# graphdeco-inria/nerfshop

Measured on AMD Instinct MI355X. Metric: render_msamples_per_s_1080p, higher is better.
Workload: dtype f16 storage / f32 accumulate (MFMA), f32 marching+compositing; 1 GPU; lego-like snapshot 1920x1080, one cage edit (BASELINE configs[2]/[4]); samples_per_frame=25213758, frames_in_flight=1, cell_records=levels 0..11, 9.2 GB (nrs_model_set_cell_cache default)

## Files before the change

### include/nrs.h

```cpp
#ifndef NRS_H
#define NRS_H

#include <stddef.h>
#include <stdint.h>

#ifdef __cplusplus
extern "C" {
#endif

#define NRS_ABI_VERSION 3

typedef enum nrs_status {
	NRS_OK = 0,
	NRS_ERR_INVALID_ARG = -1,
	NRS_ERR_UNSUPPORTED = -2,
	NRS_ERR_HIP = -3,
	NRS_ERR_NO_DEVICE = -4,
	NRS_ERR_STATE = -5
} nrs_status;

typedef enum nrs_activation {
	NRS_ACT_NONE = 0, NRS_ACT_RELU = 1, NRS_ACT_LOGISTIC = 2, NRS_ACT_EXPONENTIAL = 3
} nrs_activation;

typedef enum nrs_render_mode {
	NRS_RENDER_AO = 0, NRS_RENDER_SHADE = 1, NRS_RENDER_NORMALS = 2, NRS_RENDER_POSITIONS = 3,
	NRS_RENDER_DEPTH = 4, NRS_RENDER_DISTANCE = 5, NRS_RENDER_STEPSIZE = 6, NRS_RENDER_DISTORTION = 7,
	NRS_RENDER_COST = 8, NRS_RENDER_SLICE = 9, NRS_RENDER_ENCODING_VIS = 11
} nrs_render_mode;

typedef enum nrs_layout { NRS_PLANES = 0, NRS_INTERLEAVED = 1 } nrs_layout;

typedef enum nrs_grid_acc { NRS_GRID_ACC_FP32 = 0, NRS_GRID_ACC_NETWORK = 1 } nrs_grid_acc;
typedef enum nrs_mlp_acc { NRS_MLP_ACC_FP32 = 0, NRS_MLP_ACC_FP16 = 1 } nrs_mlp_acc;

typedef struct nrs_model_desc {
	uint32_t n_levels;
	uint32_t n_features_per_level;
	uint32_t log2_hashmap_size;
	uint32_t base_resolution;
	float    per_level_scale;
	uint32_t n_neurons;
	uint32_t density_hidden_layers;
	uint32_t density_output_dims;
	uint32_t rgb_hidden_layers;
	uint32_t sh_degree;
	uint32_t rgb_activation;
	uint32_t density_activation;
	float    aabb_min[3];
	float    aabb_max[3];
} nrs_model_desc;

#define NRS_GRID_SIZE       128u
#define NRS_GRID_CASCADES   5u
#define NRS_GRID_VOLUME     (128u * 128u * 128u)
#define NRS_BITFIELD_BYTES  (NRS_GRID_VOLUME * NRS_GRID_CASCADES / 8u)
#define NRS_NETWORK_INPUT_FLOATS 7u
#define NRS_NETWORK_OUTPUT_WIDTH 16u

typedef struct nrs_tet_mesh {
	uint32_t        n_vertices;
	uint32_t        n_tets;
	const float*    h_vertices;
	const float*    h_original_vertices;
	const uint32_t* h_tets;
	const uint32_t* h_lut_offsets;
	const uint32_t* h_lut_idx;
	const uint8_t*  h_original_bitfield;
	const float*    h_local_rotations;
	uint32_t        copy;
	uint32_t        apply_poisson;
	float           residual_amplitude;
	const float*    h_boundary_shs;
	const float*    h_boundary_outside_density;
	const float*    h_boundary_residual_density;
	uint32_t        correct_direction;
} nrs_tet_mesh;

typedef struct nrs_affine_duplication {
	float    selection_center[3];
	float    selection_scale[3];
	float    selection_rot[9];
	float    translation[3];
	float    scale[3];
	float    rotation[9];
	uint32_t hide_original;
	uint32_t correct_dir;
} nrs_affine_duplication;

typedef struct nrs_render_params {
	uint32_t struct_size;
	int32_t  resolution[2];
	float    focal_length[2];
	float    camera_matrix0[12];
	float    camera_matrix1[12];
	float    rolling_shutter[4];
	float    screen_center[2];
	float    render_aabb_min[3];
	float    render_aabb_max[3];
	uint32_t spp_index;
	uint32_t snap_to_pixel_centers;
	float    min_transmittance;
	float    cone_angle_constant;
	uint32_t render_mode;
	uint32_t linear_colors;
	uint32_t apply_operators;
	uint32_t poisson_target;
	uint32_t min_mip;
	uint32_t max_march_steps;
	uint32_t tile_size;
	uint32_t tile_first;
	uint32_t tile_stride;
	float    dof;
	float    slice_plane_z;
	float    depth_scale;
	uint32_t show_accel;
	uint32_t distortion_mode;
	float    distortion_params[7];
	const float* d_distortion_map;
	int32_t  distortion_resolution[2];
	int32_t  envmap_resolution[2];
	const float* d_envmap;
	uint32_t glow_mode;
	float    glow_y_cutoff;
	uint32_t visualized_layer;
	uint32_t visualized_dimension;
} nrs_render_params;
#define NRS_RENDER_PARAMS_INIT { (uint32_t)sizeof(nrs_render_params) }

typedef struct nrs_render_stats {
	uint64_t n_samples;
	uint32_t n_rays_alive;
	uint32_t n_rays_hit;
} nrs_render_stats;

typedef struct nrs_grid_update {
	uint32_t n_uniform_samples;
	uint32_t n_nonuniform_samples;
	uint32_t reset_grid;
	uint32_t max_cascade;
	float    decay;
	uint32_t ema_step;
	uint64_t rng_state;
	uint64_t rng_inc;
} nrs_grid_update;

typedef struct nrs_ctx   nrs_ctx;
typedef struct nrs_model nrs_model;
typedef struct nrs_edit  nrs_edit;

const char* nrs_last_error(void);
int         nrs_abi_version(void);

int  nrs_ctx_create(int device, nrs_ctx** out);
void nrs_ctx_destroy(nrs_ctx* ctx);
int  nrs_ctx_device_info(const nrs_ctx* ctx, char* name_out, size_t name_len, int* n_cus, size_t* hbm_bytes);
int  nrs_ctx_set_lane_teams(nrs_ctx* ctx, int lanes_per_ray);
int  nrs_ctx_set_ray_handover(nrs_ctx* ctx, int enabled);
int  nrs_ctx_ray_handovers(const nrs_ctx* ctx, uint64_t* n_rays, uint64_t* n_handovers);

int    nrs_model_create(nrs_ctx* ctx, const nrs_model_desc* desc, nrs_model** out);
void   nrs_model_destroy(nrs_model* model);
size_t nrs_model_n_params(const nrs_model_desc* desc);
int    nrs_model_level_table(const nrs_model_desc* desc, float* scale, uint32_t* resolution,
                             uint32_t* entry_offset, uint32_t* entry_count, uint32_t* hashed);
int    nrs_model_set_params(nrs_model* model, const void* h_params_fp16, size_t n_params);
int    nrs_model_set_params_device(nrs_model* model, const void* d_params_fp16, size_t n_params, void* stream);
int    nrs_model_set_numerics(nrs_model* model, uint32_t grid_acc, uint32_t mlp_acc);
int    nrs_model_set_cell_cache(nrs_model* model, size_t max_bytes);
size_t nrs_model_cell_cache_bytes(const nrs_model* model, uint32_t* n_levels_out);
int    nrs_model_set_sparse_cell_cache(nrs_model* model, const uint8_t* h_mask_bitfield, size_t max_bytes);
size_t nrs_model_sparse_cell_cache_bytes(const nrs_model* model, uint32_t* first_level_out, uint32_t* n_levels_out);
int    nrs_model_set_density_bitfield(nrs_model* model, const uint8_t* h_bitfield, size_t n_bytes);
int    nrs_model_set_density_grid(nrs_model* model, const float* h_grid, size_t n_floats);
int    nrs_model_get_density_bitfield(nrs_model* model, uint8_t* h_bitfield_out, size_t n_bytes);
int    nrs_model_get_march_accelerator(nrs_model* model, int which, float* h_box12, uint32_t* h_mask1024);
int    nrs_model_get_density_grid(nrs_model* model, float* h_grid_out, size_t n_floats);
int    nrs_model_update_density_grid(nrs_model* model, nrs_edit* const* edits, int n_edits, nrs_grid_update* u, void* stream);
void   nrs_rng_seed(uint64_t seed, uint64_t* state_out, uint64_t* inc_out);

typedef struct nrs_comm nrs_comm;
int  nrs_comm_unique_id(uint8_t* out128);
int  nrs_comm_create(int device, int rank, int n_ranks, const uint8_t* unique_id128, nrs_comm** out);
void nrs_comm_destroy(nrs_comm* comm);
int  nrs_comm_info(const nrs_comm* comm, int* rank_out, int* n_ranks_out, int* rccl_version_out, char* lib_path_out, size_t lib_path_len);
int  nrs_comm_probe_self_p2p(nrs_comm* comm, const float* d_src, float* d_dst, size_t n_floats, int pairs, void* stream);
int  nrs_gather_tiles(nrs_ctx* ctx, nrs_comm* comm, int root, const nrs_render_params* p, uint32_t tiles_per_rank_padded, const float* d_local,
                      float* d_recv, float* d_image, float* d_depth, void* stream);

int nrs_network_inference(nrs_model* model, void* stream, uint32_t n, const float* d_in,
                          void* d_out_fp16, uint32_t ld_out, int layout);
int nrs_network_density(nrs_model* model, void* stream, uint32_t n, const float* d_in, uint32_t ld_in,
                        void* d_out_fp16, uint32_t ld_out, int layout);
int nrs_network_input_gradient(nrs_model* model, void* stream, uint32_t n, const float* d_in, uint32_t ld_in, float* d_grad_out_nx3);
int nrs_network_visualize_activation(nrs_model* model, void* stream, uint32_t layer, uint32_t dimension, uint32_t n, const float* d_in, float* d_out_n);
int nrs_network_backward(nrs_model* model, void* stream, uint32_t n, const float* d_in, uint32_t ld_in,
                         const void* d_dL_doutput_fp16, uint32_t ld_dout, int layout, float* d_dL_dparams, size_t n_params, int accumulate,
                         float* d_dL_dinput);
int nrs_density_on_grid(nrs_model* model, void* stream, const uint32_t res3d[3], const float aabb_min[3], const float aabb_max[3],
                        int mask_with_density_grid, float* d_out);
int nrs_rgba_on_grid(nrs_model* model, void* stream, const uint32_t res3d[3], const float render_aabb_min[3],
                     const float render_aabb_max[3], const float ray_dir[3], float* d_out_rgba);
int nrs_project_selection_pixels(nrs_model* model, void* stream, const nrs_render_params* params, const int32_t* d_pixels_xy,
                                 uint32_t n_pixels, float transmittance_threshold, float* d_positions, uint32_t* d_cells, uint8_t* d_found);
uint32_t nrs_upper_cell_idx(uint32_t cell_idx, uint32_t target_level);
int nrs_selection_cells(const float* h_positions, const uint32_t* h_cells, const uint8_t* h_found, uint32_t n, int automatic_max_level,
                        uint32_t* growing_level_inout, uint32_t* out_cells, float* out_positions, uint32_t* n_out);
int  nrs_poisson_boundary(nrs_model* model, const float* h_vertices, uint32_t n_verts, uint32_t sh_width, uint32_t hemisphere_width,
                          const float* h_jitter, int is_inside, float* h_density_out, float* h_sh_out);
void nrs_poisson_sample_coords(const float* vertices, uint32_t n_verts, uint32_t sh_width, uint32_t hemisphere_width, const float* jitter,
                               const float aabb_min[3], const float aabb_max[3], float* coords7_out);
int nrs_hashgrid_encode(nrs_model* model, void* stream, uint32_t n, const float* d_in, uint32_t ld_in,
                        void* d_out_fp16);

int  nrs_edit_create(nrs_ctx* ctx, const nrs_model_desc* desc, const nrs_tet_mesh* mesh, nrs_edit** out);
int  nrs_edit_create_affine(nrs_ctx* ctx, const nrs_model_desc* desc, const nrs_affine_duplication* op, nrs_edit** out);
void nrs_edit_destroy(nrs_edit* edit);
int  nrs_edit_map_rays(nrs_edit* edit, void* stream, uint32_t n, float* d_coords, uint8_t* d_empty_mask);
int  nrs_edit_map_positions(nrs_edit* edit, void* stream, uint32_t n, float* d_pos, uint32_t ld,
                            uint8_t* d_empty_mask);

int  nrs_edit_set_mvc(nrs_edit* edit, const float* h_weights, uint32_t n_cage_vertices);
int  nrs_edit_update_cage(nrs_edit* edit, void* stream, const float* h_cage_vertices, uint32_t n_cage_vertices);
int  nrs_edit_update_vertices(nrs_edit* edit, void* stream, const float* h_vertices, uint32_t n_vertices);
int  nrs_edit_lut_size(const nrs_edit* edit, uint32_t* n_idx_out, uint32_t* max_per_cell_out);
int  nrs_edit_poisson_interpolate(nrs_edit* edit, void* stream, const float* h_gamma, uint32_t n_cage_vertices, const float* h_inside_density,
                                  const float* h_outside_density, const float* h_inside_shs, const float* h_outside_shs, float residual_amplitude);
int  nrs_edit_download_poisson(nrs_edit* edit, float* h_boundary_shs, float* h_outside_density, float* h_residual_density);
int  nrs_edit_download(nrs_edit* edit, float* h_vertices, uint32_t* h_lut_offsets, uint32_t* h_lut_idx, float* h_rotations,
                       uint8_t* h_original_bitfield, float* h_bbox6);

int nrs_render_nerf(nrs_model* model, const nrs_render_params* params, nrs_edit* const* edits, int n_edits,
                    float* d_frame, float* d_depth, uint32_t* d_steps, void* stream, nrs_render_stats* h_stats);
typedef enum nrs_color_space { NRS_COLOR_LINEAR = 0, NRS_COLOR_SRGB = 1, NRS_COLOR_VISPOSNEG = 2 } nrs_color_space;
int nrs_accumulate(nrs_ctx* ctx, void* stream, uint32_t width, uint32_t height, const float* d_frame, float* d_accumulate, uint32_t sample_count, uint32_t color_space);
uint32_t nrs_render_owned_tiles(const nrs_render_params* params);
uint32_t nrs_render_tile_pitch(const nrs_render_params* params);
int nrs_detile(nrs_ctx* ctx, void* stream, const nrs_render_params* params, uint32_t n_ranks,
               uint32_t tiles_per_rank_padded, const float* d_tiles, uint32_t channels, size_t rank_stride_floats, float* d_image);
int nrs_trace_samples(nrs_model* model, const nrs_render_params* params, void* stream, uint32_t n_pixels,
                      const uint32_t* d_pixel_idx, uint32_t max_samples, float* d_t, float* d_dt, uint32_t* d_count);

typedef struct nrs_snapshot nrs_snapshot;
int          nrs_snapshot_open(const char* path, nrs_snapshot** out);
void         nrs_snapshot_close(nrs_snapshot* snapshot);
int          nrs_snapshot_model_desc(const nrs_snapshot* snapshot, nrs_model_desc* desc_out, uint32_t* aabb_scale_out);
const void*  nrs_snapshot_params_fp16(const nrs_snapshot* snapshot, size_t* n_params_out);
const float* nrs_snapshot_density_grid(const nrs_snapshot* snapshot, size_t* n_floats_out);
int          nrs_snapshot_camera(const nrs_snapshot* snapshot, float* camera_matrix12_out);
typedef struct nrs_edits nrs_edits;
int          nrs_edits_open(const char* path, nrs_edits** out);
void         nrs_edits_close(nrs_edits* edits);
uint32_t     nrs_edits_count(const nrs_edits* edits);
const char*  nrs_edits_type(const nrs_edits* edits, uint32_t i);
int          nrs_edits_affine(const nrs_edits* edits, uint32_t i, nrs_affine_duplication* op_out);
int          nrs_edits_cage(const nrs_edits* edits, uint32_t i, nrs_tet_mesh* mesh_out, const float** h_mvc_weights_out,
                            const float** h_cage_vertices_out, const float** h_cage_original_vertices_out,
                            const uint32_t** h_cage_triangles_out, uint32_t* n_cage_vertices_out, uint32_t* n_cage_triangles_out);

typedef struct nrs_tet_lut nrs_tet_lut;
int  nrs_tet_lut_build(const float* h_vertices, uint32_t n_vertices, const uint32_t* h_tets, uint32_t n_tets,
                       int n_threads, nrs_tet_lut** out);
uint32_t        nrs_tet_lut_n_idx(const nrs_tet_lut* lut);
uint32_t        nrs_tet_lut_max_per_cell(const nrs_tet_lut* lut);
const uint32_t* nrs_tet_lut_offsets(const nrs_tet_lut* lut);
const uint32_t* nrs_tet_lut_idx(const nrs_tet_lut* lut);
const uint8_t*  nrs_tet_lut_bitfield(const nrs_tet_lut* lut);
void            nrs_tet_lut_destroy(nrs_tet_lut* lut);
int nrs_mvc_compute(const float* h_cage_vertices, uint32_t n_cage_vertices, const uint32_t* h_cage_triangles,
                    uint32_t n_cage_triangles, const float* h_points, uint32_t n_points,
                    float* h_weights_out, uint8_t* h_labels_out);
int nrs_mvc_apply(const float* h_weights, const float* h_cage_vertices, uint32_t n_cage_vertices,
                  uint32_t n_points, float* h_points_out);
int nrs_tet_local_rotations(const float* h_vertices, const float* h_original_vertices, const uint32_t* h_tets,
                            uint32_t n_tets, float* h_rotations_out);

#define NRS_SPP_BATCH_MAX 64u
#define NRS_SPP_BATCH_MAX_RESOLUTION 8192
int nrs_render_nerf_spp(nrs_model* model, const nrs_render_params* params, nrs_edit* const* edits, int n_edits, uint32_t spp_count,
                        float* d_frames, float* d_depths, uint32_t* d_steps, size_t slab_stride_pixels, void* stream, nrs_render_stats* h_stats);
int nrs_accumulate_spp(nrs_ctx* ctx, void* stream, uint32_t width, uint32_t height, const float* d_frames, size_t slab_stride_pixels, uint32_t spp_count,
                       float* d_accumulate, uint32_t sample_count, uint32_t color_space);
int nrs_ctx_render_launches(const nrs_ctx* ctx, uint64_t* n_dispatches_out, uint32_t* last_schedule_out);

typedef struct nrs_sample_view {
	float camera_matrix0[12], camera_matrix1[12];
	float focal_length[2];
	float dof;
	float slice_plane_z;
} nrs_sample_view;
int nrs_render_nerf_spp_views(nrs_model* model, const nrs_render_params* params, nrs_edit* const* edits, int n_edits, uint32_t spp_count, const nrs_sample_view* h_views,
                              float* d_frames, float* d_depths, uint32_t* d_steps, size_t slab_stride_pixels, void* stream, nrs_render_stats* h_stats);

typedef struct nrs_camera_keyframe { float R[4], T[3], slice, scale, fov, dof; } nrs_camera_keyframe;
typedef struct nrs_camera_path nrs_camera_path;
int nrs_log_space_lerp(const float begin[12], const float end[12], float t, float out[12]);
int nrs_camera_keyframe_matrix(const nrs_camera_keyframe* key, float out[12]);
int nrs_camera_keyframe_from_matrix(const float matrix[12], float slice, float scale, float fov, float dof, nrs_camera_keyframe* out);
int nrs_camera_path_eval(const nrs_camera_keyframe* keys, uint32_t n_keys, float t, nrs_camera_keyframe* out);
int nrs_camera_path_open(const char* path, nrs_camera_path** out);
uint32_t nrs_camera_path_count(const nrs_camera_path* path);
int nrs_camera_path_keyframes(const nrs_camera_path* path, nrs_camera_keyframe* out, uint32_t capacity);
void nrs_camera_path_close(nrs_camera_path* path);
int nrs_motion_views(const float start[12], const float end[12], float shutter_fraction, uint32_t spp_count, uint32_t first_sample, uint32_t spp_total,
                     const int32_t resolution[2], int fov_axis, const nrs_camera_keyframe* keys, uint32_t n_keys, float start_time, float end_time,
                     const nrs_sample_view* base_view, nrs_sample_view* out_views);

int    nrs_model_create_ex(nrs_ctx* ctx, const nrs_model_desc* desc, uint32_t n_extra_dims, nrs_model** out);
size_t nrs_model_n_params_ex(const nrs_model_desc* desc, uint32_t n_extra_dims);
int    nrs_model_n_extra_dims(const nrs_model* model);
int    nrs_model_set_light_dir(nrs_model* model, const float dir[3]);
int    nrs_network_inference_strided(nrs_model* model, void* stream, uint32_t n, const float* d_in, uint32_t ld_in, void* d_out_fp16, uint32_t ld_out, int layout);
#define NRS_SNAPSHOT_ALLOW_LIGHT_DIRS 1u
int      nrs_snapshot_open_ex(const char* path, uint32_t flags, nrs_snapshot** out);
uint32_t nrs_snapshot_n_extra_dims(const nrs_snapshot* snapshot);

typedef enum nrs_tonemap_curve { NRS_TONEMAP_IDENTITY = 0, NRS_TONEMAP_ACES = 1, NRS_TONEMAP_HABLE = 2, NRS_TONEMAP_REINHARD = 3 } nrs_tonemap_curve;
#define NRS_TONEMAP_RGBA32F 0u
#define NRS_TONEMAP_RGBA8 1u
typedef struct nrs_tonemap_params {
	uint32_t struct_size;
	float    exposure;
	float    background_color[4];
	uint32_t color_space;
	uint32_t output_color_space;
	uint32_t tonemap_curve;
	uint32_t clamp_output;
	uint32_t output_format;
} nrs_tonemap_params;
// ... 120 lines not shown
```

### nerfshop_amd/_abi.py

```python
import ctypes as C
import os

_HERE = os.path.dirname(os.path.abspath(__file__))
LIB_PATH = os.environ.get("NRS_LIB_PATH") or os.path.join(_HERE, "csrc", "libnrs.so")

NRS_OK = 0
GRID_SIZE = 128
GRID_CASCADES = 5
GRID_VOLUME = GRID_SIZE ** 3
BITFIELD_BYTES = GRID_VOLUME * GRID_CASCADES // 8
N_LUT_CELLS = GRID_VOLUME * GRID_CASCADES

ACT_NONE, ACT_RELU, ACT_LOGISTIC, ACT_EXPONENTIAL = 0, 1, 2, 3
RENDER_AO, RENDER_SHADE, RENDER_NORMALS, RENDER_POSITIONS, RENDER_DEPTH, RENDER_DISTANCE, RENDER_STEPSIZE, RENDER_DISTORTION, RENDER_COST, RENDER_SLICE = range(10)
RENDER_ENCODING_VIS = 11
LAYOUT_PLANES, LAYOUT_INTERLEAVED = 0, 1


class ModelDesc(C.Structure):
    _fields_ = [
        ("n_levels", C.c_uint32),
        ("n_features_per_level", C.c_uint32),
        ("log2_hashmap_size", C.c_uint32),
        ("base_resolution", C.c_uint32),
# ... 45 lines not shown


class RenderParams(C.Structure):
    _fields_ = [
        ("struct_size", C.c_uint32),
        ("resolution", C.c_int32 * 2),
        ("focal_length", C.c_float * 2),
        ("camera_matrix0", C.c_float * 12),
        ("camera_matrix1", C.c_float * 12),
        ("rolling_shutter", C.c_float * 4),
        ("screen_center", C.c_float * 2),
        ("render_aabb_min", C.c_float * 3),
        ("render_aabb_max", C.c_float * 3),
        ("spp_index", C.c_uint32),
        ("snap_to_pixel_centers", C.c_uint32),
        ("min_transmittance", C.c_float),
        ("cone_angle_constant", C.c_float),
        ("render_mode", C.c_uint32),
        ("linear_colors", C.c_uint32),
        ("apply_operators", C.c_uint32),
        ("poisson_target", C.c_uint32),
        ("min_mip", C.c_uint32),
        ("max_march_steps", C.c_uint32),
        ("tile_size", C.c_uint32),
        ("tile_first", C.c_uint32),
        ("tile_stride", C.c_uint32),
        ("dof", C.c_float),
        ("slice_plane_z", C.c_float),
        ("depth_scale", C.c_float),
        ("show_accel", C.c_uint32),
        ("distortion_mode", C.c_uint32),
        ("distortion_params", C.c_float * 7),
        ("d_distortion_map", C.c_void_p),
        ("distortion_resolution", C.c_int32 * 2),
        ("envmap_resolution", C.c_int32 * 2),
        ("d_envmap", C.c_void_p),
        ("glow_mode", C.c_uint32),
        ("glow_y_cutoff", C.c_float),
        ("visualized_layer", C.c_uint32),
        ("visualized_dimension", C.c_uint32),
    ]

    def __init__(self, *args, **kw):
        super().__init__(*args, **kw)
        self.struct_size = C.sizeof(RenderParams)


class RenderStats(C.Structure):
    _fields_ = [("n_samples", C.c_uint64), ("n_rays_alive", C.c_uint32), ("n_rays_hit", C.c_uint32)]


class GridUpdate(C.Structure):
    _fields_ = [
        ("n_uniform_samples", C.c_uint32),
        ("n_nonuniform_samples", C.c_uint32),
        ("reset_grid", C.c_uint32),
        ("max_cascade", C.c_uint32),
        ("decay", C.c_float),
        ("ema_step", C.c_uint32),
        ("rng_state", C.c_uint64),
        ("rng_inc", C.c_uint64),
    ]


class TonemapParams(C.Structure):
    _fields_ = [
        ("struct_size", C.c_uint32),
        ("exposure", C.c_float),
        ("background_color", C.c_float * 4),
        ("color_space", C.c_uint32),
        ("output_color_space", C.c_uint32),
        ("tonemap_curve", C.c_uint32),
        ("clamp_output", C.c_uint32),
        ("output_format", C.c_uint32),
    ]

    def __init__(self, *args, **kw):
        super().__init__(*args, **kw)
        self.struct_size = C.sizeof(TonemapParams)


class SampleView(C.Structure):
    _fields_ = [("camera_matrix0", C.c_float * 12), ("camera_matrix1", C.c_float * 12), ("focal_length", C.c_float * 2), ("dof", C.c_float), ("slice_plane_z", C.c_float)]


class CameraKeyframe(C.Structure):
    _fields_ = [("R", C.c_float * 4), ("T", C.c_float * 3), ("slice", C.c_float), ("scale", C.c_float), ("fov", C.c_float), ("dof", C.c_float)]


LOSS_L2, LOSS_L1, LOSS_MAPE, LOSS_SMAPE, LOSS_HUBER, LOSS_LOG_L1, LOSS_RELATIVE_L2 = range(7)


class RayLossParams(C.Structure):
    _fields_ = [("struct_size", C.c_uint32), ("loss_type", C.c_uint32), ("loss_scale", C.c_float), ("color_space", C.c_uint32), ("train_in_linear_colors", C.c_uint32),
                ("background", C.c_float * 3), ("near_distance", C.c_float), ("density_l1_reg", C.c_uint32), ("max_samples_compacted", C.c_uint32)]

    def __init__(self, **kw):
        super().__init__()
        self.struct_size = C.sizeof(RayLossParams)
        self.loss_type, self.loss_scale, self.color_space, self.train_in_linear_colors = LOSS_L2, 128.0, 0, 0
        for k, v in kw.items():
            if k == "background":
                self.background = (C.c_float * 3)(*[float(x) for x in v])
            elif k in dict(self._fields_):
                setattr(self, k, v)
            else:
                raise TypeError(f"RayLossParams has no field {k}")


class AdamParams(C.Structure):
    _fields_ = [("struct_size", C.c_uint32), ("beta1", C.c_float), ("beta2", C.c_float), ("epsilon", C.c_float), ("l2_reg", C.c_float),
                ("non_matrix_lr_factor", C.c_float), ("ema_decay", C.c_float)]

    def __init__(self, **kw):
        super().__init__()
        self.struct_size = C.sizeof(AdamParams)
        self.beta1, self.beta2, self.epsilon, self.l2_reg, self.non_matrix_lr_factor, self.ema_decay = 0.9, 0.99, 1e-15, 1e-6, 1.0, 0.95
        for k, v in kw.items():
            if k not in dict(self._fields_):
                raise TypeError(f"AdamParams has no field {k}")
            setattr(self, k, v)


class TrainingCamera(C.Structure):
    _fields_ = [("struct_size", C.c_uint32), ("xform_start", C.c_float * 12), ("xform_end", C.c_float * 12), ("focal_length", C.c_float * 2),
                ("principal_point", C.c_float * 2), ("rolling_shutter", C.c_float * 4), ("distortion_mode", C.c_uint32), ("distortion_params", C.c_float * 7)]

    def __init__(self, *args, **kw):
        super().__init__(*args, **kw)
        self.struct_size = C.sizeof(TrainingCamera)


class DatasetRaysParams(C.Structure):
    _fields_ = [("struct_size", C.c_uint32), ("n_rays_total", C.c_uint32), ("rng_state", C.c_uint64), ("rng_inc", C.c_uint64), ("snap_to_pixel_centers", C.c_uint32),
                ("random_bg_color", C.c_uint32)]

    def __init__(self, *args, **kw):
        super().__init__(*args, **kw)
        self.struct_size = C.sizeof(DatasetRaysParams)


IMAGE_RGBA8_SRGB, IMAGE_RGBA32F_LINEAR, IMAGE_RGBA16F_LINEAR = 0, 1, 2
IMAGE_WHITE_TRANSPARENT, IMAGE_BLACK_TRANSPARENT = 1, 2
RNG_STEP_DELTA = 1 << 32
OPT_MASTER, OPT_M, OPT_V, OPT_STEPS, OPT_EMA, OPT_PARAMS_FP16 = range(6)
OPT_EXPORT_WEIGHTS, OPT_EXPORT_EMA = 0, 1
BASE_LEARNING_RATE, BASE_DECAY_START, BASE_DECAY_INTERVAL, BASE_DECAY_BASE = 1e-2, 20000, 10000, 0.33

EXPORTS = [
    "nrs_last_error", "nrs_abi_version", "nrs_edit_poisson_interpolate", "nrs_edit_download_poisson", "nrs_comm_unique_id", "nrs_comm_create", "nrs_comm_info", "nrs_comm_destroy", "nrs_gather_tiles", "nrs_comm_probe_self_p2p",
    "nrs_ctx_create", "nrs_ctx_destroy", "nrs_ctx_device_info", "nrs_ctx_set_lane_teams", "nrs_ctx_set_ray_handover", "nrs_ctx_ray_handovers",
    "nrs_model_create", "nrs_model_destroy", "nrs_model_n_params", "nrs_model_level_table",
    "nrs_model_set_params", "nrs_model_set_params_device", "nrs_model_set_numerics", "nrs_model_set_cell_cache", "nrs_model_cell_cache_bytes", "nrs_model_set_sparse_cell_cache", "nrs_model_sparse_cell_cache_bytes", "nrs_model_set_density_bitfield", "nrs_model_set_density_grid",
    "nrs_model_get_density_bitfield", "nrs_model_get_march_accelerator", "nrs_model_get_density_grid", "nrs_model_update_density_grid", "nrs_rng_seed",
    "nrs_network_inference", "nrs_network_density", "nrs_hashgrid_encode", "nrs_density_on_grid", "nrs_rgba_on_grid", "nrs_network_input_gradient", "nrs_network_visualize_activation",
    "nrs_poisson_boundary", "nrs_poisson_sample_coords", "nrs_project_selection_pixels", "nrs_upper_cell_idx", "nrs_selection_cells",
    "nrs_edit_create", "nrs_edit_create_affine", "nrs_edit_destroy", "nrs_edit_map_rays", "nrs_edit_map_positions",
    "nrs_edit_set_mvc", "nrs_edit_update_cage", "nrs_edit_update_vertices", "nrs_edit_lut_size", "nrs_edit_download",
    "nrs_render_nerf", "nrs_render_owned_tiles", "nrs_render_tile_pitch", "nrs_detile", "nrs_trace_samples", "nrs_accumulate",
    "nrs_snapshot_open", "nrs_snapshot_close", "nrs_snapshot_model_desc", "nrs_snapshot_params_fp16", "nrs_snapshot_density_grid",
    "nrs_snapshot_camera", "nrs_edits_open", "nrs_edits_close", "nrs_edits_count", "nrs_edits_type", "nrs_edits_cage", "nrs_edits_affine",
    "nrs_tet_lut_build", "nrs_tet_lut_n_idx", "nrs_tet_lut_max_per_cell", "nrs_tet_lut_offsets",
    "nrs_tet_lut_idx", "nrs_tet_lut_bitfield", "nrs_tet_lut_destroy",
    "nrs_mvc_compute", "nrs_mvc_apply", "nrs_tet_local_rotations",
    "nrs_render_nerf_spp", "nrs_accumulate_spp", "nrs_ctx_render_launches",
    "nrs_model_create_ex", "nrs_model_n_params_ex", "nrs_model_n_extra_dims", "nrs_model_set_light_dir", "nrs_network_inference_strided",
    "nrs_snapshot_open_ex", "nrs_snapshot_n_extra_dims",
    "nrs_tonemap", "nrs_accumulate_spp_tonemap", "nrs_tonemap_output_bytes",
    "nrs_render_nerf_spp_views", "nrs_log_space_lerp", "nrs_camera_keyframe_matrix", "nrs_camera_keyframe_from_matrix", "nrs_camera_path_eval",
    "nrs_camera_path_open", "nrs_camera_path_count", "nrs_camera_path_keyframes", "nrs_camera_path_close", "nrs_motion_views",
    "nrs_marching_cubes_res", "nrs_marching_cubes_table", "nrs_mesh_write", "nrs_mesh_from_density", "nrs_mesh_extract", "nrs_mesh_color_inputs",
    "nrs_mesh_counts", "nrs_mesh_device", "nrs_mesh_download", "nrs_mesh_destroy",
    "nrs_selection_create", "nrs_selection_destroy", "nrs_selection_reset", "nrs_selection_grow", "nrs_selection_upscale", "nrs_selection_state",
    "nrs_selection_get_cells", "nrs_selection_get_bitfield", "nrs_selection_set_structuring_elements", "nrs_bitfield_morph", "nrs_bitfield_morph_host",
    "nrs_selection_dilate", "nrs_selection_erode", "nrs_selection_fine_mesh",
    "nrs_network_backward",
    "nrs_training_samples", "nrs_ray_loss",
    "nrs_adam_bias_table", "nrs_exponential_decay_lr", "nrs_optimizer_create", "nrs_optimizer_create_for_model", "nrs_optimizer_destroy", "nrs_optimizer_set_weights",
    "nrs_optimizer_step", "nrs_optimizer_get_state", "nrs_optimizer_set_state", "nrs_optimizer_export_fp16", "nrs_optimizer_step_count", "nrs_optimizer_set_step_count",
    "nrs_optimizer_n_params",
    "nrs_dataset_create", "nrs_dataset_destroy", "nrs_dataset_set_image", "nrs_dataset_set_camera", "nrs_dataset_get_image", "nrs_dataset_rays", "nrs_dataset_mark_untrained", "nrs_rng_advance",
]
SNAPSHOT_ALLOW_LIGHT_DIRS = 1
SPP_BATCH_MAX = 64
COLOR_LINEAR, COLOR_SRGB, COLOR_VISPOSNEG = 0, 1, 2
TONEMAP_IDENTITY, TONEMAP_ACES, TONEMAP_HABLE, TONEMAP_REINHARD = 0, 1, 2, 3
TONEMAP_RGBA32F, TONEMAP_RGBA8 = 0, 1
SE_CUBE, SE_SPHERE = 0, 1
MORPH_DILATE, MORPH_ERODE = 0, 1
MESH_THRESH_DEFAULT = 2.5

_lib = None


class NrsError(RuntimeError):
    pass


def load():
    global _lib
    if _lib is not None:
        return _lib
    if not os.path.exists(LIB_PATH):
        raise NrsError(
            f"{LIB_PATH} is missing: the HIP extension has not been built "
            "(run `python -c 'import __graft_entry__ as g; g.build()'`). There is no CPU fallback.")
    import torch
    lib = C.CDLL(LIB_PATH)
    P, U32, I = C.c_void_p, C.c_uint32, C.c_int
    lib.nrs_last_error.restype = C.c_char_p
    lib.nrs_abi_version.restype = I
    lib.nrs_ctx_create.argtypes = [I, C.POINTER(P)]
    lib.nrs_ctx_destroy.argtypes = [P]
    lib.nrs_ctx_destroy.restype = None
    lib.nrs_ctx_device_info.argtypes = [P, C.c_char_p, C.c_size_t, C.POINTER(I), C.POINTER(C.c_size_t)]
    lib.nrs_model_create.argtypes = [P, C.POINTER(ModelDesc), C.POINTER(P)]
    lib.nrs_ctx_set_lane_teams.argtypes = [P, C.c_int]
    lib.nrs_ctx_set_ray_handover.argtypes = [P, C.c_int]
    lib.nrs_ctx_ray_handovers.argtypes = [P, C.POINTER(C.c_uint64), C.POINTER(C.c_uint64)]
    lib.nrs_model_destroy.argtypes = [P]
    lib.nrs_model_destroy.restype = None
    lib.nrs_model_n_params.argtypes = [C.POINTER(ModelDesc)]
    lib.nrs_model_n_params.restype = C.c_size_t
    lib.nrs_model_level_table.argtypes = [C.POINTER(ModelDesc), P, P, P, P, P]
    lib.nrs_model_set_params.argtypes = [P, P, C.c_size_t]
    lib.nrs_project_selection_pixels.argtypes = [P, P, C.POINTER(RenderParams), P, C.c_uint32, C.c_float, P, P, P]
    lib.nrs_poisson_boundary.argtypes = [P, P, C.c_uint32, C.c_uint32, C.c_uint32, P, C.c_int, P, P]
    lib.nrs_poisson_sample_coords.argtypes = [P, C.c_uint32, C.c_uint32, C.c_uint32, P, P, P, P]
    lib.nrs_poisson_sample_coords.restype = None
    lib.nrs_upper_cell_idx.argtypes = [C.c_uint32, C.c_uint32]
    lib.nrs_upper_cell_idx.restype = C.c_uint32
    lib.nrs_selection_cells.argtypes = [P, P, P, C.c_uint32, C.c_int, P, P, P, P]
    lib.nrs_model_set_cell_cache.argtypes = [P, C.c_size_t]
    lib.nrs_model_cell_cache_bytes.argtypes = [P, P]
    lib.nrs_model_cell_cache_bytes.restype = C.c_size_t
    lib.nrs_model_set_numerics.argtypes = [P, C.c_uint32, C.c_uint32]
    lib.nrs_model_set_params_device.argtypes = [P, P, C.c_size_t, P]
    lib.nrs_edit_poisson_interpolate.argtypes = [P, P, P, C.c_uint32, P, P, P, P, C.c_float]
    lib.nrs_edit_download_poisson.argtypes = [P, P, P, P]
    lib.nrs_comm_unique_id.argtypes = [P]
    lib.nrs_comm_create.argtypes = [C.c_int, C.c_int, C.c_int, P, P]
    lib.nrs_comm_info.argtypes = [P, P, P, P, P, C.c_size_t]
    lib.nrs_comm_destroy.argtypes = [P]
    lib.nrs_comm_destroy.restype = None
    lib.nrs_gather_tiles.argtypes = [P, P, C.c_int, P, C.c_uint32, P, P, P, P, P]
    lib.nrs_comm_probe_self_p2p.argtypes = [P, P, P, C.c_size_t, C.c_int, P]
    lib.nrs_model_set_sparse_cell_cache.argtypes = [P, P, C.c_size_t]
    lib.nrs_model_sparse_cell_cache_bytes.argtypes = [P, P, P]
    lib.nrs_model_sparse_cell_cache_bytes.restype = C.c_size_t
    lib.nrs_model_set_density_bitfield.argtypes = [P, P, C.c_size_t]
    lib.nrs_model_set_density_grid.argtypes = [P, P, C.c_size_t]
    lib.nrs_model_get_density_bitfield.argtypes = [P, P, C.c_size_t]
    lib.nrs_model_get_density_grid.argtypes = [P, P, C.c_size_t]
    lib.nrs_model_get_march_accelerator.argtypes = [P, I, P, P]
    lib.nrs_model_update_density_grid.argtypes = [P, C.POINTER(P), I, C.POINTER(GridUpdate), P]
    lib.nrs_rng_seed.argtypes = [C.c_uint64, C.POINTER(C.c_uint64), C.POINTER(C.c_uint64)]
    lib.nrs_rng_seed.restype = None
    lib.nrs_network_inference.argtypes = [P, P, U32, P, P, U32, I]
    lib.nrs_network_density.argtypes = [P, P, U32, P, U32, P, U32, I]
    lib.nrs_hashgrid_encode.argtypes = [P, P, U32, P, U32, P]
    lib.nrs_network_input_gradient.argtypes = [P, P, U32, P, U32, P]
    lib.nrs_network_visualize_activation.argtypes = [P, P, U32, U32, U32, P, P]
    if hasattr(lib, "nrs_network_backward"):
        lib.nrs_network_backward.argtypes = [P, P, U32, P, U32, P, U32, I, P, C.c_size_t, I, P]
    if hasattr(lib, "nrs_ray_loss"):
        lib.nrs_training_samples.argtypes = [P, P, U32, P, P, C.c_float, U32, P, U32, P, P, P]
        lib.nrs_ray_loss.argtypes = [P, P, C.POINTER(RayLossParams), U32, P, P, U32, P, U32, P, U32, I, P, P, P, P, P, P, U32, I, P, P]
    if hasattr(lib, "nrs_optimizer_step"):
        lib.nrs_adam_bias_table.argtypes = [C.c_float, C.c_float, P, U32, C.POINTER(U32)]
        lib.nrs_exponential_decay_lr.argtypes = [C.c_float, U32, U32, C.c_float, U32]
        lib.nrs_exponential_decay_lr.restype = C.c_float
        lib.nrs_optimizer_create.argtypes = [P, C.c_size_t, C.c_size_t, C.POINTER(AdamParams), C.POINTER(P)]
        lib.nrs_optimizer_create_for_model.argtypes = [P, C.POINTER(AdamParams), C.POINTER(P)]
        lib.nrs_optimizer_destroy.argtypes = [P]
        lib.nrs_optimizer_destroy.restype = None
        lib.nrs_optimizer_set_weights.argtypes = [P, P, I, P]
        lib.nrs_optimizer_step.argtypes = [P, P, P, C.c_float, C.c_float, I]
        lib.nrs_optimizer_get_state.argtypes = [P, I, P, C.c_size_t]
        lib.nrs_optimizer_set_state.argtypes = [P, I, P, C.c_size_t]
        lib.nrs_optimizer_export_fp16.argtypes = [P, I, P, P]
        lib.nrs_optimizer_step_count.argtypes = [P]
        lib.nrs_optimizer_step_count.restype = U32
        lib.nrs_optimizer_set_step_count.argtypes = [P, U32]
        lib.nrs_optimizer_n_params.argtypes = [P, C.POINTER(C.c_size_t)]
        lib.nrs_optimizer_n_params.restype = C.c_size_t
    if hasattr(lib, "nrs_dataset_rays"):
        lib.nrs_dataset_create.argtypes = [P, U32, U32, U32, C.POINTER(P)]
        lib.nrs_dataset_destroy.argtypes = [P]
        lib.nrs_dataset_destroy.restype = None
        lib.nrs_dataset_set_image.argtypes = [P, U32, I, P, I, U32, U32, P]
        lib.nrs_dataset_set_camera.argtypes = [P, U32, C.POINTER(TrainingCamera)]
        lib.nrs_dataset_get_image.argtypes = [P, U32, P]
        lib.nrs_dataset_rays.argtypes = [P, P, C.POINTER(DatasetRaysParams), U32, P, P, P, P, P]
        lib.nrs_dataset_mark_untrained.argtypes = [P, P, I, P]
        lib.nrs_rng_advance.argtypes = [C.POINTER(C.c_uint64), C.c_uint64, C.c_uint64]
        lib.nrs_rng_advance.restype = None
    lib.nrs_density_on_grid.argtypes = [P, P, C.POINTER(U32 * 3), C.POINTER(C.c_float * 3), C.POINTER(C.c_float * 3), I, P]
    lib.nrs_rgba_on_grid.argtypes = [P, P, C.POINTER(U32 * 3), C.POINTER(C.c_float * 3), C.POINTER(C.c_float * 3), C.POINTER(C.c_float * 3), P]
    lib.nrs_edit_create.argtypes = [P, C.POINTER(ModelDesc), C.POINTER(TetMesh), C.POINTER(P)]
    lib.nrs_edit_create_affine.argtypes = [P, C.POINTER(ModelDesc), C.POINTER(AffineDuplicationOp), C.POINTER(P)]
    lib.nrs_edits_affine.argtypes = [P, U32, C.POINTER(AffineDuplicationOp)]
    lib.nrs_edit_destroy.argtypes = [P]
    lib.nrs_edit_destroy.restype = None
    lib.nrs_edit_map_rays.argtypes = [P, P, U32, P, P]
    lib.nrs_edit_map_positions.argtypes = [P, P, U32, P, U32, P]
    lib.nrs_edit_set_mvc.argtypes = [P, P, U32]
    lib.nrs_edit_update_cage.argtypes = [P, P, P, U32]
    lib.nrs_edit_update_vertices.argtypes = [P, P, P, U32]
    lib.nrs_edit_lut_size.argtypes = [P, C.POINTER(U32), C.POINTER(U32)]
    lib.nrs_edit_download.argtypes = [P, P, P, P, P, P, P]
    lib.nrs_render_nerf.argtypes = [P, C.POINTER(RenderParams), C.POINTER(P), I, P, P, P, P, C.POINTER(RenderStats)]
    lib.nrs_render_owned_tiles.argtypes = [C.POINTER(RenderParams)]
    lib.nrs_render_owned_tiles.restype = U32
    lib.nrs_render_tile_pitch.argtypes = [C.POINTER(RenderParams)]
    lib.nrs_render_tile_pitch.restype = U32
    lib.nrs_detile.argtypes = [P, P, C.POINTER(RenderParams), U32, U32, P, U32, C.c_size_t, P]
    lib.nrs_trace_samples.argtypes = [P, C.POINTER(RenderParams), P, U32, P, U32, P, P, P]
    lib.nrs_accumulate.argtypes = [P, P, U32, U32, P, P, U32, U32]
    if hasattr(lib, "nrs_render_nerf_spp"):
        lib.nrs_render_nerf_spp.argtypes = [P, C.POINTER(RenderParams), C.POINTER(P), I, U32, P, P, P, C.c_size_t, P, C.POINTER(RenderStats)]
        lib.nrs_accumulate_spp.argtypes = [P, P, U32, U32, P, C.c_size_t, U32, P, U32, U32]
        lib.nrs_ctx_render_launches.argtypes = [P, C.POINTER(C.c_uint64), C.POINTER(U32)]
    if hasattr(lib, "nrs_model_create_ex"):
        lib.nrs_model_create_ex.argtypes = [P, C.POINTER(ModelDesc), U32, C.POINTER(P)]
        lib.nrs_model_n_params_ex.argtypes = [C.POINTER(ModelDesc), U32]
        lib.nrs_model_n_params_ex.restype = C.c_size_t
        lib.nrs_model_n_extra_dims.argtypes = [P]
        lib.nrs_model_set_light_dir.argtypes = [P, C.POINTER(C.c_float * 3)]
        lib.nrs_network_inference_strided.argtypes = [P, P, U32, P, U32, P, U32, I]
        lib.nrs_snapshot_open_ex.argtypes = [C.c_char_p, U32, C.POINTER(P)]
        lib.nrs_snapshot_n_extra_dims.argtypes = [P]
        lib.nrs_snapshot_n_extra_dims.restype = U32
    if hasattr(lib, "nrs_tonemap"):
        lib.nrs_tonemap.argtypes = [P, P, U32, U32, P, C.POINTER(TonemapParams), P]
        lib.nrs_accumulate_spp_tonemap.argtypes = [P, P, U32, U32, P, C.c_size_t, U32, P, U32, C.POINTER(TonemapParams), P]
        lib.nrs_tonemap_output_bytes.argtypes = [U32, U32, U32]
        lib.nrs_tonemap_output_bytes.restype = C.c_size_t
    if hasattr(lib, "nrs_render_nerf_spp_views"):
        F12 = C.POINTER(C.c_float * 12)
        lib.nrs_render_nerf_spp_views.argtypes = [P, C.POINTER(RenderParams), C.POINTER(P), I, U32, P, P, P, P, C.c_size_t, P, C.POINTER(RenderStats)]
        lib.nrs_log_space_lerp.argtypes = [F12, F12, C.c_float, F12]
        lib.nrs_camera_keyframe_matrix.argtypes = [C.POINTER(CameraKeyframe), F12]
        lib.nrs_camera_keyframe_from_matrix.argtypes = [F12, C.c_float, C.c_float, C.c_float, C.c_float, C.POINTER(CameraKeyframe)]
        lib.nrs_camera_path_eval.argtypes = [P, U32, C.c_float, C.POINTER(CameraKeyframe)]
        lib.nrs_camera_path_open.argtypes = [C.c_char_p, C.POINTER(P)]
        lib.nrs_camera_path_count.argtypes = [P]
        lib.nrs_camera_path_count.restype = U32
        lib.nrs_camera_path_keyframes.argtypes = [P, P, U32]
        lib.nrs_camera_path_close.argtypes = [P]
        lib.nrs_camera_path_close.restype = None
        lib.nrs_motion_views.argtypes = [F12, F12, C.c_float, U32, U32, U32, C.POINTER(C.c_int32 * 2), I, P, U32, C.c_float, C.c_float, C.POINTER(SampleView), P]
    if hasattr(lib, "nrs_mesh_from_density"):
        F3, U3 = C.POINTER(C.c_float * 3), C.POINTER(U32 * 3)
        lib.nrs_marching_cubes_res.argtypes = [U32, F3, F3, U3]
        lib.nrs_marching_cubes_table.argtypes = [P, C.POINTER(U32)]
        lib.nrs_mesh_write.argtypes = [C.c_char_p, U32, P, P, P, U32, P, C.c_float, F3]
        lib.nrs_mesh_from_density.argtypes = [P, P, U3, F3, F3, C.c_float, P, C.POINTER(P)]
        lib.nrs_mesh_extract.argtypes = [P, P, U3, F3, F3, C.c_float, I, I, C.POINTER(P)]
        lib.nrs_mesh_color_inputs.argtypes = [P, P, P, P]
        lib.nrs_mesh_counts.argtypes = [P, C.POINTER(U32), C.POINTER(U32), C.POINTER(U32)]
        lib.nrs_mesh_device.argtypes = [P, C.POINTER(P), C.POINTER(P), C.POINTER(P), C.POINTER(P), C.POINTER(P)]
        lib.nrs_mesh_download.argtypes = [P, P, P, P, P, P]
        lib.nrs_mesh_destroy.argtypes = [P]
        lib.nrs_mesh_destroy.restype = None
    if hasattr(lib, "nrs_selection_create"):
        PU32 = C.POINTER(U32)
        lib.nrs_selection_create.argtypes = [P, C.c_size_t, U32, C.POINTER(P)]
        lib.nrs_selection_destroy.argtypes = [P]
        lib.nrs_selection_destroy.restype = None
        lib.nrs_selection_reset.argtypes = [P, P, U32, U32]
        lib.nrs_selection_grow.argtypes = [P, C.c_float, U32, U32, PU32]
        lib.nrs_selection_upscale.argtypes = [P]
        lib.nrs_selection_state.argtypes = [P, PU32, PU32, PU32, C.POINTER(I)]
        lib.nrs_selection_get_cells.argtypes = [P, P, P]
        lib.nrs_selection_get_bitfield.argtypes = [P, P]
        lib.nrs_selection_set_structuring_elements.argtypes = [P, I, I, I, I]
        lib.nrs_bitfield_morph.argtypes = [P, P, P, U32, I, I, I, P]
        lib.nrs_bitfield_morph_host.argtypes = [P, U32, I, I, I, P]
        lib.nrs_selection_dilate.argtypes = [P, P, P]
        lib.nrs_selection_erode.argtypes = [P, P, P]
        lib.nrs_selection_fine_mesh.argtypes = [P, P, P, I, C.POINTER(P)]
    lib.nrs_snapshot_open.argtypes = [C.c_char_p, C.POINTER(P)]
    lib.nrs_snapshot_close.argtypes = [P]
    lib.nrs_snapshot_close.restype = None
    lib.nrs_snapshot_model_desc.argtypes = [P, C.POINTER(ModelDesc), C.POINTER(U32)]
    lib.nrs_snapshot_params_fp16.argtypes = [P, C.POINTER(C.c_size_t)]
    lib.nrs_snapshot_params_fp16.restype = P
    lib.nrs_snapshot_density_grid.argtypes = [P, C.POINTER(C.c_size_t)]
    lib.nrs_snapshot_density_grid.restype = P
    lib.nrs_snapshot_camera.argtypes = [P, P]
    lib.nrs_edits_open.argtypes = [C.c_char_p, C.POINTER(P)]
    lib.nrs_edits_close.argtypes = [P]
    lib.nrs_edits_close.restype = None
    lib.nrs_edits_count.argtypes = [P]
    lib.nrs_edits_count.restype = U32
    lib.nrs_edits_type.argtypes = [P, U32]
    lib.nrs_edits_type.restype = C.c_char_p
    lib.nrs_edits_cage.argtypes = [P, U32, C.POINTER(TetMesh), C.POINTER(P), C.POINTER(P), C.POINTER(P), C.POINTER(P), C.POINTER(U32), C.POINTER(U32)]
    lib.nrs_tet_lut_build.argtypes = [P, U32, P, U32, I, C.POINTER(P)]
    for name in ("nrs_tet_lut_n_idx", "nrs_tet_lut_max_per_cell"):
        getattr(lib, name).argtypes = [P]
        getattr(lib, name).restype = U32
    for name in ("nrs_tet_lut_offsets", "nrs_tet_lut_idx", "nrs_tet_lut_bitfield"):
        getattr(lib, name).argtypes = [P]
        getattr(lib, name).restype = P
    lib.nrs_tet_lut_destroy.argtypes = [P]
    lib.nrs_tet_lut_destroy.restype = None
# ... 11 lines not shown
```

### nerfshop_amd/csrc/nrs_api_model.cpp

```cpp
#include "nrs_host.h"
#include "nrs_optimizer.h"

#include <cmath>
#include <cstdio>
#include <cstdlib>
#include <new>

using namespace nrs;

static int refresh_accel(nrs_model* m, void* stream) {
	hipStream_t s = (hipStream_t)stream;
	float* d_out = reinterpret_cast<float*>(m->d_accel_masks.get() + 2 * kCoarseWords);
	NRS_LAUNCH(launch_occ_accel(m->dm.bitfield, m->d_accel_masks.get(), d_out, m->d_accel_masks.get() + 2 * kCoarseWords + 24, stream));
	float h[24];
	HIP_TRY(hipMemcpyAsync(h, d_out, sizeof(h), hipMemcpyDeviceToHost, s));
	HIP_TRY(hipStreamSynchronize(s));
	OccAccel* acc[2] = {&m->accel_any, &m->accel_exact};
	for (int f = 0; f < 2; ++f)
		for (int k = 0; k < 3; ++k) {
			acc[f]->box.mn[k] = h[f * 12 + k];
			acc[f]->box.mx[k] = h[f * 12 + 3 + k];
			acc[f]->cell[k] = h[f * 12 + 6 + k];
			acc[f]->inv_cell[k] = h[f * 12 + 9 + k];
		}
	m->accel_any.mask = m->d_accel_masks.get();
	m->accel_exact.mask = m->d_accel_masks.get() + kCoarseWords;
	return NRS_OK;
}
DeviceModel nrs::model_for_launch(const nrs_model* m, const nrs_render_params& p) {
	DeviceModel dm = m->dm;
	dm.occ = (p.cone_angle_constant == 0.f && p.min_mip == 0) ? m->accel_exact : m->accel_any;
	return dm;
}
int nrs::model_refresh_bitfield(nrs_model* m, void* stream) {
	hipStream_t s = (hipStream_t)stream;
	HIP_TRY(hipMemsetAsync(m->d_bitfield.get(), 0, NRS_BITFIELD_BYTES, s));
	NRS_LAUNCH(launch_grid_to_bitfield(m->d_density_grid.get(), m->d_bitfield.get(), m->ctx->d_mean.get(), stream));
	NRS_TRY(refresh_accel(m, stream));
	m->have_bitfield = true;
	return NRS_OK;
}

extern "C" {

static void update_light(nrs_model* m) {
	const float* l = m->light_dir;
	const float n = std::sqrt(l[0] * l[0] + l[1] * l[1] + l[2] * l[2]);
	for (int k = 0; k < 3; ++k) m->dm.light01[k] = (l[k] / n + 1.0f) * 0.5f;
}
int nrs_model_n_extra_dims(const nrs_model* m) { return m ? (int)m->n_extra_dims : 0; }
int nrs_model_set_light_dir(nrs_model* m, const float dir[3]) {
	if (!m || !dir) return fail(NRS_ERR_INVALID_ARG, "nrs_model_set_light_dir: NULL argument");
	const float n2 = dir[0] * dir[0] + dir[1] * dir[1] + dir[2] * dir[2];
	if (!std::isfinite(n2) || !(n2 > 0.f)) return fail(NRS_ERR_INVALID_ARG, "nrs_model_set_light_dir: the direction must be finite and non-zero (it is normalised at use)");
	for (int k = 0; k < 3; ++k) m->light_dir[k] = dir[k];
	update_light(m);
	return NRS_OK;
}
static int model_create(nrs_ctx* ctx, const nrs_model_desc* desc, uint32_t n_extra_dims, nrs_model** out, const char* who) {
	if (!ctx || !desc || !out) return fail(NRS_ERR_INVALID_ARG, std::string(who) + ": NULL argument");
	if (n_extra_dims != 0u && n_extra_dims != 3u) return fail(NRS_ERR_UNSUPPORTED, "nrs_model_create_ex: n_extra_dims must be 0 or 3 (light directions, dataset.has_light_dirs)");
	if (desc_supported(*desc))
		if (const char* why = extra_dims_refusal(*desc, n_extra_dims)) return fail(NRS_ERR_UNSUPPORTED, std::string("nrs_model_create_ex: ") + why);
	if (!desc_supported(*desc)) return fail(NRS_ERR_UNSUPPORTED, "model description outside configs/nerf/base.json's family (hash grid 16 x 2, 64-wide density network of 0..1 hidden layers, rgb network of 0..3 hidden layers or none)");
	for (int k = 0; k < 3; ++k)
		if (!(desc->aabb_max[k] > desc->aabb_min[k])) return fail(NRS_ERR_INVALID_ARG, std::string(who) + ": empty aabb");
	HIP_TRY(hipSetDevice(ctx->device));
	nrs_model* m = new (std::nothrow) nrs_model();
	if (!m) return fail(NRS_ERR_STATE, "out of host memory");
	m->ctx = ctx;
	m->desc = *desc;
	m->total_entries = make_levels(*desc, m->dm.levels);
	for (int k = 0; k < 3; ++k) { m->dm.aabb.mn[k] = desc->aabb_min[k]; m->dm.aabb.mx[k] = desc->aabb_max[k]; }
	m->dm.diag_pow2 = 1;
	for (int k = 0; k < 3; ++k) {
		const float diag = desc->aabb_max[k] - desc->aabb_min[k];
		int e = 0;
		if (std::frexp(diag, &e) != 0.5f) m->dm.diag_pow2 = 0;
		m->dm.inv_diag[k] = 1.0f / diag;
	}
	m->dm.rgb_deep = desc->sh_degree != 0 && desc->rgb_hidden_layers == 3 ? 1u : 0u;
	m->dm.no_dir = desc->sh_degree == 0 ? 1u : 0u;
	m->n_extra_dims = m->dm.n_extra_dims = n_extra_dims;
	update_light(m);
	m->dm.rgb_activation = desc->rgb_activation;
	m->dm.density_activation = desc->density_activation;
	hipError_t he = m->d_grid.alloc(m->total_entries);
	if (he == hipSuccess) he = m->d_wfrag.alloc(kWfragDeviceBytes / 2);
	if (he == hipSuccess) he = m->d_bitfield.alloc(NRS_BITFIELD_BYTES);
	if (he == hipSuccess) he = m->d_accel_masks.alloc(2 * kCoarseWords + 64);
	if (he == hipSuccess) he = hipMemset(m->d_accel_masks.get(), 0, 2 * kCoarseWords * 4);
	if (he == hipSuccess) he = m->d_density_grid.alloc((size_t)kGridVol * kCascades);
	if (he == hipSuccess) he = hipMemset(m->d_density_grid.get(), 0, (size_t)kGridVol * kCascades * 4);
	if (he != hipSuccess) {
		nrs_model_destroy(m);
		return fail_hip(he, n_extra_dims ? "nrs_model_create_ex: device allocation" : "nrs_model_create: device allocation");
	}
	m->dm.grid = m->d_grid.get();
	m->dm.wfrag = m->d_wfrag.get();
	m->dm.bitfield = m->d_bitfield.get();
	if (const char* e = getenv("NRS_CELL_CACHE_GB")) {
		size_t budget = (size_t)(atof(e) * 1073741824.0), free_b = 0, total_b = 0;
		if (hipMemGetInfo(&free_b, &total_b) == hipSuccess) budget = std::min(budget, free_b / 4);
		if (nrs_model_set_cell_cache(m, budget) != NRS_OK) (void)nrs_model_set_cell_cache(m, 0);
	}
	*out = m;
	return NRS_OK;
}
int nrs_model_create(nrs_ctx* ctx, const nrs_model_desc* desc, nrs_model** out) { return model_create(ctx, desc, 0u, out, "nrs_model_create"); }
int nrs_model_create_ex(nrs_ctx* ctx, const nrs_model_desc* desc, uint32_t n_extra_dims, nrs_model** out) { return model_create(ctx, desc, n_extra_dims, out, "nrs_model_create_ex"); }
void nrs_model_destroy(nrs_model* m) {
	delete m;
}
static uint32_t plan_cell_cache(const LevelParams* lv, size_t budget, LevelParams* out, size_t* bytes) {
	uint32_t n = 0;
	uint64_t records = 0, fit = 0;
	for (uint32_t l = 0; l < kLevels; ++l) {
		const uint64_t cells = (uint64_t)lv[l].resolution * lv[l].resolution * lv[l].resolution;
		if ((records + cells) * 32ull > budget || records + cells >= (1ull << 32) || lv[l].resolution >= 4096u) break;
		records += cells;
		if (l & 1u) { n = l + 1; fit = records; }
	}
	uint64_t first = 0;
	for (uint32_t l = 0; l < kLevels; ++l) {
		out[l] = lv[l];
		out[l].cached = l < n ? 1u : 0u;
		out[l].rec_first = l < n ? (uint32_t)first : 0u;
		out[l].rec_res = l < n ? lv[l].resolution : 0u;
		out[l].rec_res2 = out[l].rec_res * out[l].rec_res;
		if (l < n) first += (uint64_t)lv[l].resolution * lv[l].resolution * lv[l].resolution;
	}
	*bytes = (size_t)fit * 32;
	return n;
}
static int rebuild_cell_cache(nrs_model* m, void* stream = nullptr, bool sync = true) {
	if (!m->have_params) return NRS_OK;
	if (m->cached_levels) NRS_LAUNCH(launch_cell_records(m->dm, m->cached_levels, m->d_records.get(), stream));
	for (uint32_t l = m->sparse_first; l < m->sparse_first + m->sparse_levels; ++l)
		NRS_LAUNCH(launch_brick_fill(m->dm, m->dm.levels[l], m->d_slots.get() + m->slot_first[l], m->slot_count[l], m->d_records2.get(), stream));
	if (sync) HIP_TRY(hipStreamSynchronize((hipStream_t)stream));
	return NRS_OK;
}
static void drop_sparse_cell_cache(nrs_model* m) {
	m->d_bricks.reset(); m->d_slots.reset(); m->d_records2.reset();
	m->sparse_bytes = 0; m->sparse_first = m->sparse_levels = 0;
	for (uint32_t l = 0; l < kLevels; ++l)
		if (m->dm.levels[l].cached == 2u) { m->dm.levels[l].cached = 0; m->dm.levels[l].rec_first = m->dm.levels[l].rec_res = m->dm.levels[l].rec_res2 = m->dm.levels[l].tab_first = 0; }
	m->dm.records2 = nullptr; m->dm.bricks = nullptr;
}
static int mark_sparse_bricks(nrs_model* m, const uint8_t* h_mask_bitfield, size_t max_bytes) {
	const uint32_t first = m->cached_levels;
	DeviceBuffer<uint8_t> d_mask;
	DeviceBuffer<uint32_t> d_counter, d_tmp_table;
	hipError_t he = d_mask.alloc(NRS_BITFIELD_BYTES);
	if (he == hipSuccess) he = hipMemcpy(d_mask.get(), h_mask_bitfield, NRS_BITFIELD_BYTES, hipMemcpyHostToDevice);
	if (he == hipSuccess) he = d_counter.alloc(kLevels);
	if (he == hipSuccess) he = hipMemset(d_counter.get(), 0, 4 * kLevels);
	if (he != hipSuccess) { (void)hipGetLastError(); return fail(NRS_ERR_HIP, "nrs_model_set_sparse_cell_cache: out of device memory"); }
	LevelParams lv[kLevels];
	uint32_t counts[kLevels] = {}, nbs[kLevels] = {};
	uint64_t used = 0, table_total = 0, bricks_total = 0;
	uint32_t n_ok = 0;
	for (uint32_t l = first; l + 1 < kLevels; l += 2) {
		uint64_t pair_bytes = 0, pair_tables = 0, pair_bricks = 0;
		bool ok = true;
		for (uint32_t k = l; k < l + 2 && ok; ++k) {
			const uint32_t nb = (m->dm.levels[k].resolution + kBrick - 1) / kBrick;
			const uint64_t entries = (uint64_t)nb * nb * nb;
			if (entries * 4ull > max_bytes - std::min<uint64_t>(max_bytes, used + pair_bytes) || table_total + pair_tables + entries >= (1ull << 32)) { ok = false; break; }
			if (d_tmp_table.alloc(entries) != hipSuccess || hipMemset(d_tmp_table.get(), 0, entries * 4ull) != hipSuccess) { (void)hipGetLastError(); ok = false; break; }
			lv[k] = m->dm.levels[k];
			lv[k].rec_res = nb; lv[k].rec_res2 = nb * nb; lv[k].tab_first = 0; lv[k].rec_first = 0;
			NRS_LAUNCH(launch_brick_mark(m->dm, lv[k], d_mask.get(), d_tmp_table.get(), d_counter.get() + k, nullptr, 0, nullptr));
			if (hipMemcpy(&counts[k], d_counter.get() + k, 4, hipMemcpyDeviceToHost) != hipSuccess) return fail(NRS_ERR_HIP, "nrs_model_set_sparse_cell_cache: read-back");
			d_tmp_table.reset();
			nbs[k] = nb;
			pair_tables += entries; pair_bricks += counts[k];
			pair_bytes += entries * 4ull + (uint64_t)counts[k] * ((uint64_t)kBrickCells * 32ull + 4ull);
			if (dev_knob("NRS_SPARSE_LOG"))
				fprintf(stderr, "[nrs sparse] level %u: res %u, %u^3 bricks (table %.1f MB), %u bricks marked = %.2f GB of records\n", k, m->dm.levels[k].resolution, nb, entries * 4e-6,
				        counts[k], counts[k] * 16384e-9);
		}
		if (!ok || used + pair_bytes > max_bytes || (bricks_total + pair_bricks) * kBrickCells >= (1ull << 32)) break;
		used += pair_bytes; table_total += pair_tables; bricks_total += pair_bricks;
		n_ok += 2;
	}
	if (!n_ok || !bricks_total) return NRS_OK;
	he = m->d_bricks.alloc(table_total);
	if (he == hipSuccess) he = hipMemset(m->d_bricks.get(), 0, table_total * 4ull);
	if (he == hipSuccess) he = m->d_slots.alloc(bricks_total);
	if (he == hipSuccess) he = m->d_records2.alloc(bricks_total * kBrickCells * 2ull);
	if (he == hipSuccess) he = hipMemset(d_counter.get(), 0, 4 * kLevels);
	if (he != hipSuccess) { (void)hipGetLastError(); return fail(NRS_ERR_HIP, "nrs_model_set_sparse_cell_cache: out of device memory (records)"); }
	m->dm.records2 = m->d_records2.get(); m->dm.bricks = m->d_bricks.get();
	uint64_t tab = 0, slot0 = 0;
	for (uint32_t l = first; l < first + n_ok; ++l) {
		lv[l].tab_first = (uint32_t)tab;
		lv[l].rec_first = (uint32_t)(slot0 * kBrickCells);
		NRS_LAUNCH(launch_brick_mark(m->dm, lv[l], d_mask.get(), m->d_bricks.get() + tab, d_counter.get() + l, m->d_slots.get() + slot0, counts[l], nullptr));
		m->slot_first[l] = (uint32_t)slot0; m->slot_count[l] = counts[l];
		lv[l].cached = 2u;
		m->dm.levels[l] = lv[l];
		tab += (uint64_t)nbs[l] * nbs[l] * nbs[l];
		slot0 += counts[l];
	}
	m->sparse_first = first; m->sparse_levels = n_ok;
	m->sparse_bytes = (size_t)used;
	return NRS_OK;
}
int nrs_model_set_sparse_cell_cache(nrs_model* m, const uint8_t* h_mask_bitfield, size_t max_bytes) {
	if (!m) return fail(NRS_ERR_INVALID_ARG, "nrs_model_set_sparse_cell_cache: NULL model");
	HIP_TRY(hipSetDevice(m->ctx->device));
	HIP_TRY(hipDeviceSynchronize());
	drop_sparse_cell_cache(m);
	if (!h_mask_bitfield || !max_bytes) return NRS_OK;
	if (const int st = mark_sparse_bricks(m, h_mask_bitfield, max_bytes)) {
		drop_sparse_cell_cache(m);
		return st;
	}
	return m->sparse_levels ? rebuild_cell_cache(m) : NRS_OK;
}
size_t nrs_model_sparse_cell_cache_bytes(const nrs_model* m, uint32_t* first_level, uint32_t* n_levels) {
	if (!m) return 0;
	if (first_level) *first_level = m->sparse_first;
	if (n_levels) *n_levels = m->sparse_levels;
	return m->sparse_bytes;
}
int nrs_model_set_cell_cache(nrs_model* m, size_t max_bytes) {
	if (!m) return fail(NRS_ERR_INVALID_ARG, "nrs_model_set_cell_cache: NULL model");
	HIP_TRY(hipSetDevice(m->ctx->device));
	HIP_TRY(hipDeviceSynchronize());
	drop_sparse_cell_cache(m);
	LevelParams lv[kLevels];
	size_t bytes = 0;
	const uint32_t n = plan_cell_cache(m->dm.levels, max_bytes, lv, &bytes);
	if (bytes != m->records_bytes) {
		m->d_records.reset();
		m->records_bytes = 0;
		m->cached_levels = 0;
		for (uint32_t l = 0; l < kLevels; ++l) { m->dm.levels[l].cached = 0; }
		m->dm.records = nullptr;
		if (bytes && m->d_records.alloc(bytes / sizeof(uint4)) != hipSuccess) {
			(void)hipGetLastError();
			return fail(NRS_ERR_HIP, "nrs_model_set_cell_cache: out of device memory for the cell records");
// ... 18 lines not shown
	if (n_mlp) *n_mlp = k;
	if (n_params) *n_params = (size_t)k + (size_t)m->total_entries * 2;
}
uint16_t* nrs::model_grid_fp16(nrs_model* m) { return (uint16_t*)m->d_grid.get(); }
int nrs::model_mlp_from_device(nrs_model* m, const uint16_t* d, void* stream) {
	if (!m->d_wfrag_src.get()) {
		static_assert(kDensityW + 64 * 48 + 2 * 64 * 64 + 16 * 64 < kFragNegate, "weight indices + 1 fit 15 bits");
		std::vector<uint16_t> ident(n_mlp_weights(m->desc, m->n_extra_dims)), canon(kCanonW), src(kWfragDeviceBytes / 2);
		for (size_t i = 0; i < ident.size(); ++i) ident[i] = (uint16_t)(i + 1);
		lower_weights(m->desc, ident.data(), canon.data(), kLowerIndices, m->n_extra_dims);
		make_weight_fragments(canon.data(), src.data(), kFragOne);
		DeviceBuffer<uint16_t> fresh;
		HIP_TRY(fresh.alloc(kWfragDeviceBytes / 2));
		const hipError_t up = hipMemcpy(fresh.get(), src.data(), kWfragDeviceBytes, hipMemcpyHostToDevice);
		if (up != hipSuccess) return fail_hip(up, "nrs_model_set_params_device: upload of the weight permutation");
		m->d_wfrag_src = std::move(fresh);
	}
	NRS_LAUNCH(launch_weight_fragments(d, m->d_wfrag_src.get(), (uint16_t*)m->d_wfrag.get(), kWfragDeviceBytes / 2, stream));
	return NRS_OK;
}
int nrs::model_grid_written(nrs_model* m, void* stream) {
	m->have_params = true;
	return rebuild_cell_cache(m, stream, false);
}
extern "C" {

int nrs_model_set_params(nrs_model* m, const void* h_params_fp16, size_t n_params) {
	if (!m || !h_params_fp16) return fail(NRS_ERR_INVALID_ARG, "nrs_model_set_params: NULL argument");
	const uint32_t n_mlp = n_mlp_weights(m->desc, m->n_extra_dims);
	const size_t expect = (size_t)n_mlp + (size_t)m->total_entries * 2;
	if (n_params != expect) {
		char buf[160];
		snprintf(buf, sizeof(buf), "nrs_model_set_params: got %zu params, the description implies %zu", n_params, expect);
		return fail(NRS_ERR_INVALID_ARG, buf);
	}
	HIP_TRY(hipSetDevice(m->ctx->device));
	const uint16_t* w = (const uint16_t*)h_params_fp16;
	std::vector<uint16_t> canon(kCanonW), frag(kWfragDeviceBytes / 2);
	lower_weights(m->desc, w, canon.data(), kLowerValues, m->n_extra_dims);
	make_weight_fragments(canon.data(), frag.data());
	HIP_TRY(hipMemcpy(m->d_wfrag.get(), frag.data(), kWfragDeviceBytes, hipMemcpyHostToDevice));
	HIP_TRY(hipMemcpy(m->d_grid.get(), w + n_mlp, (size_t)m->total_entries * 4, hipMemcpyHostToDevice));
	m->have_params = true;
	return rebuild_cell_cache(m);
}
int nrs_model_set_params_device(nrs_model* m, const void* d_params_fp16, size_t n_params, void* stream) {
	if (!m || !d_params_fp16) return fail(NRS_ERR_INVALID_ARG, "nrs_model_set_params_device: NULL argument");
	const uint32_t n_mlp = n_mlp_weights(m->desc, m->n_extra_dims);
	const size_t expect = (size_t)n_mlp + (size_t)m->total_entries * 2;
	if (n_params != expect) {
		char buf[160];
		snprintf(buf, sizeof(buf), "nrs_model_set_params_device: got %zu params, the description implies %zu", n_params, expect);
		return fail(NRS_ERR_INVALID_ARG, buf);
	}
	HIP_TRY(hipSetDevice(m->ctx->device));
	const uint16_t* d = (const uint16_t*)d_params_fp16;
	NRS_TRY(model_mlp_from_device(m, d, stream));
	HIP_TRY(hipMemcpyAsync(m->d_grid.get(), d + n_mlp, (size_t)m->total_entries * 4, hipMemcpyDeviceToDevice, (hipStream_t)stream));
	return model_grid_written(m, stream);
}
int nrs_model_set_numerics(nrs_model* m, uint32_t grid_acc, uint32_t mlp_acc) {
	if (!m) return fail(NRS_ERR_INVALID_ARG, "nrs_model_set_numerics: NULL model");
	if (grid_acc > NRS_GRID_ACC_NETWORK || mlp_acc > NRS_MLP_ACC_FP16) return fail(NRS_ERR_INVALID_ARG, "nrs_model_set_numerics: unknown mode");
	m->dm.numerics = (grid_acc == NRS_GRID_ACC_NETWORK ? 1u : 0u) | (mlp_acc == NRS_MLP_ACC_FP16 ? 2u : 0u);
	return NRS_OK;
}
int nrs_model_set_density_bitfield(nrs_model* m, const uint8_t* h_bitfield, size_t n_bytes) {
	if (!m || !h_bitfield) return fail(NRS_ERR_INVALID_ARG, "nrs_model_set_density_bitfield: NULL argument");
	if (n_bytes != NRS_BITFIELD_BYTES) return fail(NRS_ERR_INVALID_ARG, "nrs_model_set_density_bitfield: expected 5*128^3/8 bytes");
	HIP_TRY(hipSetDevice(m->ctx->device));
	HIP_TRY(hipMemcpy(m->d_bitfield.get(), h_bitfield, n_bytes, hipMemcpyHostToDevice));
	NRS_TRY(refresh_accel(m, nullptr));
	m->have_bitfield = true;
	return NRS_OK;
}
int nrs_model_set_density_grid(nrs_model* m, const float* h_grid, size_t n_floats) {
	if (!m || !h_grid) return fail(NRS_ERR_INVALID_ARG, "nrs_model_set_density_grid: NULL argument");
	if (n_floats != (size_t)kGridVol * kCascades) return fail(NRS_ERR_INVALID_ARG, "nrs_model_set_density_grid: expected 5*128^3 floats");
	HIP_TRY(hipSetDevice(m->ctx->device));
	HIP_TRY(hipMemcpy(m->d_density_grid.get(), h_grid, n_floats * 4, hipMemcpyHostToDevice));
	return model_refresh_bitfield(m, nullptr);
}
int nrs_model_get_density_grid(nrs_model* m, float* h_out, size_t n_floats) {
	if (!m || !h_out || n_floats != (size_t)kGridVol * kCascades) return fail(NRS_ERR_INVALID_ARG, "nrs_model_get_density_grid: bad argument");
	HIP_TRY(hipSetDevice(m->ctx->device));
	HIP_TRY(hipMemcpy(h_out, m->d_density_grid.get(), n_floats * 4, hipMemcpyDeviceToHost));
	return NRS_OK;
}

static const uint64_t kPcgMult = 0x5851f42d4c957f2dULL;
static uint64_t pcg_advance(uint64_t state, uint64_t inc, uint64_t delta) {
	uint64_t cur_mult = kPcgMult, cur_plus = inc, acc_mult = 1u, acc_plus = 0u;
	while (delta > 0) {
		if (delta & 1) { acc_mult *= cur_mult; acc_plus = acc_plus * cur_mult + cur_plus; }
		cur_plus = (cur_mult + 1) * cur_plus;
		cur_mult *= cur_mult;
		delta >>= 1;
	}
	return acc_mult * state + acc_plus;
}
void nrs_rng_advance(uint64_t* state, uint64_t inc, uint64_t delta) {
	if (state) *state = pcg_advance(*state, inc, delta);
}
void nrs_rng_seed(uint64_t seed, uint64_t* state_out, uint64_t* inc_out) {
	const uint64_t inc = (1u << 1u) | 1u;
	uint64_t state = 0u;
	state = state * kPcgMult + inc;
	state += seed;
	state = state * kPcgMult + inc;
	if (state_out) *state_out = state;
	if (inc_out) *inc_out = inc;
}

int nrs_model_update_density_grid(nrs_model* m, nrs_edit* const* edits, int n_edits, nrs_grid_update* u, void* stream) {
	if (!m || !u) return fail(NRS_ERR_INVALID_ARG, "nrs_model_update_density_grid: NULL argument");
	if (!m->have_params) return fail(NRS_ERR_STATE, "nrs_model_update_density_grid: parameters not set (nrs_model_set_params)");
	if (u->max_cascade >= kCascades) return fail(NRS_ERR_INVALID_ARG, "nrs_model_update_density_grid: max_cascade must be < 5");
	if (n_edits < 0 || n_edits > nrs_ctx::kMaxEdits) return fail(NRS_ERR_INVALID_ARG, "nrs_model_update_density_grid: too many edit operators");
	if (n_edits > 0 && !edits) return fail(NRS_ERR_INVALID_ARG, "nrs_model_update_density_grid: edits is NULL");
	if ((uint64_t)u->n_uniform_samples + u->n_nonuniform_samples > 0x40000000ull)
		return fail(NRS_ERR_INVALID_ARG, "nrs_model_update_density_grid: more than 2^30 samples");
	nrs_ctx* ctx = m->ctx;
	HIP_TRY(hipSetDevice(ctx->device));
	hipStream_t s = (hipStream_t)stream;
	const size_t grid_bytes = (size_t)kGridVol * kCascades * 4;
	if (!m->d_density_tmp.get()) HIP_TRY(m->d_density_tmp.alloc((size_t)kGridVol * kCascades));
	DeviceEdit* d_refresh_edits = ctx->d_edits.get() + (size_t)nrs_ctx::kInFlight * nrs_ctx::kMaxEdits;
	if (n_edits > 0) {
		DeviceEdit host_edits[nrs_ctx::kMaxEdits];
		for (int i = 0; i < n_edits; ++i) {
			if (!edits[i]) return fail(NRS_ERR_INVALID_ARG, "nrs_model_update_density_grid: NULL edit operator");
			host_edits[i] = edits[i]->de;
		}
		HIP_TRY(hipMemcpyAsync(d_refresh_edits, host_edits, sizeof(DeviceEdit) * n_edits, hipMemcpyHostToDevice, s));
		HIP_TRY(hipStreamSynchronize(s));
	}
	if (u->reset_grid) HIP_TRY(hipMemsetAsync(m->d_density_grid.get(), 0, grid_bytes, s));
	HIP_TRY(hipMemsetAsync(m->d_density_tmp.get(), 0, grid_bytes, s));
	const uint64_t rng_nonuniform = pcg_advance(u->rng_state, u->rng_inc, 1ull << 32);
	NRS_LAUNCH(launch_grid_update(m->dm, d_refresh_edits, n_edits, *u, rng_nonuniform, m->d_density_grid.get(), m->d_density_tmp.get(), ctx->n_cus, stream));
	u->rng_state = pcg_advance(u->rng_state, u->rng_inc, 2ull << 32);
	u->ema_step += 1;
	return model_refresh_bitfield(m, stream);
}
int nrs_model_get_march_accelerator(nrs_model* m, int which, float* h_box12, uint32_t* h_mask) {
	if (!m || !h_box12 || !h_mask || which < 0 || which > 1) return fail(NRS_ERR_INVALID_ARG, "nrs_model_get_march_accelerator: bad argument");
	if (!m->have_bitfield) return fail(NRS_ERR_STATE, "nrs_model_get_march_accelerator: occupancy not set (nrs_model_set_density_bitfield/_grid)");
	HIP_TRY(hipSetDevice(m->ctx->device));
	const OccAccel& a = which ? m->accel_exact : m->accel_any;
	for (int k = 0; k < 3; ++k) { h_box12[k] = a.box.mn[k]; h_box12[3 + k] = a.box.mx[k]; h_box12[6 + k] = a.cell[k]; h_box12[9 + k] = a.inv_cell[k]; }
	HIP_TRY(hipMemcpy(h_mask, a.mask, kCoarseWords * 4, hipMemcpyDeviceToHost));
	return NRS_OK;
}
int nrs_model_get_density_bitfield(nrs_model* m, uint8_t* h_out, size_t n_bytes) {
	if (!m || !h_out || n_bytes != NRS_BITFIELD_BYTES) return fail(NRS_ERR_INVALID_ARG, "nrs_model_get_density_bitfield: bad argument");
	HIP_TRY(hipSetDevice(m->ctx->device));
	HIP_TRY(hipMemcpy(h_out, m->d_bitfield.get(), n_bytes, hipMemcpyDeviceToHost));
	return NRS_OK;
}

}
```

### nerfshop_amd/csrc/nrs_device.cuh

```cuda
#pragma once
#include <hip/hip_runtime.h>
#include "nrs_internal.h"

namespace nrs {

struct f3 { float x, y, z; };
__device__ __forceinline__ f3 mk3(float x, float y, float z) { return f3{x, y, z}; }
__device__ __forceinline__ f3 operator+(f3 a, f3 b) { return {a.x + b.x, a.y + b.y, a.z + b.z}; }
__device__ __forceinline__ f3 operator-(f3 a, f3 b) { return {a.x - b.x, a.y - b.y, a.z - b.z}; }
__device__ __forceinline__ f3 operator*(f3 a, float s) { return {a.x * s, a.y * s, a.z * s}; }
__device__ __forceinline__ f3 operator*(float s, f3 a) { return {s * a.x, s * a.y, s * a.z}; }
__device__ __forceinline__ float sum3(float a, float b, float c) { return a + (b + c); }
__device__ __forceinline__ float dot3(f3 a, f3 b) { return sum3(a.x * b.x, a.y * b.y, a.z * b.z); }
__device__ __forceinline__ f3 mat3_mul(const float* M, f3 v) {
	return {sum3(M[0] * v.x, M[3] * v.y, M[6] * v.z), sum3(M[1] * v.x, M[4] * v.y, M[7] * v.z), sum3(M[2] * v.x, M[5] * v.y, M[8] * v.z)};
}
__device__ __forceinline__ f3 cross3(f3 a, f3 b) { return {a.y * b.z - a.z * b.y, a.z * b.x - a.x * b.z, a.x * b.y - a.y * b.x}; }

__device__ __forceinline__ bool box_contains(const Box3& b, f3 p) {
	return p.x >= b.mn[0] && p.x <= b.mx[0] && p.y >= b.mn[1] && p.y <= b.mx[1] && p.z >= b.mn[2] && p.z <= b.mx[2];
}

#define NRS_SQRT3 1.73205080757f
#define NRS_MIN_STEP (NRS_SQRT3 / 1024)
// ... 193 lines not shown
		apply_camera_distortion(prm, x0 + step0, x1, f00, f01);
		apply_camera_distortion(prm, x0, x1 - step1, b10, b11);
		apply_camera_distortion(prm, x0, x1 + step1, f10, f11);
		const float J00 = 1 + (f00 - b00) / (2 * step0), J01 = (f10 - b10) / (2 * step1), J10 = (f01 - b01) / (2 * step0), J11 = 1 + (f11 - b11) / (2 * step1);
		const float invdet = 1.0f / (J00 * J11 - J10 * J01);
		const float i00 = J11 * invdet, i10 = -J10 * invdet, i01 = -J01 * invdet, i11 = J00 * invdet;
		const float r0 = x0 + dx0 - x00, r1 = x1 + dx1 - x01;
		const float s0 = i00 * r0 + i01 * r1, s1 = i10 * r0 + i11 * r1;
		x0 -= s0; x1 -= s1;
		if (s0 * s0 + s1 * s1 < kMaxStepNorm) break;
	}
	u = x0; v = x1;
}
template <typename P>
__device__ __forceinline__ bool f_theta_undistortion(P prm, float uvx, float uvy, float cx, float cy, f3& dir) {
	const float xpix = (uvx - cx) * prm[5], ypix = (uvy - cy) * prm[6];
	const float norm = sqrtf(xpix * xpix + ypix * ypix);
	const float alpha = prm[0] + norm * (prm[1] + norm * (prm[2] + norm * (prm[3] + norm * prm[4])));
	float sin_alpha, cos_alpha;
	sincosf(alpha, &sin_alpha, &cos_alpha);
	if (cos_alpha <= 1.17549435e-38f || norm == 0.f) return false;
	sin_alpha *= 1.f / norm;
	dir = {sin_alpha * xpix, sin_alpha * ypix, cos_alpha};
	return true;
}
__device__ __forceinline__ void read_image2(const float* __restrict__ data, const int32_t* res, float px, float py, float& o0, float& o1) {
	const float fx = px * (float)(res[0] - 1), fy = py * (float)(res[1] - 1);
	const int tx = (int)fx, ty = (int)fy;
	const float wx = fx - (float)tx, wy = fy - (float)ty;
	const int x0 = max(min(tx, res[0] - 1), 0), x1 = max(min(tx + 1, res[0] - 1), 0), y0 = max(min(ty, res[1] - 1), 0), y1 = max(min(ty + 1, res[1] - 1), 0);
	const float2* d = reinterpret_cast<const float2*>(data);
	const float2 a = d[x0 + y0 * res[0]], b = d[x1 + y0 * res[0]], c = d[x0 + y1 * res[0]], e = d[x1 + y1 * res[0]];
	const float w00 = (1 - wx) * (1 - wy), w10 = (wx) * (1 - wy), w01 = (1 - wx) * (wy), w11 = (wx) * (wy);
	o0 = ((w00 * a.x + w10 * b.x) + w01 * c.x) + w11 * e.x;
	o1 = ((w00 * a.y + w10 * b.y) + w01 * c.y) + w11 * e.y;
}
__device__ __forceinline__ float4 read_envmap(const float* __restrict__ data, const int32_t* res, f3 dir) {
	const float PI = 3.14159265358979323846f;
	const f3 d = {dir.z, -dir.x, dir.y};
	const float theta = acosf(fminf(fmaxf(d.z, -1.0f), 1.0f));
	const float phi = atan2f(d.y, d.x);
	const float cyl_x = theta / PI, cyl_y = (phi / (2.0f * PI) + 0.5f);
	const float fx = cyl_y * (float)(res[0] - 1), fy = cyl_x * (float)(res[1] - 1);
	const int tx = (int)fx, ty = (int)fy;
	const float wx = fx - (float)tx, wy = fy - (float)ty;
	auto wrapx = [&](int x) { return x < 0 ? x + res[0] : (x >= res[0] ? x - res[0] : x); };
	const int x0 = wrapx(tx), x1 = wrapx(tx + 1), y0 = max(min(ty, res[1] - 1), 0), y1 = max(min(ty + 1, res[1] - 1), 0);
	const float4* q = reinterpret_cast<const float4*>(data);
	const float4 a = q[x0 + y0 * res[0]], b = q[x1 + y0 * res[0]], c = q[x0 + y1 * res[0]], e = q[x1 + y1 * res[0]];
	const float w00 = (1 - wx) * (1 - wy), w10 = (wx) * (1 - wy), w01 = (1 - wx) * (wy), w11 = (wx) * (wy);
	return make_float4(((w00 * a.x + w10 * b.x) + w01 * c.x) + w11 * e.x, ((w00 * a.y + w10 * b.y) + w01 * c.y) + w11 * e.y,
	                   ((w00 * a.z + w10 * b.z) + w01 * c.z) + w11 * e.z, ((w00 * a.w + w10 * b.w) + w01 * c.w) + w11 * e.w);
}

#define NRS_GLOBAL __attribute__((address_space(1)))
#define NRS_CONSTANT __attribute__((address_space(4)))
template <bool LENS = false, bool SPP = false, bool UNIFORM = false>
__device__ __forceinline__ void pixel_ray_raw(const nrs_render_params& p, uint32_t x, uint32_t y, float off_x, float off_y, float focus_z, f3& o, f3& d, bool use_dof = true, uint32_t spp = 0u,
                                              const nrs_sample_view* vw = nullptr) {
	const float W = (float)p.resolution[0], H = (float)p.resolution[1];
	const uint32_t idx = x + (uint32_t)p.resolution[0] * y;
	float u = ((float)x + 0.5f) * (1.f / W);
	float v = ((float)y + 0.5f) * (1.f / H);
	float ray_time = p.rolling_shutter[0] + p.rolling_shutter[1] * u + p.rolling_shutter[2] * v;
	float rs_rand = (p.rolling_shutter[3] != 0.f) ? ld_random_val(SPP ? spp : p.spp_index, idx * 72239731u) : 0.f;
	ray_time = ray_time + p.rolling_shutter[3] * rs_rand;
	float cam[12], v_focal_x = 0.f, v_focal_y = 0.f, v_dof = 0.f;
	const bool viewed = SPP && vw;
	if (!viewed) {
		#pragma unroll
		for (int i = 0; i < 12; ++i) cam[i] = p.camera_matrix0[i] * ray_time + p.camera_matrix1[i] * (1.f - ray_time);
	} else {
		if (UNIFORM) {
			const NRS_CONSTANT float* c = (const NRS_CONSTANT float*)vw;
			v_focal_x = c[24]; v_focal_y = c[25]; v_dof = c[26];
			if (use_dof) focus_z = c[27];
		} else {
			const NRS_GLOBAL float* c = (const NRS_GLOBAL float*)vw;
			v_focal_x = c[24]; v_focal_y = c[25]; v_dof = c[26];
			if (use_dof) focus_z = c[27];
		}
	}
	float uvx = ((float)x + off_x) / W;
	float uvy = ((float)y + off_y) / H;
	f3 dir = {(uvx - p.screen_center[0]) * W / (viewed ? v_focal_x : p.focal_length[0]), (uvy - p.screen_center[1]) * H / (viewed ? v_focal_y : p.focal_length[1]), 1.0f};
	if (LENS && p.distortion_mode == 2u) {
		if (!f_theta_undistortion(p.distortion_params, uvx, uvy, p.screen_center[0], p.screen_center[1], dir)) {
			o = mk3(1000.f, 0.f, 0.f); d = mk3(0.f, 0.f, 1.f);
			return;
		}
	} else if (LENS && p.distortion_mode == 1u) {
		iterative_camera_undistortion(p.distortion_params, dir.x, dir.y);
	}
	if (LENS && p.d_distortion_map) {
		float d0, d1;
		read_image2(p.d_distortion_map, p.distortion_resolution, uvx, uvy, d0, d1);
		dir.x += d0; dir.y += d1;
	}
	if (viewed) {
		static_assert(offsetof(nrs_sample_view, camera_matrix1) == 48 && offsetof(nrs_sample_view, focal_length) == 96 && offsetof(nrs_sample_view, slice_plane_z) == 108, "record layout");
		if (UNIFORM) {
			const NRS_CONSTANT float* c = (const NRS_CONSTANT float*)vw;
			#pragma unroll
			for (int i = 0; i < 12; ++i) cam[i] = c[i] * ray_time + c[12 + i] * (1.f - ray_time);
		} else {
			const NRS_GLOBAL float* c = (const NRS_GLOBAL float*)vw;
			#pragma unroll
			for (int i = 0; i < 12; ++i) cam[i] = c[i] * ray_time + c[12 + i] * (1.f - ray_time);
		}
	}
	d = mat3_mul(cam, dir);
	o = {cam[9], cam[10], cam[11]};
	if (LENS && use_dof && (viewed ? v_dof : p.dof) != 0.0f) {
		const f3 lookat = o + d * focus_z;
		float r0, r1, bx, by;
		ld_random_val_2d(SPP ? spp : p.spp_index, x * 19349663u + y * 96925573u, r0, r1);
		square2disk_shirley(r0 * 2.0f - 1.0f, r1 * 2.0f - 1.0f, bx, by);
		bx = (viewed ? v_dof : p.dof) * bx; by = (viewed ? v_dof : p.dof) * by;
		o = {o.x + (cam[0] * bx + cam[3] * by), o.y + (cam[1] * bx + cam[4] * by), o.z + (cam[2] * bx + cam[5] * by)};
		const f3 diff = lookat - o;
		d = {diff.x / focus_z, diff.y / focus_z, diff.z / focus_z};
	}
}
template <bool LENS = false, bool SPP = false, bool UNIFORM = false>
__device__ __forceinline__ void ray_origin_dir(const nrs_render_params& p, uint32_t x, uint32_t y, float off_x, float off_y, f3& o, f3& d, uint32_t spp = 0u, const nrs_sample_view* vw = nullptr) {
	pixel_ray_raw<LENS, SPP, UNIFORM>(p, x, y, off_x, off_y, p.slice_plane_z, o, d, true, spp, vw);
	float n = sqrtf(dot3(d, d));
	d = {d.x / n, d.y / n, d.z / n};
}

template <bool LENS = false, bool SPP = false>
__device__ __forceinline__ Ray init_ray(const nrs_render_params& p, uint32_t x, uint32_t y, float off_x, float off_y, uint32_t spp = 0u, const nrs_sample_view* vw = nullptr) {
	Ray r;
	ray_origin_dir<LENS, SPP, SPP>(p, x, y, off_x, off_y, r.o, r.d, spp, vw);
	float tmin;
	ray_intersect(p.render_aabb_min, p.render_aabb_max, r.o, r.d, tmin);
	r.t = fmaxf(tmin, NRS_NEAR_DISTANCE) + 1e-6f;
	Box3 bb;
	#pragma unroll
	for (int i = 0; i < 3; ++i) { bb.mn[i] = p.render_aabb_min[i]; bb.mx[i] = p.render_aabb_max[i]; }
	r.alive = box_contains(bb, r.o + r.d * r.t);
	return r;
}

__device__ __forceinline__ bool ray_meets_box_ahead(const Box3& b, f3 o, f3 idir, float t) {
	const float ax = (b.mn[0] - o.x) * idir.x, bx = (b.mx[0] - o.x) * idir.x;
	const float ay = (b.mn[1] - o.y) * idir.y, by = (b.mx[1] - o.y) * idir.y;
	const float az = (b.mn[2] - o.z) * idir.z, bz = (b.mx[2] - o.z) * idir.z;
	const float tnear = fmaxf(fmaxf(fminf(ax, bx), fminf(ay, by)), fmaxf(fminf(az, bz), t));
	const float tfar = fminf(fminf(fmaxf(ax, bx), fmaxf(ay, by)), fmaxf(az, bz));
	return tnear <= tfar;
}

__device__ __forceinline__ float coarse_safe_until(const DeviceModel& m, const uint32_t* __restrict__ mask, f3 o, f3 d, f3 idir, float t) {
	const Box3& b = m.occ.box;
	const float ax = (b.mn[0] - o.x) * idir.x, bx = (b.mx[0] - o.x) * idir.x;
	const float ay = (b.mn[1] - o.y) * idir.y, by = (b.mx[1] - o.y) * idir.y;
	const float az = (b.mn[2] - o.z) * idir.z, bz = (b.mx[2] - o.z) * idir.z;
	const float tnear = fmaxf(fmaxf(fminf(ax, bx), fminf(ay, by)), fmaxf(fminf(az, bz), t));
	const float tfar = fminf(fminf(fmaxf(ax, bx), fmaxf(ay, by)), fmaxf(az, bz));
	if (!(tnear <= tfar)) return -1.f;
	const f3 p = o + d * tnear;
	const float hi = (float)(kCoarse - 1);
	int cx = (int)__builtin_amdgcn_fmed3f((p.x - b.mn[0]) * m.occ.inv_cell[0], 0.f, hi);
	int cy = (int)__builtin_amdgcn_fmed3f((p.y - b.mn[1]) * m.occ.inv_cell[1], 0.f, hi);
	int cz = (int)__builtin_amdgcn_fmed3f((p.z - b.mn[2]) * m.occ.inv_cell[2], 0.f, hi);
	const int sx = d.x >= 0.f ? 1 : -1, sy = d.y >= 0.f ? 1 : -1, sz = d.z >= 0.f ? 1 : -1;
	const float inf = __builtin_huge_valf();
	float tmx = d.x != 0.f ? ((b.mn[0] + (float)(cx + (sx > 0 ? 1 : 0)) * m.occ.cell[0]) - o.x) * idir.x : inf;
	float tmy = d.y != 0.f ? ((b.mn[1] + (float)(cy + (sy > 0 ? 1 : 0)) * m.occ.cell[1]) - o.y) * idir.y : inf;
	float tmz = d.z != 0.f ? ((b.mn[2] + (float)(cz + (sz > 0 ? 1 : 0)) * m.occ.cell[2]) - o.z) * idir.z : inf;
	const float tdx = fabsf(m.occ.cell[0] * idir.x), tdy = fabsf(m.occ.cell[1] * idir.y), tdz = fabsf(m.occ.cell[2] * idir.z);
	float t_enter = tnear;
	#pragma unroll 1
	for (int it = 0; it < (int)(3 * kCoarse); ++it) {
		const uint32_t idx = ((uint32_t)cz * kCoarse + (uint32_t)cy) * kCoarse + (uint32_t)cx;
		if ((mask[idx >> 5] >> (idx & 31)) & 1u) return fmaxf(t_enter - 1e-4f, 0.f);
		const bool step_x = tmx <= tmy && tmx <= tmz, step_y = !step_x && tmy <= tmz, step_z = !step_x && !step_y;
		t_enter = step_x ? tmx : (step_y ? tmy : tmz);
		cx += step_x ? sx : 0; cy += step_y ? sy : 0; cz += step_z ? sz : 0;
		tmx += step_x ? tdx : 0.f; tmy += step_y ? tdy : 0.f; tmz += step_z ? tdz : 0.f;
		if ((uint32_t)(cx | cy | cz) > kCoarse - 1) return -1.f;
	}
	return 0.f;
}

constexpr uint32_t kJumpMinSteps = 14u;
__device__ __forceinline__ bool lattice_jump(f3 o, f3 d, f3 idir, float t_safe, uint32_t mip, float& t) {
	const float margin = 0.02f * (float)(1u << mip);
	const float k_want = floorf((t_safe - t - margin) * (1.0f / NRS_MIN_STEP));
	bool ok = k_want >= (float)kJumpMinSteps && k_want < 60000.0f;
	float k_left = ok ? k_want : 0.0f;
	float tc = t;
	#pragma unroll 1
	for (int seg = 0; seg < 2; ++seg) {
		const uint32_t b = __float_as_uint(tc);
		const int e_t = (int)(b >> 23);
		const float x = ldexpf(NRS_MIN_STEP, 150 - e_t), qf = rintf(x);
		const bool seg_ok = e_t >= 24 && e_t <= 137 && fabsf(x - qf) != 0.5f && qf >= 1.0f && qf < 8388608.0f;
		const float left = (float)(0x7fffffu - (b & 0x7fffffu));
		const float k_bin = fmaxf(floorf(left * __builtin_amdgcn_rcpf(qf)) - 1.0f, 0.0f);
		const float k = seg_ok ? fminf(k_left, k_bin) : 0.0f;
		tc = __uint_as_float(b + (uint32_t)k * (uint32_t)qf);
		k_left -= k;
		#pragma unroll
		for (int i = 0; i < 3; ++i) {
			const bool step = k_left > 0.0f;
			tc = step ? tc + NRS_MIN_STEP : tc;
			k_left = step ? k_left - 1.0f : k_left;
		}
	}
	ok = ok && (k_want - k_left) >= (float)kJumpMinSteps + 8.0f;
	ok = ok && mip_from_pos(o + d * t) == 0 && mip_from_pos(o + d * tc) == 0;
	__builtin_amdgcn_sched_barrier(0);
	const uint32_t bk = __float_as_uint(tc);
	const float q_here = rintf(ldexpf(NRS_MIN_STEP, 150 - (int)(bk >> 23)));
	const uint32_t back = 4u * (uint32_t)q_here;
	const uint32_t res = kGrid >> mip;
	const float inv_res = ldexpf(1.0f, (int)mip - 7);
	const float B = (fmaxf(fmaxf(fabsf(idir.x), fabsf(idir.y)), fabsf(idir.z)) + 1.0f) * 2e-6f * fmaxf(t_safe, 1.0f);
	bool taken = false;
	float t_new = t;
	#pragma unroll 1
	for (uint32_t attempt = 0; attempt < 3u; ++attempt) {
		const bool in_binade = attempt == 0u || (bk & 0x7fffffu) >= attempt * back + (uint32_t)q_here;
		const float tk = __uint_as_float(bk - (in_binade ? attempt * back : 0u));
		const f3 pk = o + d * tk;
		const float g = tk + distance_to_next_voxel(pk, d, idir, res, inv_res);
		float u = tk + NRS_MIN_STEP;
		#pragma unroll
		for (int i = 0; i < 7; ++i) {
			const float mstep = __builtin_amdgcn_fmed3f((g - u) * 0x1p100f, 0.0f, 1.0f);
			u = fmaf(mstep, NRS_MIN_STEP, u);
		}
		bool pass = ok && in_binade && u >= g;
		pass = pass && (g + NRS_MIN_STEP + B < t_safe);
		pass = pass && (u - g > B) && (g - (u - NRS_MIN_STEP) > B);
		t_new = (pass && !taken) ? u : t_new;
		taken = taken || pass;
		if (!__any(ok && !taken)) break;
	}
	t = t_new;
	return taken;
}

constexpr float kJumpSpan = 0.06f;
constexpr int kLookEvery = 6;
constexpr uint32_t kMarchLdsWords = kCoarseWords + kGrid;
__device__ __forceinline__ void stage_march_lds(uint32_t* __restrict__ lds, const uint32_t* __restrict__ mask) {
	for (uint32_t i = threadIdx.x; i < kCoarseWords; i += blockDim.x) lds[i] = mask[i];
	for (uint32_t i = threadIdx.x; i < kGrid; i += blockDim.x) lds[kCoarseWords + i] = expand_bits(i);
}
struct OccWord { uint32_t tag; uint32_t lo, hi; };
__device__ __forceinline__ uint32_t occupancy_bit_index(f3 pos, uint32_t mip, const uint32_t* __restrict__ march_lds) {
	const float mip_scale = ldexpf(1.0f, -(int)mip);
	f3 q = pos - mk3(0.5f, 0.5f, 0.5f);
	q = q * mip_scale;
	q = q + mk3(0.5f, 0.5f, 0.5f);
	const int ix = (int)(q.x * (float)kGrid), iy = (int)(q.y * (float)kGrid), iz = (int)(q.z * (float)kGrid);
	const uint32_t* spread = march_lds + kCoarseWords;
	return (spread[clampi_(ix, 0, kGrid - 1)] | (spread[clampi_(iy, 0, kGrid - 1)] << 1) | (spread[clampi_(iz, 0, kGrid - 1)] << 2)) + mip * kGridVol;
}
__device__ __forceinline__ bool occupied_at_cached(f3 pos, const uint8_t* __restrict__ bitfield, uint32_t mip, const uint32_t* __restrict__ march_lds, OccWord& w) {
	const uint32_t idx = occupancy_bit_index(pos, mip, march_lds);
	const uint32_t tag = idx >> 6;
	if (tag != w.tag) {
		const uint2 v = reinterpret_cast<const uint2*>(bitfield)[tag];
		w.tag = tag; w.lo = v.x; w.hi = v.y;
	}
	const uint32_t bit = idx & 63u;
	return (((bit & 32u) ? w.hi : w.lo) >> (bit & 31u)) & 1u;
}
__device__ __forceinline__ bool occupied_at(f3 pos, const uint8_t* __restrict__ bitfield, uint32_t mip, const uint32_t* __restrict__ march_lds) {
	const float mip_scale = ldexpf(1.0f, -(int)mip);
	f3 q = pos - mk3(0.5f, 0.5f, 0.5f);
	q = q * mip_scale;
	q = q + mk3(0.5f, 0.5f, 0.5f);
	const int ix = (int)(q.x * (float)kGrid), iy = (int)(q.y * (float)kGrid), iz = (int)(q.z * (float)kGrid);
	const uint32_t* spread = march_lds + kCoarseWords;
	const uint32_t idx = spread[clampi_(ix, 0, kGrid - 1)] | (spread[clampi_(iy, 0, kGrid - 1)] << 1) | (spread[clampi_(iz, 0, kGrid - 1)] << 2);
	return get_bitfield_at(idx, mip, bitfield);
}
template <bool JUMP = false>
__device__ __forceinline__ bool march_to_occupied(const nrs_render_params& p, const DeviceModel& m, const uint32_t* __restrict__ march_lds, f3 o, f3 d,
                                                  float& t, f3& pos, float& dt, uint32_t* n_iter = nullptr) {
	const uint32_t* __restrict__ coarse_mask = march_lds;
	const uint8_t* __restrict__ bitfield = m.bitfield;
	const Box3& occ_box = m.occ.box;
	Box3 bb;
	#pragma unroll
	for (int i = 0; i < 3; ++i) { bb.mn[i] = p.render_aabb_min[i]; bb.mx[i] = p.render_aabb_max[i]; }
	const float cone = p.cone_angle_constant;
	int until_look = 0;
	uint32_t mip;
	bool in_occ;
	OccWord occ_word{0xffffffffu, 0u, 0u};
	#define NRS_OCCUPIED(pos_, mip_) occupied_at_cached(pos_, bitfield, mip_, march_lds, occ_word)
	if (n_iter) ++*n_iter;
	pos = o + d * t;
	if (!box_contains(bb, pos)) return false;
	dt = calc_dt(t, cone);
	mip = max(p.min_mip, (uint32_t)mip_from_dt(dt, pos));
	in_occ = box_contains(occ_box, pos);
	if (in_occ && NRS_OCCUPIED(pos, mip)) return true;
	const f3 idir = mk3(1.0f / d.x, 1.0f / d.y, 1.0f / d.z);
	bool first = true;
	while (1) {
		if (!first) {
			if (n_iter) ++*n_iter;
			pos = o + d * t;
			if (!box_contains(bb, pos)) return false;
			dt = calc_dt(t, cone);
			mip = max(p.min_mip, (uint32_t)mip_from_dt(dt, pos));
			in_occ = box_contains(occ_box, pos);
			if (in_occ && NRS_OCCUPIED(pos, mip)) return true;
		}
		first = false;
		if (!in_occ && !ray_meets_box_ahead(occ_box, o, idir, t)) return false;
		if (until_look-- == 0) {
			until_look = kLookEvery;
			float t_safe = coarse_safe_until(m, coarse_mask, o, d, idir, t);
			if (t_safe < 0.f) return false;
			{
				const float ax = (bb.mn[0] - o.x) * idir.x, bx = (bb.mx[0] - o.x) * idir.x;
				const float ay = (bb.mn[1] - o.y) * idir.y, by = (bb.mx[1] - o.y) * idir.y;
				const float az = (bb.mn[2] - o.z) * idir.z, bz = (bb.mx[2] - o.z) * idir.z;
				t_safe = fminf(t_safe, fminf(fminf(fmaxf(ax, bx), fmaxf(ay, by)), fmaxf(az, bz)) - 1e-4f);
			}
			while (1) {
				if (JUMP && cone == 0.f && t_safe - t > kJumpSpan && lattice_jump(o, d, idir, t_safe, mip, t)) {
					if (n_iter) ++*n_iter;
					pos = o + d * t;
					dt = calc_dt(t, cone);
					mip = max(p.min_mip, (uint32_t)mip_from_dt(dt, pos));
				}
				const uint32_t lres = kGrid >> mip;
				const float linv = ldexpf(1.0f, (int)mip - 7);
				const float border = t + distance_to_next_voxel(pos, d, idir, lres, linv);
				if (!(border + calc_dt(border, cone) < t_safe)) break;
				t = advance_to_next_voxel(t, cone, pos, d, idir, lres, linv);
				if (n_iter) ++*n_iter;
				pos = o + d * t;
				dt = calc_dt(t, cone);
				mip = max(p.min_mip, (uint32_t)mip_from_dt(dt, pos));
			}
		}
		uint32_t res = kGrid >> mip;
		t = advance_to_next_voxel(t, cone, pos, d, idir, res, ldexpf(1.0f, (int)mip - 7));
	}
	#undef NRS_OCCUPIED
}

__device__ __forceinline__ bool stands_in_occupied_cell(const nrs_render_params& p, const DeviceModel& m, const uint32_t* __restrict__ march_lds, f3 o, f3 d, float t) {
	Box3 bb;
	#pragma unroll
	for (int i = 0; i < 3; ++i) { bb.mn[i] = p.render_aabb_min[i]; bb.mx[i] = p.render_aabb_max[i]; }
	const f3 pos = o + d * t;
	if (!box_contains(bb, pos)) return false;
	const float dt = calc_dt(t, p.cone_angle_constant);
	const uint32_t mip = max(p.min_mip, (uint32_t)mip_from_dt(dt, pos));
	if (!box_contains(m.occ.box, pos)) return false;
	return occupied_at(pos, m.bitfield, mip, march_lds);
}

template <bool SPP = false>
__device__ __forceinline__ bool first_hit(const nrs_render_params& p, const DeviceModel& m, const uint32_t* __restrict__ march_lds, uint32_t pixel_idx, Ray& r,
                                          uint32_t* n_iter = nullptr, uint32_t spp = 0u) {
	float dt = calc_dt(r.t, p.cone_angle_constant);
	r.t += ld_random_val(SPP ? spp : p.spp_index, pixel_idx * 786433u) * dt;
	f3 pos;
	return march_to_occupied<true>(p, m, march_lds, r.o, r.d, r.t, pos, dt, n_iter);
}

__device__ __forceinline__ float scalar_tp(f3 a, f3 b, f3 c) { return dot3(a, cross3(b, c)); }
__device__ __forceinline__ bool same_side_tet(f3 v1, f3 v2, f3 v3, f3 v4, f3 p) {
	f3 normal = cross3(v2 - v1, v3 - v1);
	float dotV4 = dot3(normal, v4 - v1);
	float dotP = dot3(normal, p - v1);
	return signbit(dotV4) == signbit(dotP);
}
__device__ __forceinline__ bool point_in_tet(f3 v1, f3 v2, f3 v3, f3 v4, f3 p) {
	return same_side_tet(v1, v2, v3, v4, p) && same_side_tet(v2, v3, v4, v1, p) && same_side_tet(v3, v4, v1, v2, p) &&
	       same_side_tet(v4, v1, v2, v3, p);
}
__device__ __forceinline__ void bary_tet(f3 a, f3 b, f3 c, f3 d, f3 p, float out[4]) {
	f3 vap = p - a, vbp = p - b, vab = b - a, vac = c - a, vad = d - a, vbc = c - b, vbd = d - b;
	float va6 = scalar_tp(vbp, vbd, vbc);
	float vb6 = scalar_tp(vap, vac, vad);
	float vc6 = scalar_tp(vap, vad, vab);
	float vd6 = scalar_tp(vap, vab, vac);
	float v6 = (float)(1. / (double)scalar_tp(vab, vac, vad));
	out[0] = va6 * v6; out[1] = vb6 * v6; out[2] = vc6 * v6; out[3] = vd6 * v6;
}
template <typename T>
__device__ __forceinline__ const NRS_GLOBAL T* gp(const T* p) { return (const NRS_GLOBAL T*)p; }
__device__ __forceinline__ f3 ld3(const float* __restrict__ a, uint32_t i) {
	typedef float f3a __attribute__((ext_vector_type(3), aligned(4)));
	const f3a v = *(const NRS_GLOBAL f3a*)(gp(a) + 3 * (size_t)i);
	return {v.x, v.y, v.z};
}

__device__ __forceinline__ bool point_in_tet_rec(const float* __restrict__ recs, uint32_t t, f3 p) {
	typedef float f4n __attribute__((ext_vector_type(4)));
	const NRS_GLOBAL f4n* q = gp(reinterpret_cast<const f4n*>(recs)) + 8 * (size_t)t;
	const f4n v0 = q[0], v1 = q[1], v2 = q[2], n0 = q[3], n1 = q[4], n2 = q[5], sg = q[6];
	const float d0 = dot3(mk3(n0.x, n0.y, n0.z), p - mk3(v0.x, v0.y, v0.z));
	const float d1 = dot3(mk3(n0.w, n1.x, n1.y), p - mk3(v0.w, v1.x, v1.y));
	const float d2 = dot3(mk3(n1.z, n1.w, n2.x), p - mk3(v1.z, v1.w, v2.x));
	const float d3 = dot3(mk3(n2.y, n2.z, n2.w), p - mk3(v2.y, v2.z, v2.w));
	const uint32_t got = (__float_as_uint(d0) >> 31) | ((__float_as_uint(d1) >> 31) << 1) | ((__float_as_uint(d2) >> 31) << 2) | ((__float_as_uint(d3) >> 31) << 3);
	return got == __float_as_uint(sg.x);
}
__device__ __forceinline__ uint32_t scan_entries_for_tet(const DeviceEdit& e, const NRS_GLOBAL uint32_t* lut_idx, uint32_t j0, uint32_t j1, uint32_t t, f3 p, uint32_t* n_tested) {
	uint32_t found = 0xffffffffu;
	#pragma unroll 1
	for (uint32_t j = j0; j < j1; ++j) {
		const uint32_t t_next = lut_idx[min(j + 1, j1 - 1)];
		if (n_tested) ++*n_tested;
		if (point_in_tet_rec(e.planes, t, p)) { found = t; break; }
		t = t_next;
	}
	return found;
}
__device__ __forceinline__ uint32_t scan_list_for_tet(const DeviceEdit& e, const uint32_t* __restrict__ off, const uint32_t* __restrict__ idx, uint32_t cell, f3 p, uint32_t* n_tested = nullptr) {
	const NRS_GLOBAL uint32_t* lut_off = gp(off);
	const NRS_GLOBAL uint32_t* lut_idx = gp(idx);
	const uint32_t j0 = lut_off[cell], j1 = lut_off[cell + 1];
	if (j0 >= j1) return 0xffffffffu;
	return scan_entries_for_tet(e, lut_idx, j0, j1, lut_idx[j0], p, n_tested);
}
__device__ __forceinline__ uint32_t scan_cell_for_tet(const DeviceEdit& e, uint32_t cell, f3 p, uint32_t* n_tested = nullptr) { return scan_list_for_tet(e, e.lut_off, e.lut_idx, cell, p, n_tested); }
__device__ __forceinline__ uint32_t scan_fine_cell_for_tet(const DeviceEdit& e, uint32_t cell, f3 p, uint32_t* n_tested = nullptr) {
	typedef uint32_t u2n __attribute__((ext_vector_type(2)));
	const u2n head = *reinterpret_cast<const NRS_GLOBAL u2n*>(gp(e.fine_head) + cell);
	const uint32_t n = head.y >> kFineHeadTetBits;
	return scan_entries_for_tet(e, gp(e.fine_idx), head.x, head.x + n, head.y & ((1u << kFineHeadTetBits) - 1u), p, n_tested);
}
template <bool SHORT = true>
__device__ __forceinline__ uint32_t find_tet(const DeviceEdit& e, f3 u, const uint32_t* __restrict__ march_lds, uint32_t* n_tested = nullptr) {
	const int level = mip_from_pos(u);
	if (e.fine_off) {
		typedef int32_t i4n __attribute__((ext_vector_type(4)));
		i4n lo, ext;
		const int level_u = __builtin_amdgcn_readfirstlane(level);
		if (SHORT && __all(level == level_u)) {
			const NRS_CONSTANT i4n* win = (const NRS_CONSTANT i4n*)reinterpret_cast<const i4n*>(&e.fine_win[0][0]) + 2 * level_u;
			lo = win[0]; ext = win[1];
		} else {
			const NRS_GLOBAL i4n* win = gp(reinterpret_cast<const i4n*>(&e.fine_win[0][0])) + 2 * level;
			lo = win[0]; ext = win[1];
		}
		const float mip_scale = ldexpf(1.0f, -level);
		f3 q = u - mk3(0.5f, 0.5f, 0.5f);
		q = q * mip_scale;
		q = q + mk3(0.5f, 0.5f, 0.5f);
		if (ext.w != kFinePlain) {
			const int fres_i = (int)(kGrid << ext.w);
			const float fres = (float)fres_i;
			const int hi = fres_i - 1;
			const int fx = clampi_((int)(q.x * fres), 0, hi) - lo.x, fy = clampi_((int)(q.y * fres), 0, hi) - lo.y, fz = clampi_((int)(q.z * fres), 0, hi) - lo.z;
			if ((uint32_t)fx >= (uint32_t)ext.x || (uint32_t)fy >= (uint32_t)ext.y || (uint32_t)fz >= (uint32_t)ext.z) return 0xffffffffu;
			const uint32_t cell = (uint32_t)lo.w + ((uint32_t)fz * (uint32_t)ext.y + (uint32_t)fy) * (uint32_t)ext.x + (uint32_t)fx;
			if (SHORT && e.fine_head) return scan_fine_cell_for_tet(e, cell, u, n_tested);
			return scan_list_for_tet(e, e.fine_off, e.fine_idx, cell, u, n_tested);
		}
	}
	const uint32_t cell = march_lds ? occupancy_bit_index(u, (uint32_t)level, march_lds) : (uint32_t)level * kGridVol + cascaded_grid_idx_at(u, (uint32_t)level);
	return scan_cell_for_tet(e, cell, u, n_tested);
}

constexpr uint32_t kTetNotSearched = 0xfffffffeu;
template <bool RECORD = true, bool SHORT = true>
__device__ __forceinline__ bool tet_warp(const DeviceEdit& e, bool with_dir, f3& wpos, f3& wdir, const uint32_t* __restrict__ march_lds = nullptr, uint32_t* scan_out = nullptr,
                                         uint32_t* n_tested = nullptr) {
	bool in_deformed = false;
	if (scan_out) *scan_out = kTetNotSearched;
	if (box_contains(e.warped_bbox, wpos)) {
		const f3 u = unwarp_position(wpos, e.aabb);
		if (n_tested) *n_tested |= 0x10000u;
		const uint32_t found = find_tet<SHORT>(e, u, march_lds, n_tested);
		if (n_tested && found != 0xffffffffu) *n_tested |= 0x20000u;
		if (scan_out) *scan_out = found;
		__builtin_amdgcn_sched_barrier(0);
		if (found != 0xffffffffu) {
			if constexpr (!RECORD) {
				typedef uint32_t u4n __attribute__((ext_vector_type(4)));
				const u4n tv = gp(reinterpret_cast<const u4n*>(e.tets))[found];
				float bc[4];
				{
					const f3 a = ld3(e.verts, tv.x), b = ld3(e.verts, tv.y), c = ld3(e.verts, tv.z), d = ld3(e.verts, tv.w);
					bary_tet(a, b, c, d, u, bc);
				}
				__builtin_amdgcn_sched_barrier(0);
				f3 canon = bc[0] * ld3(e.orig, tv.x) + bc[1] * ld3(e.orig, tv.y);
				canon = canon + bc[2] * ld3(e.orig, tv.z);
				canon = canon + bc[3] * ld3(e.orig, tv.w);
				wpos = e.diag_pow2 ? mk3((canon.x - e.aabb.mn[0]) * e.inv_diag[0], (canon.y - e.aabb.mn[1]) * e.inv_diag[1], (canon.z - e.aabb.mn[2]) * e.inv_diag[2])
				                   : warp_position(canon, e.aabb);
				__builtin_amdgcn_sched_barrier(0);
				if (with_dir && e.rot) {
					const f3 ud = unwarp_direction(wdir);
					const f3 c0 = ld3(e.rot, 3u * found), c1 = ld3(e.rot, 3u * found + 1u), c2 = ld3(e.rot, 3u * found + 2u);
					const float R[9] = {c0.x, c0.y, c0.z, c1.x, c1.y, c1.z, c2.x, c2.y, c2.z};
					const f3 rd = mat3_mul(R, ud);
					wdir = warp_direction(rd);
				}
			} else {
				typedef float f4n __attribute__((ext_vector_type(4)));
				const NRS_GLOBAL f4n* pq = gp(reinterpret_cast<const f4n*>(e.planes)) + 8 * (size_t)found;
				const NRS_GLOBAL f4n* mq = gp(reinterpret_cast<const f4n*>(e.mapback)) + 6 * (size_t)found;
				const bool rotate = with_dir && e.rot;
				const f4n v0 = pq[0], v1 = pq[1], v2 = pq[2];
				const f4n o0 = mq[0], o1 = mq[1], o2 = mq[2];
				float bc[4];
				bary_tet(mk3(v0.x, v0.y, v0.z), mk3(v0.w, v1.x, v1.y), mk3(v1.z, v1.w, v2.x), mk3(v2.y, v2.z, v2.w), u, bc);
				__builtin_amdgcn_sched_barrier(0);
				f4n r0 = {0.f, 0.f, 0.f, 0.f}, r1 = {0.f, 0.f, 0.f, 0.f};
				float r2 = 0.f;
				if (rotate) { r0 = mq[3]; r1 = mq[4]; r2 = reinterpret_cast<const NRS_GLOBAL float*>(mq)[20]; }
				f3 canon = bc[0] * mk3(o0.x, o0.y, o0.z) + bc[1] * mk3(o0.w, o1.x, o1.y);
				canon = canon + bc[2] * mk3(o1.z, o1.w, o2.x);
				canon = canon + bc[3] * mk3(o2.y, o2.z, o2.w);
				wpos = e.diag_pow2 ? mk3((canon.x - e.aabb.mn[0]) * e.inv_diag[0], (canon.y - e.aabb.mn[1]) * e.inv_diag[1], (canon.z - e.aabb.mn[2]) * e.inv_diag[2])
				                   : warp_position(canon, e.aabb);
// ... 283 lines not shown
```

### nerfshop_amd/csrc/nrs_internal.h

```cpp
#pragma once
#include <stdint.h>
#include <stddef.h>
#include "../../include/nrs.h"
#include "nrs_route.h"

#include <stdlib.h>
#include <hip/hip_vector_types.h>

namespace nrs {

inline const char* dev_knob(const char* name) {
	static const bool on = []() { const char* e = getenv("NRS_DEV_KNOBS"); return e && e[0] && e[0] != '0'; }();
	return on ? getenv(name) : nullptr;
}

constexpr uint32_t kGrid = 128;
constexpr uint32_t kCascades = 5;
constexpr uint32_t kGridVol = kGrid * kGrid * kGrid;
constexpr uint32_t kLevels = 16;
constexpr uint32_t kCoarse = 32;
constexpr uint32_t kCoarseWords = kCoarse * kCoarse * kCoarse / 32;
static_assert((kCoarse & (kCoarse - 1)) == 0, "the block walk's bounds test (cx | cy | cz) needs a power of two");
constexpr uint32_t kDensityW = 64 * 32 + 16 * 64;
constexpr uint32_t kRgbW = 64 * 32 + 64 * 64 + 16 * 64;
constexpr uint32_t kCanonW = kDensityW + kRgbW + 64 * 64 + 64 * 16;

struct LevelParams {
	float    scale;
	uint32_t resolution;
	uint32_t res2;
	uint32_t offset;
	uint32_t count;
	uint32_t hashed;
	uint32_t mask;
	uint32_t cached;
	uint32_t rec_first;
	uint32_t rec_res;
	uint32_t rec_res2;
	uint32_t tab_first;
};

constexpr uint32_t kNumFrags = 26;
constexpr uint32_t kNumFragsDevice = 56;
constexpr uint32_t kFragBytes = 64 * 8 * 2;
constexpr uint32_t kWfragBytes = kNumFrags * kFragBytes;
constexpr uint32_t kWfragDeviceBytes = kNumFragsDevice * kFragBytes;
constexpr uint16_t kFragOne = 0xffffu, kFragMinusOne = 0xfffeu, kFragNegate = 0x8000u;

struct Box3 { float mn[3]; float mx[3]; };

inline uint32_t tile_pitch(uint32_t width, uint32_t tile_size) { return ((width + tile_size - 1u) / tile_size) | 1u; }

struct OccAccel {
	Box3 box;
	float cell[3], inv_cell[3];
	const uint32_t* mask;
};

struct DeviceModel {
	const uint32_t* grid;
	const uint16_t* wfrag;
	const uint8_t*  bitfield;
	const void*     records;
	const void*     records2;
	const uint32_t* bricks;
	LevelParams     levels[kLevels];
	Box3            aabb;
	float           inv_diag[3];
	uint32_t        diag_pow2;
	OccAccel        occ;
	uint32_t        rgb_activation;
	uint32_t        density_activation;
	uint32_t        numerics;
	uint32_t        rgb_deep;
	uint32_t        no_dir;
	uint32_t        n_extra_dims;
	float           light01[3];
};

struct AffineBox { float mn[3]; float u[3]; float v[3]; float w[3]; float uu, vv, ww; float center[3]; };
enum EditKind : uint32_t { kEditCage = 0, kEditAffine = 1 };

struct DeviceEdit {
	uint32_t kind;
	uint32_t a_hide_original, a_correct_dir, a_pad;
	AffineBox a_dst, a_sel;
	float a_translation[3], a_scale[3], a_rot[9];
	Box3 aabb;
	float inv_diag[3];
	uint32_t diag_pow2;
	Box3 bbox;
	Box3 warped_bbox;
	Box3 orig_warped_bbox;
	const uint32_t* lut_off;
	const uint32_t* lut_idx;
	const uint32_t* tets;
	const float*    verts;
	const float*    orig;
	const float*    rot;
	const uint32_t* fine_off;
	const uint32_t* fine_idx;
	int32_t         fine_win[kCascades][8];
	const float*    planes;
	const uint2*    fine_head;
	const float*    mapback;
	const uint8_t*  orig_bitfield;
	const float*    shs;
	const float*    out_density;
	const float*    res_density;
	float           residual_amplitude;
	uint32_t        copy;
	uint32_t        apply_poisson;
	uint32_t        pad;
};

struct RenderCounters {
	unsigned long long n_samples;
	uint32_t next_packet;
	uint32_t n_rays_alive;
	uint32_t n_rays_hit;
	uint32_t blocks_done;
	unsigned long long phase_cycles[8];
	unsigned long long walk[13];
};

struct RenderArgs {
	nrs_render_params p;
	const DeviceEdit* edits;
	int32_t  n_edits;
	uint32_t any_poisson;
	uint32_t any_affine;
	uint32_t extra;
	uint32_t gate;
	uint32_t n_packets;
	uint32_t tiles_x;
	uint32_t packets_per_tile_x;
	uint32_t pixels_owned;
	unsigned long long* feedback;
	uint32_t tail_every;
	uint32_t reteam;
	uint32_t tail_target;
	uint32_t all_tail;
	uint32_t steal;
	uint32_t fill_lanes;
	uint32_t p_big;
	uint32_t team;
	uint32_t spp_count;
	uint32_t spp_packets;
	uint32_t spp_big;
	uint32_t slab_stride;
	uint32_t max_steps;
	uint32_t dbg;
	float*    frame;
	float*    depth;
	uint32_t* steps;
	RenderCounters* counters;
	RenderCounters* counters_next;
	unsigned long long* wave_log;
	const nrs_sample_view* views;
};

int launch_render(RouteId row, const DeviceModel& m, const RenderArgs& a, int n_cus, void* stream);
int launch_views_upload(const nrs_sample_view* h_views, uint32_t n, nrs_sample_view* d_views, void* stream);
unsigned long long launch_render_dispatches();
int launch_slice(const DeviceModel& m, const RenderArgs& a, int n_cus, void* stream);
int launch_trace_samples(const DeviceModel& m, const nrs_render_params& p, uint32_t n_pixels, const uint32_t* d_pixel_idx,
                         uint32_t max_samples, float* d_t, float* d_dt, uint32_t* d_count, void* stream);
int launch_network(const DeviceModel& m, int mode, uint32_t n, const float* d_in, uint32_t ld_in, void* d_out, uint32_t ld_out,
                   int layout, int n_cus, void* stream, bool per_sample_light = false);
int launch_network_backward(const DeviceModel& m, uint32_t n, const float* d_in, uint32_t ld_in, const void* d_dout, uint32_t ld_dout, int layout,
                            float* d_dparams, float* d_dinput, int n_cus, void* stream);
int launch_selection_rays(const DeviceModel& m, const nrs_render_params& p, const int32_t* d_pixels, uint32_t n, float threshold,
                          float* d_positions, uint32_t* d_cells, uint8_t* d_found, void* stream);
int launch_poisson_fit(const DeviceModel& m, uint32_t n_verts, uint32_t n_sh, const float* d_coords, const void* d_net, int is_inside, float scale,
                       float* d_density, float* d_sh, void* stream);
int launch_cell_records(const DeviceModel& m, uint32_t n_levels, void* d_records, void* stream);
int launch_weight_fragments(const uint16_t* d_params, const uint16_t* d_src, uint16_t* d_frag, uint32_t n, void* stream);
constexpr uint32_t kBrick = 8, kBrickCells = kBrick * kBrick * kBrick;
#ifndef NRS_BRICK_MORTON
#define NRS_BRICK_MORTON 0
#endif
#if defined(__HIPCC__)
__host__ __device__
#endif
inline uint32_t brick_slot(uint32_t x, uint32_t y, uint32_t z) {
#if NRS_BRICK_MORTON
	auto spread = [](uint32_t v) { return (v & 1u) | ((v & 2u) << 2) | ((v & 4u) << 4); };
	return spread(x) | (spread(y) << 1) | (spread(z) << 2);
#else
	return (z << 6) | (y << 3) | x;
#endif
}
int launch_brick_mark(const DeviceModel& m, const LevelParams& lp, const uint8_t* d_mask, uint32_t* d_table, uint32_t* d_counter, uint32_t* d_slots, uint32_t capacity, void* stream);
int launch_brick_fill(const DeviceModel& m, const LevelParams& lp, const uint32_t* d_slots, uint32_t n_bricks, void* d_records2, void* stream);
int launch_grid_eval(const DeviceModel& m, int mode, const uint32_t res[3], const float box_mn[3], const float box_mx[3], const float dir01[3],
                     const float* d_density_grid, float* d_out, int n_cus, void* stream);
int launch_map_rays(const DeviceEdit& e, uint32_t n, float* d_coords, uint32_t ld, int with_dir, uint8_t* d_empty, void* stream);
int launch_grid_to_bitfield(const float* d_grid, uint8_t* d_bitfield, float* d_scratch_mean, void* stream);
int launch_occ_accel(const uint8_t* d_bitfield, uint32_t* d_masks, float* d_out, uint32_t* d_keys, void* stream);
int launch_grid_update(const DeviceModel& m, const DeviceEdit* d_edits, int n_edits, const nrs_grid_update& u, uint64_t rng_state_nonuniform,
                       float* d_grid, uint32_t* d_grid_tmp, int n_cus, void* stream);
int launch_accumulate(uint32_t n_pixels, const float* d_frame, float* d_accum, uint32_t sample_count, int color_space, void* stream);
int launch_accumulate_spp(uint32_t n_pixels, const float* d_frames, size_t slab_stride_pixels, uint32_t spp_count, float* d_accum, uint32_t sample_count, int color_space, void* stream);
int launch_tonemap(uint32_t n_pixels, const float* d_accum, const nrs_tonemap_params& p, void* d_out, void* stream);
int launch_accumulate_spp_tonemap(uint32_t n_pixels, const float* d_frames, size_t slab_stride_pixels, uint32_t spp_count, float* d_accum, uint32_t sample_count,
                                  const nrs_tonemap_params& p, void* d_out, void* stream);
int launch_detile(const nrs_render_params& p, uint32_t n_ranks, size_t rank_stride_floats, const float* d_tiles, uint32_t channels,
                  float* d_image, void* stream);
const char* launch_last_error();

constexpr uint32_t kLutScanTiles = kGridVol * kCascades / 4096;
constexpr uint32_t kFineMaxCells = 16u << 20;
constexpr uint32_t kFineScanTiles = kFineMaxCells / 4096;
constexpr int32_t kFinePlain = 0xff;
constexpr int32_t kFineMaxList = 96;
constexpr uint32_t kFineHeadTetBits = 25;
static_assert(kFineMaxList < (1 << (32 - kFineHeadTetBits)), "a fine list (a filtered LUT list of at most kFineMaxList tets) must fit the head word's length field");
int launch_mvc_apply(uint32_t n_points, uint32_t n_cv, const float* d_weights, const float* d_cage, float* d_points, void* stream);
int launch_bbox(uint32_t n, const float* d_verts, float* d_out6, void* stream);
int launch_poisson_interpolate(uint32_t n_points, uint32_t n_cv, const float* d_gamma, const float* d_per_cage, float* d_shs, float* d_out_density, float* d_res_density, void* stream);
int launch_lut_count_scan(uint32_t n_tets, const float* d_verts, const uint32_t* d_tets, uint32_t* d_counts, uint32_t* d_tile_sums,
                          uint32_t* d_offsets, uint32_t* d_total, unsigned long long* d_hit_masks ,
                          float cells0 , void* stream);
int launch_lut_fill(uint32_t n_tets, const float* d_verts, const uint32_t* d_tets, uint32_t* d_counts, const uint32_t* d_offsets, uint32_t* d_idx,
                    uint8_t* d_bitfield, uint32_t* d_scratch_u32 , uint32_t* d_big_cells, uint32_t n_work , unsigned long long* d_hit_masks , float cells0, void* stream);
uint32_t lut_big_list_capacity(size_t idx_capacity);
int launch_tet_planes(uint32_t n_tets, const float* d_verts, const uint32_t* d_tets, float* d_planes, void* stream);
int launch_fine_window(const uint32_t* d_lut_off, int32_t* d_window_out, void* stream);
int launch_fine_count_scan(const DeviceEdit& de, uint32_t n_fine_cells, uint32_t* d_counts, uint32_t* d_tile_sums, uint32_t* d_fine_off, uint32_t* d_total, void* stream);
int launch_fine_fill(const DeviceEdit& de, uint32_t n_fine_cells, const uint32_t* d_fine_off, uint32_t* d_fine_idx, uint2* d_fine_head , void* stream);
int launch_local_rotations(uint32_t n_tets, const float* d_verts, const float* d_orig, const uint32_t* d_tets, float* d_out, float* d_mapback, void* stream);
int launch_tet_mapback(uint32_t n_tets, const float* d_orig, const uint32_t* d_tets, const float* d_rot, float* d_mapback, void* stream);

constexpr uint32_t kMcBlock = 256;
constexpr uint32_t kMcRowCap = 32;
struct McGrid {
	uint32_t res[3];
	uint32_t n;
	float scale[3], offset[3];
	float thresh;
};
int launch_mc_count(const McGrid& g, const float* d_density, const uint8_t* d_n_tris , uint32_t* d_code, uint32_t* d_block_sums, void* stream);
int launch_mc_scan(uint32_t n_blocks, uint32_t* d_block_sums, uint32_t* d_totals, void* stream);
int launch_mc_emit(const McGrid& g, const float* d_density, const int8_t* d_table, uint32_t row_len, const uint32_t* d_code, const uint32_t* d_block_offs,
                   float* d_verts, uint32_t* d_vert_src, uint32_t* d_indices, void* stream);
int launch_mc_1ring(const McGrid& g, const float* d_density, const int8_t* d_table, uint32_t row_len, const uint32_t* d_code, const uint32_t* d_block_offs, uint32_t n_verts,
                    const uint32_t* d_vert_src, const float* d_verts, const uint32_t* d_indices, float* d_smoothed, float* d_normals, void* stream);
int launch_mesh_color_inputs(uint32_t n, const float* d_verts, const Box3& aabb, float* d_coords7, void* stream);
int launch_mesh_colors(uint32_t n, const void* d_net_fp16, uint32_t rgb_activation, int linear_colors, float* d_colors, void* stream);

constexpr uint32_t kMorphLevelWords = kGridVol / 32;
constexpr int32_t kMorphMaxRadius = 10;
constexpr uint32_t kMorphMaxTaps = (2 * kMorphMaxRadius + 1) * (2 * kMorphMaxRadius + 1);
struct MorphPlan {
	uint32_t n_taps, invert;
	int8_t dy[kMorphMaxTaps], dz[kMorphMaxTaps], half[kMorphMaxTaps];
};
int launch_morph_pack(const uint32_t* d_morton_level, uint32_t* d_rows, void* stream);
int launch_morph_unpack(const uint32_t* d_rows, uint32_t* d_morton_level, void* stream);
int launch_morph_rows(const MorphPlan& plan, const uint32_t* d_rows_in, uint32_t* d_rows_out, void* stream);
int launch_selection_lattice(const uint32_t* d_rows, float* d_lattice, void* stream);

struct RouteProbe {
	int32_t  status;
	int32_t  row;
	uint32_t team, all_tail, fill_lanes, tail_every, tail_target, hybrid;
	uint32_t row_has_batch;
	char     name[96];
	char     message[256];
};

void set_last_error(const char* msg);

}

extern "C" int nrs_route_probe(const nrs::RouteRequest* requests, uint32_t request_size, uint32_t n, nrs::RouteProbe* out, uint32_t probe_size);
extern "C" int nrs_route_probe_views(const nrs::RouteRequest* requests, uint32_t request_size, uint32_t n, uint32_t* views_out);
```

### nerfshop_amd/csrc/nrs_occupancy.hip

```cpp
#include <hip/hip_runtime.h>
#include "nrs_internal.h"
#include "nrs_launch.h"
#include "nrs_device.cuh"
#include "nrs_mlp.cuh"

namespace nrs {

constexpr uint32_t kMeanBlocks = 256;
__global__ __launch_bounds__(256) void grid_mean_partial_kernel(const float* __restrict__ grid, double* __restrict__ partial) {
	__shared__ double part[256];
	double acc = 0.0;
	const uint32_t per = kGridVol / kMeanBlocks;
	const float* g = grid + (size_t)blockIdx.x * per;
	for (uint32_t i = threadIdx.x; i < per; i += 256) acc += (double)(fmaxf(g[i], 0.f) / (float)kGridVol);
	part[threadIdx.x] = acc;
	__syncthreads();
	for (int s = 128; s > 0; s >>= 1) {
		if ((int)threadIdx.x < s) part[threadIdx.x] += part[threadIdx.x + s];
		__syncthreads();
	}
	if (threadIdx.x == 0) partial[blockIdx.x] = part[0];
}
__global__ __launch_bounds__(256) void grid_mean_final_kernel(const double* __restrict__ partial, float* __restrict__ mean_out) {
	__shared__ double part[256];
	part[threadIdx.x] = partial[threadIdx.x];
	__syncthreads();
	for (int s = 128; s > 0; s >>= 1) {
		if ((int)threadIdx.x < s) part[threadIdx.x] += part[threadIdx.x + s];
		__syncthreads();
	}
	if (threadIdx.x == 0) mean_out[0] = (float)part[0];
}
__global__ void grid_to_bitfield_kernel(uint32_t n_elements, const float* __restrict__ grid, uint8_t* __restrict__ bitfield, const float* __restrict__ mean) {
	const uint32_t i = blockIdx.x * blockDim.x + threadIdx.x;
	if (i >= n_elements) return;
	const float thresh = fminf(0.01f, *mean);
	uint8_t bits = 0;
	#pragma unroll
	for (uint32_t j = 0; j < 8; ++j) bits |= grid[(size_t)i * 8 + j] > thresh ? (uint8_t)(1u << j) : 0;
	bitfield[i] = bits;
}
__global__ void bitfield_max_pool_kernel(uint32_t n_elements, const uint8_t* __restrict__ prev_level, uint8_t* __restrict__ next_level) {
	const uint32_t i = blockIdx.x * blockDim.x + threadIdx.x;
	if (i >= n_elements) return;
	uint8_t bits = 0;
	#pragma unroll
	for (uint32_t j = 0; j < 8; ++j) bits |= prev_level[i * 8 + j] > 0 ? (uint8_t)(1u << j) : 0;
	const uint32_t x = morton3D_invert(i >> 0) + kGrid / 8, y = morton3D_invert(i >> 1) + kGrid / 8, z = morton3D_invert(i >> 2) + kGrid / 8;
	next_level[morton3D(x, y, z)] |= bits;
}

int launch_grid_to_bitfield(const float* d_grid, uint8_t* d_bitfield, float* d_scratch_mean, void* stream) {
	hipStream_t s = (hipStream_t)stream;
	double* partial = reinterpret_cast<double*>(d_scratch_mean + 2);
	hipLaunchKernelGGL(grid_mean_partial_kernel, dim3(kMeanBlocks), dim3(256), 0, s, d_grid, partial);
	hipLaunchKernelGGL(grid_mean_final_kernel, dim3(1), dim3(256), 0, s, partial, d_scratch_mean);
	const uint32_t n = kGridVol / 8 * kCascades;
	hipLaunchKernelGGL(grid_to_bitfield_kernel, dim3((n + 255) / 256), dim3(256), 0, s, n, d_grid, d_bitfield, d_scratch_mean);
	for (uint32_t level = 1; level < kCascades; ++level) {
		const uint32_t ne = kGridVol / 64;
		hipLaunchKernelGGL(bitfield_max_pool_kernel, dim3((ne + 255) / 256), dim3(256), 0, s, ne, d_bitfield + (size_t)(level - 1) * kGridVol / 8,
		                   d_bitfield + (size_t)level * kGridVol / 8);
	}
	NRS_LAUNCH_CHECK("grid_to_bitfield launch");
	return NRS_OK;
}

struct OccAccelOut { float mn[3], mx[3], cell[3], inv_cell[3]; };
__device__ __forceinline__ uint32_t float_key(float f) { const uint32_t u = __float_as_uint(f); return u ^ ((u >> 31) ? 0xffffffffu : 0x80000000u); }
__device__ __forceinline__ float key_float(uint32_t k) { return __uint_as_float(k ^ ((k >> 31) ? 0x80000000u : 0xffffffffu)); }
__device__ __forceinline__ bool accel_block_relevant(uint32_t level, const uint32_t c[3], float s, float margin) {
	if (level == 0) return true;
	float far = 0.f;
	for (int k = 0; k < 3; ++k) {
		const float a = ((float)c[k] / (float)kGrid - 0.5f) * s - margin, b = ((float)(c[k] + 2u) / (float)kGrid - 0.5f) * s + margin;
		far = fmaxf(far, fmaxf(fabsf(a), fabsf(b)));
	}
	return far >= ldexpf(1.0f, (int)level - 2);
}
__global__ void __launch_bounds__(256) occ_accel_bounds_kernel(const uint64_t* __restrict__ bitfield, uint32_t* __restrict__ keys) {
	const uint32_t i = blockIdx.x * 256 + threadIdx.x;
	const uint64_t w = bitfield[i];
	const float inf = __builtin_huge_valf();
	float mn[2][3] = {{inf, inf, inf}, {inf, inf, inf}}, mx[2][3] = {{-inf, -inf, -inf}, {-inf, -inf, -inf}};
	if (w) {
		const uint32_t level = i / (kGridVol / 64), byte0 = (i % (kGridVol / 64)) * 8;
		const float s = ldexpf(1.0f, (int)level), margin = s / (float)kGrid / 16.f;
		for (uint32_t j = 0; j < 8; ++j) {
			if (!((w >> (8 * j)) & 0xffu)) continue;
			const uint32_t m = (byte0 + j) * 8;
			const uint32_t c[3] = {morton3D_invert(m), morton3D_invert(m >> 1), morton3D_invert(m >> 2)};
			const bool exact = accel_block_relevant(level, c, s, margin);
			for (int k = 0; k < 3; ++k) {
				const float lo = ((float)c[k] / (float)kGrid - 0.5f) * s + 0.5f - margin, hi = ((float)(c[k] + 2u) / (float)kGrid - 0.5f) * s + 0.5f + margin;
				mn[0][k] = fminf(mn[0][k], lo); mx[0][k] = fmaxf(mx[0][k], hi);
				if (exact) { mn[1][k] = fminf(mn[1][k], lo); mx[1][k] = fmaxf(mx[1][k], hi); }
			}
		}
	}
	if (!__ballot(w != 0)) return;
	for (int f = 0; f < 2; ++f)
		for (int k = 0; k < 3; ++k) {
			float a = mn[f][k], b = mx[f][k];
			for (int o = 32; o; o >>= 1) { a = fminf(a, __shfl_xor(a, o)); b = fmaxf(b, __shfl_xor(b, o)); }
			if ((threadIdx.x & 63) == 0) {
				if (a < inf) atomicMin(&keys[f * 6 + k], float_key(a));
				if (b > -inf) atomicMax(&keys[f * 6 + 3 + k], float_key(b));
			}
		}
}
__global__ void occ_accel_box_kernel(const uint32_t* __restrict__ keys, OccAccelOut* __restrict__ out) {
	const uint32_t f = threadIdx.x;
	if (f >= 2) return;
	const float inf = __builtin_huge_valf();
	OccAccelOut o;
	const bool any = keys[f * 6] != 0xffffffffu;
	for (int k = 0; k < 3; ++k) {
		o.mn[k] = any ? key_float(keys[f * 6 + k]) : inf;
		o.mx[k] = any ? key_float(keys[f * 6 + 3 + k]) : -inf;
		o.cell[k] = any ? (o.mx[k] - o.mn[k]) / (float)kCoarse : 1.f;
		o.inv_cell[k] = any ? 1.0f / o.cell[k] : 1.f;
	}
	out[f] = o;
}
constexpr uint32_t kAccelMaskBlocks = 160, kAccelWordsPerThread = kCascades * (kGridVol / 64) / (kAccelMaskBlocks * 256);
static_assert(kAccelMaskBlocks * 256 * kAccelWordsPerThread == kCascades * (kGridVol / 64), "the mask pass covers the bitfield exactly");
__global__ void __launch_bounds__(256) occ_accel_mask_kernel(const uint64_t* __restrict__ bitfield, const OccAccelOut* __restrict__ acc, uint32_t* __restrict__ masks) {
	__shared__ uint32_t lmask[2 * kCoarseWords];
	for (uint32_t j = threadIdx.x; j < 2 * kCoarseWords; j += 256) lmask[j] = 0u;
	__syncthreads();
	const OccAccelOut a0 = acc[0], a1 = acc[1];
	for (uint32_t r = 0; r < kAccelWordsPerThread; ++r) {
		const uint32_t i = (blockIdx.x * kAccelWordsPerThread + r) * 256 + threadIdx.x;
		const uint64_t w = bitfield[i];
		if (!w) continue;
		const uint32_t level = i / (kGridVol / 64), byte0 = (i % (kGridVol / 64)) * 8;
		const float s = ldexpf(1.0f, (int)level), margin = s / (float)kGrid / 16.f;
		for (uint32_t j = 0; j < 8; ++j) {
			if (!((w >> (8 * j)) & 0xffu)) continue;
			const uint32_t m = (byte0 + j) * 8;
			const uint32_t c[3] = {morton3D_invert(m), morton3D_invert(m >> 1), morton3D_invert(m >> 2)};
			const bool exact = accel_block_relevant(level, c, s, margin);
			for (int f = 0; f < (exact ? 2 : 1); ++f) {
				const OccAccelOut& a = f ? a1 : a0;
				int lo[3], hi[3];
				for (int k = 0; k < 3; ++k) {
					const float wmin = ((float)c[k] / (float)kGrid - 0.5f) * s + 0.5f - margin, wmax = ((float)(c[k] + 2u) / (float)kGrid - 0.5f) * s + 0.5f + margin;
					lo[k] = min((int)kCoarse - 1, max(0, (int)floorf((wmin - a.mn[k]) * a.inv_cell[k])));
					hi[k] = min((int)kCoarse - 1, max(0, (int)floorf((wmax - a.mn[k]) * a.inv_cell[k])));
				}
				uint32_t* mask = lmask + f * kCoarseWords;
				static_assert(kCoarse == 32, "one mask word = one row of blocks along x");
				const uint32_t row = (0xffffffffu >> (31 - hi[0])) & (0xffffffffu << lo[0]);
				for (int z = lo[2]; z <= hi[2]; ++z)
					for (int y = lo[1]; y <= hi[1]; ++y) {
						const uint32_t word = (uint32_t)z * kCoarse + (uint32_t)y;
						if ((mask[word] & row) != row) atomicOr(&mask[word], row);
					}
			}
		}
	}
	__syncthreads();
	for (uint32_t j = threadIdx.x; j < 2 * kCoarseWords; j += 256)
		if (lmask[j]) atomicOr(&masks[j], lmask[j]);
}
int launch_occ_accel(const uint8_t* d_bitfield, uint32_t* d_masks, float* d_out, uint32_t* d_keys, void* stream) {
	hipStream_t s = (hipStream_t)stream;
	static const uint32_t init_keys[12] = {0xffffffffu, 0xffffffffu, 0xffffffffu, 0u, 0u, 0u, 0xffffffffu, 0xffffffffu, 0xffffffffu, 0u, 0u, 0u};
	hipError_t e = hipMemcpyAsync(d_keys, init_keys, sizeof(init_keys), hipMemcpyHostToDevice, s);
	if (e == hipSuccess) e = hipMemsetAsync(d_masks, 0, 2 * kCoarseWords * 4, s);
	if (e != hipSuccess) return hip_fail(e, "occ_accel: clear");
	const uint32_t n_words = kCascades * (kGridVol / 64);
	static_assert(kCascades * (kGridVol / 64) % 256 == 0, "one thread per bitfield word, no tail");
	hipLaunchKernelGGL(occ_accel_bounds_kernel, dim3(n_words / 256), dim3(256), 0, s, (const uint64_t*)d_bitfield, d_keys);
	hipLaunchKernelGGL(occ_accel_box_kernel, dim3(1), dim3(64), 0, s, d_keys, (OccAccelOut*)d_out);
	hipLaunchKernelGGL(occ_accel_mask_kernel, dim3(kAccelMaskBlocks), dim3(256), 0, s, (const uint64_t*)d_bitfield, (const OccAccelOut*)d_out, d_masks);
	NRS_LAUNCH_CHECK("occ_accel launch");
	return NRS_OK;
}

struct GridUpdateArgs {
	const float* grid;
	uint32_t* grid_tmp;
	const DeviceEdit* edits;
	int32_t n_edits;
	uint32_t n_uniform, n_nonuniform, step, n_cascades;
	uint64_t rng_state, rng_inc, rng_state_nonuniform;
	uint32_t cell_order;
};

constexpr uint32_t kSampleMul = 56924617u, kSampleAdd = 96925573u;
__host__ __device__ constexpr uint32_t inverse_mod_2_32(uint32_t k) {
	uint32_t x = k;
	for (int i = 0; i < 5; ++i) x *= 2u - k * x;
	return x;
}
constexpr uint32_t kSampleMulInv = inverse_mod_2_32(kSampleMul) & (kGridVol - 1u);
static_assert(((kSampleMul * kSampleMulInv) & (kGridVol - 1u)) == 1u, "inverse of the sample multiplier mod 2^21");

template <int NUM>
__global__ __launch_bounds__(256) void grid_refresh_kernel(const DeviceModel m, const GridUpdateArgs a) {
	const uint32_t nm = NUM == kNumRuntime ? (uint32_t)__builtin_amdgcn_readfirstlane((int)m.numerics) : (uint32_t)NUM;
	__shared__ NetSmem sm;
	__shared__ uint64_t wrap_mult[65], wrap_plus[65];
	if (threadIdx.x < 65) Pcg32::skip_coefficients(a.rng_inc, 0ull - ((uint64_t)threadIdx.x << 23), wrap_mult[threadIdx.x], wrap_plus[threadIdx.x]);
	stage_model_to_lds(m, sm.ml);
	const int lane = threadIdx.x & 63;
	const int g = lane >> 5;
	FeatLds& fl = sm.fl[__builtin_amdgcn_readfirstlane(threadIdx.x >> 6)];
	const GridView gv = make_grid_view(m);
	const uint32_t wave_global = blockIdx.x * (blockDim.x >> 6) + (uint32_t)__builtin_amdgcn_readfirstlane(threadIdx.x >> 6);
	const uint32_t n_waves = gridDim.x * (blockDim.x >> 6);
	uint64_t lane_mult, lane_plus, mlane_mult, mlane_plus;
	Pcg32::skip_coefficients(a.rng_inc, (uint64_t)(4 * lane), lane_mult, lane_plus);
	Pcg32::skip_coefficients(a.rng_inc, 4ull * (uint64_t)lane * (uint64_t)kSampleMulInv, mlane_mult, mlane_plus);
	const bool morton = a.cell_order && (a.n_uniform & (kGridVol - 1u)) == 0u;
	const uint32_t n = a.n_uniform + a.n_nonuniform;
	const uint32_t n_tiles = (n + 63) / 64;
	for (uint32_t tile = wave_global; tile < n_tiles; tile += n_waves) {
		const uint32_t s = tile * 64 + lane;
		const bool have = s < n;
		f3 wpos = mk3(0, 0, 0);
		uint32_t cell = 0;
		if (have) {
			const uint32_t t0 = tile * 64, t1 = t0 + 63;
			const bool uni = s < a.n_uniform;
			uint32_t i = uni ? s : s - a.n_uniform;
			Pcg32 rng{uni ? a.rng_state : a.rng_state_nonuniform, a.rng_inc};
			if (morton && t1 < a.n_uniform) {
				const uint32_t k = t0 >> 21, c0 = t0 & (kGridVol - 1u);
				const uint32_t i_first = ((c0 - kSampleAdd) * kSampleMulInv) & (kGridVol - 1u);
				const uint32_t sum = i_first + (uint32_t)lane * kSampleMulInv;
				const uint32_t w = sum >> 21;
				i = (sum & (kGridVol - 1u)) + (k << 21);
				uint64_t mt, pt;
				Pcg32::skip_coefficients(a.rng_inc, 4ull * (uint64_t)i_first + ((uint64_t)k << 23), mt, pt);
				const uint64_t st = mlane_mult * (mt * rng.state + pt) + mlane_plus;
				rng.state = wrap_mult[w] * st + wrap_plus[w];
			} else if ((t0 < a.n_uniform) == (t1 < a.n_uniform)) {
				const uint32_t i0 = (t0 < a.n_uniform) ? t0 : t0 - a.n_uniform;
				uint64_t mt, pt;
				Pcg32::skip_coefficients(a.rng_inc, (uint64_t)(i0 * 4u), mt, pt);
				rng.state = lane_mult * (mt * rng.state + pt) + lane_plus;
			} else {
				rng.advance((uint64_t)(i * 4u));
			}
			cell = generate_grid_sample(rng, i, uni ? a.n_uniform : a.n_nonuniform, a.step, m.aabb, a.grid, a.n_cascades, uni ? -0.01f : 0.01f, wpos);
			f3 unused = mk3(0.5f, 0.5f, 0.5f);
			for (int k = a.n_edits - 1; k >= 0; --k) (void)edit_warp(a.edits[k], false, wpos, unused);
		}
		encode_num<NUM, true, true, NRS_REFRESH_GATE_PHASES>(nm, gv, m.levels, sm.ml, fl, lane, g, wpos, have);
		_Float16 raw_b0 = (_Float16)0, raw_b1 = (_Float16)0;
		#pragma unroll 1
		for (int b = 0; b < 2; ++b) {
			const int sel = (b != g) ? 1 : 0;
			const half8 x0 = load_features(fl, lane, sel, 0), x1 = load_features(fl, lane, sel, 1);
			const half8 dout = density_mlp_num<NUM>(nm, sm.ml.w, lane, x0, x1);
			if (b == 0) raw_b0 = dout[0]; else raw_b1 = dout[0];
		}
		const float from_partner = xchg32((float)raw_b1);
		_Float16 raw = g ? (_Float16)from_partner : raw_b0;
		if (!have) continue;
		_Float16 act = (_Float16)network_to_density((float)raw, m.density_activation);
		for (int k = a.n_edits - 1; k >= 0; --k) {
			const DeviceEdit& e = a.edits[k];
			float r;
			if (e.apply_poisson && poisson_residual_density(e, wpos, r)) act = act + (_Float16)r;
		}
		const float thickness = (float)act * NRS_MIN_STEP;
		atomicMax(a.grid_tmp + cell, __float_as_uint(thickness));
	}
}

__global__ void grid_ema_kernel(uint32_t n_elements, float decay, float* __restrict__ grid, const uint32_t* __restrict__ grid_tmp) {
	const uint32_t i = blockIdx.x * blockDim.x + threadIdx.x;
	if (i >= n_elements) return;
	const float importance = __uint_as_float(grid_tmp[i]);
	const float prev = grid[i];
	grid[i] = (prev < 0.f) ? prev : fmaxf(prev * decay, importance);
}

int launch_grid_update(const DeviceModel& m, const DeviceEdit* d_edits, int n_edits, const nrs_grid_update& u, uint64_t rng_state_nonuniform,
                       float* d_grid, uint32_t* d_grid_tmp, int n_cus, void* stream) {
	hipStream_t s = (hipStream_t)stream;
	const uint32_t n_elements = kGridVol * kCascades;
	GridUpdateArgs a{};
	a.grid = d_grid;
	a.grid_tmp = d_grid_tmp;
	a.edits = d_edits;
	a.n_edits = n_edits;
	a.n_uniform = u.n_uniform_samples;
	a.n_nonuniform = u.n_nonuniform_samples;
	a.step = u.ema_step;
	a.n_cascades = u.max_cascade + 1;
	a.rng_state = u.rng_state;
	a.rng_inc = u.rng_inc;
	a.rng_state_nonuniform = rng_state_nonuniform;
	static const uint32_t cell_order = []() { const char* e = dev_knob("NRS_REFRESH_ORDER"); return e ? (uint32_t)atoi(e) : 1u; }();
	a.cell_order = cell_order;
	const uint32_t n = a.n_uniform + a.n_nonuniform;
	if (n > 0) {
		const uint32_t n_tiles = (n + 63) / 64;
		uint32_t grid = (n_tiles + 3) / 4;
		const uint32_t cap = (uint32_t)n_cus * 8;
		if (grid > cap) grid = cap;
		if (m.numerics) hipLaunchKernelGGL(grid_refresh_kernel<kNumRuntime>, dim3(grid), dim3(256), 0, s, m, a);
		else hipLaunchKernelGGL(grid_refresh_kernel<0>, dim3(grid), dim3(256), 0, s, m, a);
		NRS_LAUNCH_CHECK("grid_refresh_kernel launch");
	}
	hipLaunchKernelGGL(grid_ema_kernel, dim3((n_elements + 255) / 256), dim3(256), 0, s, n_elements, u.decay, d_grid, d_grid_tmp);
	NRS_LAUNCH_CHECK("grid_ema_kernel launch");
	return NRS_OK;
}

}
```

### nerfshop_amd/csrc/nrs_render.cuh

```cuda
#pragma once
#include <hip/hip_runtime.h>
#include "nrs_internal.h"
#include "nrs_device.cuh"
#include "nrs_mlp.cuh"

namespace nrs {

__device__ __forceinline__ uint32_t lds_peek(const uint32_t* p) { return __atomic_load_n(p, __ATOMIC_RELAXED); }
__device__ __forceinline__ void lds_poke(uint32_t* p, uint32_t v) { __atomic_store_n(p, v, __ATOMIC_RELAXED); }
constexpr int kRing = 128;
constexpr int kTeamMax = 4;
#ifndef NRS_MEASURE
#define NRS_MEASURE 0
#endif
constexpr uint32_t kRefillWhenIdle = 64;

template <int WAVES>
struct RenderSmem {
	ModelLds ml;
	FeatLds fl[WAVES];
	uint2 ring[WAVES][kRing];
	uint32_t coarse[kMarchLdsWords];
	unsigned long long queue;
	unsigned long long sum_samples;
// ... 184 lines not shown
			};
			if (ring_count != 0u) {
				if (__any(have)) {
					const uint32_t target = claim_waiting_wave();
					if (target != 0xffffffffu) {
						const uint32_t n = min(ring_count, 64u);
						if ((uint32_t)ln < n) sm.ring[target][ln] = ring[(ring_head + (uint32_t)ln) & (kRing - 1)];
						ring_head += n;
						ring_count -= n;
						__builtin_amdgcn_fence(__ATOMIC_RELEASE, "workgroup");
						__builtin_amdgcn_wave_barrier();
						if (ln == 0) { lds_poke(&sm.mail[target], n | 0x80000000u); atomicAdd(&a1.counters->walk[7], (unsigned long long)n | (1ull << 32)); }
					}
				}
			} else if (ring_count == 0u) {
				const unsigned long long lead_mask = __ballot(have && tk == 0);
				const uint32_t live = (uint32_t)__popcll(lead_mask);
				const uint32_t target = live > kGiveMin ? claim_waiting_wave() : 0xffffffffu;
				if (target != 0xffffffffu) {
					const uint32_t keep = (live + 1u) / 2u, give = live - keep;
					const bool team_live = ((lead_mask >> team_base) & 1ull) != 0ull;
					const uint32_t lead_rank = (uint32_t)__popcll(lead_mask & ((1ull << team_base) - 1ull));
					const bool moved = team_live && lead_rank >= keep;
					uint32_t* mb = &sm.fl[target].feat[0][0][0];
					if (moved && tk == 0) {
						const uint32_t r = lead_rank - keep;
						mb[0 * 32 + r] = __float_as_uint(o.x); mb[1 * 32 + r] = __float_as_uint(o.y); mb[2 * 32 + r] = __float_as_uint(o.z);
						mb[3 * 32 + r] = __float_as_uint(d.x); mb[4 * 32 + r] = __float_as_uint(d.y); mb[5 * 32 + r] = __float_as_uint(d.z);
						mb[6 * 32 + r] = __float_as_uint(t);
						mb[7 * 32 + r] = __float_as_uint(cr); mb[8 * 32 + r] = __float_as_uint(cg); mb[9 * 32 + r] = __float_as_uint(cb); mb[10 * 32 + r] = __float_as_uint(ca);
						mb[11 * 32 + r] = __float_as_uint(ray_depth); mb[12 * 32 + r] = __float_as_uint(max_weight);
						mb[13 * 32 + r] = out_idx; mb[14 * 32 + r] = n_steps;
					}
					if (moved) have = false;
					__builtin_amdgcn_fence(__ATOMIC_RELEASE, "workgroup");
					__builtin_amdgcn_wave_barrier();
					if (ln == 0) { lds_poke(&sm.mail[target], give); atomicAdd(&a1.counters->walk[7], (unsigned long long)give | (1ull << 32)); }
				}
			}
		}
		if (TEAM == 0 && a1.reteam && (((a1.reteam & 2u) && tail_seen) || (!more && ring_count == 0u))) {
			const unsigned long long lead_mask = __ballot(have && tk == 0);
			const uint32_t live = (uint32_t)__popcll(lead_mask);
			const uint32_t new_t = live <= 16u ? 4u : (live <= 32u ? 2u : 1u);
			if (live != 0u && new_t > gen_t) {
				if (have && tk == 0) {
					const uint32_t rank = __builtin_amdgcn_mbcnt_hi((uint32_t)(lead_mask >> 32), __builtin_amdgcn_mbcnt_lo((uint32_t)lead_mask, 0u));
					fl.feat[0][0][rank] = (uint32_t)lane;
				}
				__builtin_amdgcn_wave_barrier();
				const uint32_t r = (uint32_t)lane / new_t;
				const int src = r < live ? (int)fl.feat[0][0][r] : lane;
				__builtin_amdgcn_wave_barrier();
				o.x = __shfl(o.x, src, 64); o.y = __shfl(o.y, src, 64); o.z = __shfl(o.z, src, 64);
				d.x = __shfl(d.x, src, 64); d.y = __shfl(d.y, src, 64); d.z = __shfl(d.z, src, 64);
				t = __shfl(t, src, 64);
				cr = __shfl(cr, src, 64); cg = __shfl(cg, src, 64); cb = __shfl(cb, src, 64); ca = __shfl(ca, src, 64);
				ray_depth = __shfl(ray_depth, src, 64); max_weight = __shfl(max_weight, src, 64);
				out_idx = (uint32_t)__shfl((int)out_idx, src, 64); n_steps = (uint32_t)__shfl((int)n_steps, src, 64);
				have = r < live;
				valid = true;
				gen_t = new_t;
				tk = lane & (int)(gen_t - 1u);
				team_base = lane & ~(int)(gen_t - 1u);
				if (have) {
					for (int j = 0; j < tk && valid; ++j) {
						t += calc_dt(t, p1.cone_angle_constant);
						f3 npos; float ndt;
						valid = march_to_occupied(p1, m1, sm.coarse, o, d, t, npos, ndt, nullptr);
					}
				}
			}
		}
		const unsigned long long free_mask = __ballot(!have);
		const uint32_t nfree = (uint32_t)__popcll(free_mask);

		while (more && ring_count < (TEAM > 1 ? 64u / gen_t : (TEAM == 0 && tail_seen ? a1.tail_target : nfree)) && nfree >= kRefillWhenIdle) {
			uint32_t pk = claim_packet(&sm.queue, &a1.counters->next_packet, a1.n_packets, lane);
			if (pk == kNoPacket) { more = false; if (PROF) { pf_tq = wall_clock64() - pf_wall0; pf_rounds_q = pf_rounds; } break; }
			if (PROF) ++pf_packets;
			uint32_t bs = 0u;
			bool b_small = false;
			float fo_x = off_x, fo_y = off_y;
			if (BATCH && a1.spp_count > 1u) {
				uint32_t per = a1.spp_packets;
				if (TEAM == 0 && !a1.all_tail && a1.p_big) {
					b_small = pk >= a1.p_big;
					per = b_small ? a1.spp_packets - a1.spp_big : a1.spp_big;
					pk = b_small ? pk - a1.p_big : pk;
				}
				bs = pk / per;
				pk -= bs * per;
			}
			const uint32_t spp = p1.spp_index + bs;
			if (BATCH) {
				ld_random_pixel_offset(p1.snap_to_pixel_centers ? 0u : spp, fo_x, fo_y);
				fo_x = __uint_as_float((uint32_t)__builtin_amdgcn_readfirstlane((int)__float_as_uint(fo_x)));
				fo_y = __uint_as_float((uint32_t)__builtin_amdgcn_readfirstlane((int)__float_as_uint(fo_y)));
			}
			uint32_t x, y, oi;
			bool alive = false;
			float t0 = 0.f;
			bool small = TEAM > 1, inside;
			if (TEAM == 0 && a1.all_tail) {
				small = true;
				tail_seen = true;
				inside = a1.fill_lanes == 4u ? packet_pixel<4>(a1, pk, lane, x, y, oi) : (a1.fill_lanes == 2u ? packet_pixel<2>(a1, pk, lane, x, y, oi) : packet_pixel<1>(a1, pk, lane, x, y, oi));
			} else if (TEAM == 0 && a1.p_big) {
				small = BATCH && a1.spp_count > 1u ? b_small : pk >= a1.p_big;
				tail_seen = tail_seen || small;
				inside = small ? packet_pixel_tail(a1, BATCH && a1.spp_count > 1u ? pk : pk - a1.p_big, lane, x, y, oi) : packet_pixel_bulk(a1, pk, lane, x, y, oi);
			} else {
				inside = packet_pixel<(TEAM ? TEAM : 1)>(a1, pk, lane, x, y, oi);
			}
			const bool first_of_team = TEAM == 0 ? (!small || (lane & (int)(a1.fill_lanes - 1u)) == 0) : tk == 0;
			if (BATCH) oi += bs * a1.slab_stride;
			if (inside) {
				Ray r = BATCH ? init_ray<EXTRA, true>(p1, x, y, fo_x, fo_y, spp, (VIEWS && a1.views) ? a1.views + bs : nullptr) : init_ray<EXTRA>(p1, x, y, off_x, off_y);
				if (first_of_team) {
					a1.depth[oi] = 1e10f;
					if (a1.steps) a1.steps[oi] = 0;
				}
				alive = r.alive;
				if (EXTRA) {
					if (p1.d_envmap) reinterpret_cast<float4*>(a1.frame)[oi] = read_envmap(p1.d_envmap, p1.envmap_resolution, r.d);
					if (alive && p1.render_mode == NRS_RENDER_DISTORTION) {
						float d0 = 0.f, d1 = 0.f;
						if (p1.d_distortion_map) {
							read_image2(p1.d_distortion_map, p1.distortion_resolution, ((float)x + 0.5f) / (float)p1.resolution[0], ((float)y + 0.5f) / (float)p1.resolution[1], d0, d1);
							d0 = d0 * 50.0f + 0.5f; d1 = d1 * 50.0f + 0.5f;
						} else {
							d0 = 0.5f; d1 = 0.5f;
						}
						reinterpret_cast<float4*>(a1.frame)[oi] = make_float4(d0, d1, 0.5f, 1.0f);
						a1.depth[oi] = 1.0f;
						alive = false;
					}
				}
				uint32_t it_fill = 0;
#if NRS_MEASURE == 1
				if (alive) { Ray r2 = r; const bool a2 = first_hit(p1, m1, sm.coarse, x + (uint32_t)p1.resolution[0] * y, r2, nullptr); asm volatile("" :: "v"(r2.t), "s"((int)__ballot(a2))); }
#endif
				if (alive) alive = BATCH ? first_hit<true>(p1, m1, sm.coarse, x + (uint32_t)p1.resolution[0] * y, r, PROF ? &it_fill : nullptr, spp)
				                         : first_hit(p1, m1, sm.coarse, x + (uint32_t)p1.resolution[0] * y, r, PROF ? &it_fill : nullptr);
				if (PROF) {
					uint32_t mx = it_fill;
					for (int sh = 32; sh > 0; sh >>= 1) mx = max(mx, (uint32_t)__shfl_xor((int)mx, sh, 64));
					pf_walk[0] += it_fill; pf_walk[1] += (lane == 0) ? mx : 0u;
				}
				t0 = r.t;
			}
			if (TEAM != 1) alive = alive && first_of_team;
			const unsigned long long am = __ballot(alive);
			if (alive) {
				const uint32_t slot = ring_head + ring_count + __builtin_amdgcn_mbcnt_hi((uint32_t)(am >> 32), __builtin_amdgcn_mbcnt_lo((uint32_t)am, 0u));
				ring[slot & (kRing - 1)] = make_uint2(BATCH ? x | (y << kBatchXYBits) | (bs << (2u * kBatchXYBits)) : x | (y << 16), __float_as_uint(t0));
				++st_alive;
			}
			ring_count += (uint32_t)__popcll(am);
		}
		__builtin_amdgcn_wave_barrier();
		NRS_PHASE(1);

		if (nfree >= kRefillWhenIdle && ring_count) {
			if (TEAM == 0) {
				gen_t = tail_seen ? (ring_count > 32u && (!a1.all_tail || (a1.fill_lanes == 1u && ring_count >= kFullGen)) ? 1u : (ring_count > 16u ? 2u : 4u)) : 1u;
				tk = lane & (int)(gen_t - 1u);
				team_base = lane & ~(int)(gen_t - 1u);
			}
			const uint32_t take = min(TEAM != 1 ? 64u / gen_t : nfree, ring_count);
			const uint32_t rank = TEAM != 1 ? (uint32_t)lane / gen_t
			                                : __builtin_amdgcn_mbcnt_hi((uint32_t)(free_mask >> 32), __builtin_amdgcn_mbcnt_lo((uint32_t)free_mask, 0u));
			if (!have && rank < take) {
				const uint2 e = ring[(ring_head + rank) & (kRing - 1)];
				const uint32_t x = BATCH ? e.x & kBatchXYMask : e.x & 0xffffu, y = BATCH ? (e.x >> kBatchXYBits) & kBatchXYMask : e.x >> 16;
				if (BATCH) {
					const uint32_t es = e.x >> (2u * kBatchXYBits), espp = p1.spp_index + es;
					float eo_x, eo_y;
					ld_random_pixel_offset(p1.snap_to_pixel_centers ? 0u : espp, eo_x, eo_y);
					ray_origin_dir<EXTRA, true>(p1, x, y, eo_x, eo_y, o, d, espp, (VIEWS && a1.views) ? a1.views + es : nullptr);
					out_idx = pixel_out_idx(a1, x, y) + es * a1.slab_stride;
				} else {
				ray_origin_dir<EXTRA>(p1, x, y, off_x, off_y, o, d);
				out_idx = pixel_out_idx(a1, x, y);
				}
				t = __uint_as_float(e.y);
				cr = cg = cb = ca = 0.f;
				ray_depth = 0.f; max_weight = 0.f; n_steps = 0;
				have = true;
				if (TEAM != 1) {
					valid = true;
					for (int j = 0; j < tk && valid; ++j) {
						t += calc_dt(t, p1.cone_angle_constant);
						f3 npos; float ndt;
						valid = march_to_occupied(p1, m1, sm.coarse, o, d, t, npos, ndt, nullptr);
					}
				}
			}
			ring_head += take;
			ring_count -= take;
		}
		__builtin_amdgcn_wave_barrier();

		if (!__any(have)) {
			if (!more && ring_count == 0) {
				if (!(TEAM == 0 && a1.steal)) break;
				uint32_t got = 0u;
				int ln = lane;
				asm volatile("" : "+v"(ln));
				if (ln == 0) {
					const uint32_t bit = 1u << wave;
					atomicOr(&sm.idle_mask, bit);
					atomicSub(&sm.n_busy, 1u);
					bool promised = false;
					for (;;) {
						got = lds_peek(&sm.mail[wave]);
						if (got) break;
						if (!promised && lds_peek(&sm.n_busy) == 0u) {
							if (atomicAnd(&sm.idle_mask, ~bit) & bit) break;
							promised = true;
						}
						__builtin_amdgcn_s_sleep(8);
					}
				}
				got = (uint32_t)__builtin_amdgcn_readfirstlane((int)got);
				if (!got) break;
				__builtin_amdgcn_fence(__ATOMIC_ACQUIRE, "workgroup");
				if (got & 0x80000000u) {
					ring_head = 0u;
					ring_count = got & 0x7fffffffu;
					tail_seen = true;
					__builtin_amdgcn_wave_barrier();
					if (ln == 0) lds_poke(&sm.mail[wave], 0u);
					continue;
				}
				const uint32_t* mb = &sm.fl[wave].feat[0][0][0];
				gen_t = got <= 16u ? 4u : 2u;
				tk = ln & (int)(gen_t - 1u);
				team_base = ln & ~(int)(gen_t - 1u);
				const uint32_t r = (uint32_t)ln / gen_t;
				have = r < got;
				valid = true;
				if (have) {
					o = mk3(__uint_as_float(mb[0 * 32 + r]), __uint_as_float(mb[1 * 32 + r]), __uint_as_float(mb[2 * 32 + r]));
					d = mk3(__uint_as_float(mb[3 * 32 + r]), __uint_as_float(mb[4 * 32 + r]), __uint_as_float(mb[5 * 32 + r]));
					t = __uint_as_float(mb[6 * 32 + r]);
					cr = __uint_as_float(mb[7 * 32 + r]); cg = __uint_as_float(mb[8 * 32 + r]); cb = __uint_as_float(mb[9 * 32 + r]); ca = __uint_as_float(mb[10 * 32 + r]);
					ray_depth = __uint_as_float(mb[11 * 32 + r]); max_weight = __uint_as_float(mb[12 * 32 + r]);
					out_idx = mb[13 * 32 + r]; n_steps = mb[14 * 32 + r];
					for (int j = 0; j < tk && valid; ++j) {
						t += calc_dt(t, p1.cone_angle_constant);
						f3 npos; float ndt;
						valid = march_to_occupied(p1, m1, sm.coarse, o, d, t, npos, ndt, nullptr);
					}
				}
				__builtin_amdgcn_wave_barrier();
				if (ln == 0) lds_poke(&sm.mail[wave], 0u);
			}
			continue;
		}

		NRS_FRESH_ARGS(m2, a2);
		const nrs_render_params& p2 = a2.p;
		const GridView gv = make_grid_view(m2);
		NRS_PHASE(2);
		if (PROF) ++pf_rounds;
		const f3 pos = o + d * t;
		const float dt = calc_dt(t, p2.cone_angle_constant);
		f3 wpos = m2.diag_pow2 ? mk3((pos.x - m2.aabb.mn[0]) * m2.inv_diag[0], (pos.y - m2.aabb.mn[1]) * m2.inv_diag[1], (pos.z - m2.aabb.mn[2]) * m2.inv_diag[2])
		                      : warp_position(pos, m2.aabb);
		f3 wdir = warp_direction(d);
		float wdt = p2.cone_angle_constant == 0.f ? 0.f : warp_dt(dt);
		bool empty = false;
		uint32_t warp_scan = kTetNotSearched;
		const bool act = TEAM != 1 ? (have && valid) : have;
		uint32_t pf_scan = 0;
		if (ops && act) {
#if NRS_MEASURE == 2
			{ f3 wp2 = wpos, wd2 = wdir; asm volatile("" : "+v"(wp2.x), "+v"(wp2.y), "+v"(wp2.z)); bool e2 = false;
			  for (int ei = a2.n_edits - 1; ei >= 0; --ei) e2 |= AFFINE ? edit_warp<!POISSON>(a2.edits[ei], true, wp2, wd2) : tet_warp<!POISSON && GATE == 0, GATE == 0>(a2.edits[ei], true, wp2, wd2);
			  asm volatile("" :: "v"(wp2.x), "v"(wp2.y), "v"(wp2.z), "v"(wd2.x), "v"(wd2.y), "v"(wd2.z), "s"((int)__ballot(e2))); }
#endif
			for (int ei = a2.n_edits - 1; ei >= 0; --ei) {
				if (AFFINE) {
					empty |= edit_warp<!POISSON>(a2.edits[ei], true, wpos, wdir);
				} else if (POISSON) {
					uint32_t scan;
					empty |= tet_warp<false>(a2.edits[ei], true, wpos, wdir, sm.coarse, &scan);
					if (ei == a2.n_edits - 1) warp_scan = scan;
				} else {
					empty |= tet_warp<GATE == 0, GATE == 0>(a2.edits[ei], true, wpos, wdir, sm.coarse, nullptr, PROF ? &pf_scan : nullptr);
				}
			}
		}
		if (PROF && !POISSON && !AFFINE) {
			uint32_t mx = pf_scan & 0xffffu;
			for (int sh = 32; sh > 0; sh >>= 1) mx = max(mx, (uint32_t)__shfl_xor((int)mx, sh, 64));
			pf_walk[8] += (pf_scan >> 16) & 1u; pf_walk[9] += (lane == 0 && __any((pf_scan >> 16) & 1u)) ? 1u : 0u;
			pf_walk[10] += pf_scan & 0xffffu; pf_walk[11] += (lane == 0) ? mx : 0u; pf_walk[12] += (pf_scan >> 17) & 1u;
		}
		if (POISSON && !AFFINE) poisson_stash[wave * 64 + lane] = warp_scan;
		NRS_PHASE(3);
#if NRS_MEASURE == 3
		{ f3 wp2 = wpos; asm volatile("" : "+v"(wp2.x), "+v"(wp2.y), "+v"(wp2.z));
		  encode_num<NUM, kQuads>(nm, gv, m2.levels, sm.ml, fl, lane, g, wp2, act); }
#endif
// ... 456 lines not shown
```

### nerfshop_amd/runtime.py

```python
import ctypes as C
import os

import numpy as np
import torch

from . import _abi
from ._abi import NrsError, RenderParams, RenderStats, check


def _stream_handle(stream):
    if stream is None:
        stream = torch.cuda.current_stream()
    if isinstance(stream, torch.cuda.Stream):
        return C.c_void_p(stream.cuda_stream)
    return C.c_void_p(int(stream))


def _require_cuda(t, dtype, name):
    if not isinstance(t, torch.Tensor) or not t.is_cuda:
        raise NrsError(f"{name} must be a CUDA (HIP) tensor")
    if t.dtype != dtype:
        raise NrsError(f"{name} must have dtype {dtype}, got {t.dtype}")
    if not t.is_contiguous():
        raise NrsError(f"{name} must be contiguous")


class Context:
    def __init__(self, device=0):
        self.lib = _abi.load()
        self.h = C.c_void_p()
        check(self.lib.nrs_ctx_create(int(device), C.byref(self.h)))
        self.device = int(device)
        name = C.create_string_buffer(256)
        ncu, hbm = C.c_int(), C.c_size_t()
        check(self.lib.nrs_ctx_device_info(self.h, name, 256, C.byref(ncu), C.byref(hbm)))
        self.device_name, self.n_cus, self.hbm_bytes = name.value.decode(), ncu.value, hbm.value

    def set_lane_teams(self, lanes_per_ray):
        check(self.lib.nrs_ctx_set_lane_teams(self.h, int(lanes_per_ray)))

    def set_ray_handover(self, enabled):
        check(self.lib.nrs_ctx_set_ray_handover(self.h, int(bool(enabled))))

    def ray_handovers(self):
        n, k = C.c_uint64(), C.c_uint64()
        check(self.lib.nrs_ctx_ray_handovers(self.h, C.byref(n), C.byref(k)))
        return n.value, k.value

    def render_launches(self):
        n, sched = C.c_uint64(), C.c_uint32()
        check(self.lib.nrs_ctx_render_launches(self.h, C.byref(n), C.byref(sched)))
        return n.value, sched.value

    def close(self):
        if self.h:
            self.lib.nrs_ctx_destroy(self.h)
            self.h = C.c_void_p()

    def __del__(self):
        try:
            self.close()
        except Exception:
            pass


DEFAULT_CELL_CACHE_BYTES = 10 << 30


class NerfNetwork:

    def __init__(self, ctx, desc, cell_cache_bytes=DEFAULT_CELL_CACHE_BYTES, n_extra_dims=0):
        self.ctx, self.lib, self.desc = ctx, ctx.lib, desc
        self.h = C.c_void_p()
        self._n_extra_dims = int(n_extra_dims)
        if self._n_extra_dims:
            check(self.lib.nrs_model_create_ex(ctx.h, C.byref(desc), self._n_extra_dims, C.byref(self.h)))
        else:
            check(self.lib.nrs_model_create(ctx.h, C.byref(desc), C.byref(self.h)))
        if cell_cache_bytes and "NRS_CELL_CACHE_GB" not in os.environ:
            free_b = torch.cuda.mem_get_info(ctx.device)[0]
            try:
                self.set_cell_cache(min(int(cell_cache_bytes), free_b // 4))
            except NrsError:
                self.set_cell_cache(0)

    def padded_output_width(self):
        return 16

    def input_width(self):
        return 7

    def n_extra_dims(self):
        return int(self.lib.nrs_model_n_extra_dims(self.h))

    def n_params(self):
        return int(self.lib.nrs_model_n_params_ex(C.byref(self.desc), self._n_extra_dims))

    def set_light_dir(self, light_dir):
        check(self.lib.nrs_model_set_light_dir(self.h, C.byref((C.c_float * 3)(*[float(v) for v in light_dir]))))

    def set_params(self, params_fp16):
        p = np.ascontiguousarray(params_fp16)
        if p.dtype == np.float16:
            p = p.view(np.uint16)
        if p.dtype != np.uint16:
            raise NrsError("set_params expects fp16 parameters (numpy float16 or their uint16 bits)")
        check(self.lib.nrs_model_set_params(self.h, p.ctypes.data, p.size))

    def set_params_device(self, params_fp16_cuda, stream=None):
        t = params_fp16_cuda
        if not t.is_cuda or t.element_size() != 2 or not t.is_contiguous():
            raise NrsError("set_params_device expects a contiguous 2-byte CUDA tensor")
        check(self.lib.nrs_model_set_params_device(self.h, t.data_ptr(), t.numel(), _stream_handle(stream)))

    def set_numerics(self, grid_acc=0, mlp_acc=0):
        check(self.lib.nrs_model_set_numerics(self.h, int(grid_acc), int(mlp_acc)))

    def set_cell_cache(self, max_bytes):
        check(self.lib.nrs_model_set_cell_cache(self.h, int(max_bytes)))

    def cell_cache(self):
        n = C.c_uint32()
        b = self.lib.nrs_model_cell_cache_bytes(self.h, C.byref(n))
        return int(b), int(n.value)

    def set_sparse_cell_cache(self, mask_bitfield_u8, max_bytes):
        if mask_bitfield_u8 is None:
            check(self.lib.nrs_model_set_sparse_cell_cache(self.h, None, 0))
            return
        b = np.ascontiguousarray(mask_bitfield_u8, np.uint8)
        assert b.size == _abi.BITFIELD_BYTES
        check(self.lib.nrs_model_set_sparse_cell_cache(self.h, b.ctypes.data, int(max_bytes)))

    def sparse_cell_cache(self):
        f, n = C.c_uint32(), C.c_uint32()
        b = self.lib.nrs_model_sparse_cell_cache_bytes(self.h, C.byref(f), C.byref(n))
        return int(b), int(f.value), int(n.value)

    def set_density_bitfield(self, bitfield_u8):
        b = np.ascontiguousarray(bitfield_u8, np.uint8)
        check(self.lib.nrs_model_set_density_bitfield(self.h, b.ctypes.data, b.size))

    def set_density_grid(self, grid_f32):
        g = np.ascontiguousarray(grid_f32, np.float32)
        check(self.lib.nrs_model_set_density_grid(self.h, g.ctypes.data, g.size))

    def get_density_bitfield(self):
        out = np.zeros(_abi.BITFIELD_BYTES, np.uint8)
        check(self.lib.nrs_model_get_density_bitfield(self.h, out.ctypes.data, out.size))
        return out

    def get_march_accelerator(self, which):
        box = np.zeros(12, np.float32)
        mask = np.zeros(1024, np.uint32)
        check(self.lib.nrs_model_get_march_accelerator(self.h, int(which), box.ctypes.data, mask.ctypes.data))
        bits = np.unpackbits(mask.view(np.uint8), bitorder="little").reshape(32, 32, 32).astype(bool)
        return box, bits

    def get_density_grid(self):
        out = np.zeros(_abi.GRID_VOLUME * _abi.GRID_CASCADES, np.float32)
        check(self.lib.nrs_model_get_density_grid(self.h, out.ctypes.data, out.size))
        return out

    def inference_mixed_precision(self, stream, input, output):
        _require_cuda(input, torch.float32, "input")
        _require_cuda(output, torch.float16, "output")
        if input.dim() != 2 or input.shape[1] != 7:
            raise NrsError("NerfNetwork::inference_mixed_precision input must be [n, 7]")
        n = input.shape[0]
        layout, ld = self._out_layout(output, n)
        check(self.lib.nrs_network_inference(self.h, _stream_handle(stream), n, input.data_ptr(), output.data_ptr(), ld, layout))

    def inference_strided(self, stream, input, output):
        _require_cuda(input, torch.float32, "input")
        _require_cuda(output, torch.float16, "output")
        if input.dim() != 2 or input.shape[1] < 7 or not input.is_contiguous():
            raise NrsError("inference_strided input must be a contiguous [n, >= 7] tensor")
        n = input.shape[0]
        layout, ld = self._out_layout(output, n)
        check(self.lib.nrs_network_inference_strided(self.h, _stream_handle(stream), n, input.data_ptr(), input.shape[1], output.data_ptr(), ld, layout))

    def density(self, stream, input, output):
        _require_cuda(input, torch.float32, "input")
        _require_cuda(output, torch.float16, "output")
        if input.dim() != 2 or not (3 <= input.shape[1] <= 7):
            raise NrsError("NerfNetwork::density input must be in column major format ([n, 3..7] here).")
        n = input.shape[0]
        layout, ld = self._out_layout(output, n)
        check(self.lib.nrs_network_density(self.h, _stream_handle(stream), n, input.data_ptr(), input.shape[1], output.data_ptr(), ld, layout))

    def input_gradient(self, stream, input, output):
        _require_cuda(input, torch.float32, "input")
        _require_cuda(output, torch.float32, "output")
        n = input.shape[0]
        assert output.shape == (n, 3) and output.is_contiguous() and input.is_contiguous()
        check(self.lib.nrs_network_input_gradient(self.h, _stream_handle(stream), n, input.data_ptr(), input.shape[1], output.data_ptr()))

    def backward(self, stream, input, dL_doutput, dL_dparams, dL_dinput=None, accumulate=False):
        _require_cuda(input, torch.float32, "input")
        _require_cuda(dL_doutput, torch.float16, "dL_doutput")
        _require_cuda(dL_dparams, torch.float32, "dL_dparams")
        if input.dim() != 2 or input.shape[1] < 7 or not input.is_contiguous():
            raise NrsError("NerfNetwork::backward input must be a contiguous [n, >= 7] tensor")
        if dL_dparams.dim() != 1 or not dL_dparams.is_contiguous() or not dL_doutput.is_contiguous():
            raise NrsError("NerfNetwork::backward: dL_dparams must be a contiguous 1-d tensor and dL_doutput contiguous")
        n = input.shape[0]
        layout, ld = self._out_layout(dL_doutput, n)
        din = None
        if dL_dinput is not None:
            _require_cuda(dL_dinput, torch.float32, "dL_dinput")
            if tuple(dL_dinput.shape) != tuple(input.shape) or not dL_dinput.is_contiguous():
                raise NrsError("NerfNetwork::backward: dL_dinput must be contiguous and shaped like input")
            din = dL_dinput.data_ptr()
        check(self.lib.nrs_network_backward(self.h, _stream_handle(stream), n, input.data_ptr(), input.shape[1], dL_doutput.data_ptr(), ld, layout,
                                            dL_dparams.data_ptr(), dL_dparams.numel(), 1 if accumulate else 0, din))

    def ray_loss(self, stream, params, numsteps, coords, output, target_rgba, background=None, ray_origins=None, ray_counter=None, n_rays=None,
                 out=None, dl_planes=False):
        if not isinstance(params, _abi.RayLossParams):
            raise NrsError("ray_loss: params must be a RayLossParams")
        _require_cuda(numsteps, torch.int32, "numsteps")
        _require_cuda(coords, torch.float32, "coords")
        _require_cuda(output, torch.float16, "output")
        _require_cuda(target_rgba, torch.float32, "target_rgba")
        if numsteps.dim() != 2 or numsteps.shape[1] != 2:
            raise NrsError("ray_loss: numsteps must be [n_rays, 2]")
        n = int(numsteps.shape[0]) if n_rays is None else int(n_rays)
        if n > numsteps.shape[0] or tuple(target_rgba.shape) != (numsteps.shape[0], 4):
            raise NrsError("ray_loss: target_rgba must be [n_rays, 4] and n_rays no more than numsteps has rows")
        if coords.dim() != 2 or coords.shape[1] < 7:
            raise NrsError("ray_loss: coords must be a contiguous [n_samples, >= 7] tensor")
        n_samples, ld_in = int(coords.shape[0]), int(coords.shape[1])
        layout, ld_out = self._out_layout(output, n_samples)
        for t, name in ((background, "background"), (ray_origins, "ray_origins")):
            if t is not None:
                _require_cuda(t, torch.float32, name)
                if tuple(t.shape) != (numsteps.shape[0], 3):
                    raise NrsError(f"ray_loss: {name} must be [n_rays, 3]")
        if ray_counter is not None:
            _require_cuda(ray_counter, torch.int32, "ray_counter")
        cap = int(params.max_samples_compacted)
        if cap <= 0:
            raise NrsError("ray_loss: params.max_samples_compacted must be positive")
        dev = coords.device
        if out is None:
            out = (torch.empty_like(numsteps), torch.empty(cap, ld_in, dtype=torch.float32, device=dev),
                   torch.zeros((16, cap) if dl_planes else (cap, 16), dtype=torch.float16, device=dev),
                   torch.empty(numsteps.shape[0], dtype=torch.float32, device=dev), torch.empty(1, dtype=torch.int32, device=dev))
        numsteps_out, coords_out, dl, loss, counter = out
        _require_cuda(numsteps_out, torch.int32, "numsteps_out")
        _require_cuda(coords_out, torch.float32, "coords_out")
        _require_cuda(dl, torch.float16, "dL_doutput")
        _require_cuda(loss, torch.float32, "loss")
        _require_cuda(counter, torch.int32, "counter")
        if tuple(numsteps_out.shape) != tuple(numsteps.shape) or tuple(coords_out.shape) != (cap, ld_in) or loss.numel() < numsteps.shape[0] or counter.numel() < 1:
            raise NrsError("ray_loss: an output tensor has the wrong shape")
        dl_layout, ld_dl = self._out_layout(dl, cap)
        check(self.lib.nrs_ray_loss(self.h, _stream_handle(stream), C.byref(params), n, None if ray_counter is None else ray_counter.data_ptr(), numsteps.data_ptr(),
                                    n_samples, coords.data_ptr(), ld_in, output.data_ptr(), ld_out, layout, target_rgba.data_ptr(),
                                    None if background is None else background.data_ptr(), None if ray_origins is None else ray_origins.data_ptr(),
                                    numsteps_out.data_ptr(), coords_out.data_ptr(), dl.data_ptr(), ld_dl, dl_layout, loss.data_ptr(), counter.data_ptr()))
        return numsteps_out, coords_out, dl, loss, counter

    def training_samples(self, stream, rays, jitter, cone_angle_constant, max_samples, ld=7):
        _require_cuda(rays, torch.float32, "rays")
        if rays.dim() != 2 or rays.shape[1] != 6:
            raise NrsError("training_samples: rays must be [n, 6]")
        n = int(rays.shape[0])
        if jitter is not None:
            _require_cuda(jitter, torch.float32, "jitter")
            if jitter.numel() != n:
                raise NrsError("training_samples: jitter must be [n]")
        if int(max_samples) <= 0 or int(ld) < 7:
            raise NrsError("training_samples: max_samples must be positive and ld >= 7")
        dev = rays.device
        coords = torch.zeros(int(max_samples), int(ld), dtype=torch.float32, device=dev)
        numsteps = torch.zeros(n, 2, dtype=torch.int32, device=dev)
        ray_indices = torch.zeros(n, dtype=torch.int32, device=dev)
        counters = torch.zeros(2, dtype=torch.int32, device=dev)
        check(self.lib.nrs_training_samples(self.h, _stream_handle(stream), n, rays.data_ptr(), None if jitter is None else jitter.data_ptr(), float(cone_angle_constant),
                                            int(max_samples), coords.data_ptr(), int(ld), numsteps.data_ptr(), ray_indices.data_ptr(), counters.data_ptr()))
        return coords, numsteps, ray_indices, counters

    def visualize_activation(self, stream, layer, dimension, input, output):
        _require_cuda(input, torch.float32, "input")
        _require_cuda(output, torch.float32, "output")
        n = input.shape[0]
        assert input.shape[1] == 7 and output.shape == (n,) and output.is_contiguous() and input.is_contiguous()
        check(self.lib.nrs_network_visualize_activation(self.h, _stream_handle(stream), int(layer), int(dimension), n, input.data_ptr(), output.data_ptr()))

    def hashgrid_encode(self, stream, input, output):
        _require_cuda(input, torch.float32, "input")
        _require_cuda(output, torch.float16, "output")
        n = input.shape[0]
        if tuple(output.shape) != (n, 32):
            raise NrsError("hashgrid_encode output must be [n, 32]")
        check(self.lib.nrs_hashgrid_encode(self.h, _stream_handle(stream), n, input.data_ptr(), input.shape[1], output.data_ptr()))

    @staticmethod
    def _out_layout(output, n):
        if output.dim() == 2 and output.shape[0] == 16 and output.shape[1] >= n:
            return _abi.LAYOUT_PLANES, int(output.shape[1])
        if output.dim() == 2 and output.shape[1] == 16 and output.shape[0] >= n:
            return _abi.LAYOUT_INTERLEAVED, 16
        raise NrsError("output must be [16, n_el] (planes) or [n, 16] (interleaved) fp16")

    def close(self):
        if self.h:
            self.lib.nrs_model_destroy(self.h)
            self.h = C.c_void_p()
# ... 912 lines not shown
```

Before: 13230 Msamples/s.

## Add hierarchical occupancy pyramid to coarse empty-space skipping walk

Builds a four-level occupancy mip pyramid (32^3 down to 4^3) on top of the coarse march mask and changes the coarse DDA walk to skip whole empty blocks at the coarsest empty level, recomputing the cell from the ray position after each jump. This is meant to cut the number of coarse-cell iterations rays spend crossing large empty regions before the first hit. The cost is a larger LDS footprint per block, extra mask loads per step and a float re-derivation of the cell index that may have edge-case rounding issues. It also adds measurement-only variants behind NRS_MEASURE and a query API for the pyramid.

```diff
diff --git a/include/nrs.h b/include/nrs.h
--- a/include/nrs.h
+++ b/include/nrs.h
@@ -175,6 +175,7 @@
 int    nrs_model_set_density_grid(nrs_model* model, const float* h_grid, size_t n_floats);
 int    nrs_model_get_density_bitfield(nrs_model* model, uint8_t* h_bitfield_out, size_t n_bytes);
 int    nrs_model_get_march_accelerator(nrs_model* model, int which, float* h_box12, uint32_t* h_mask1024);
+int    nrs_model_get_look_pyramid(nrs_model* model, int which, uint32_t* h_pyramid146);
 int    nrs_model_get_density_grid(nrs_model* model, float* h_grid_out, size_t n_floats);
 int    nrs_model_update_density_grid(nrs_model* model, nrs_edit* const* edits, int n_edits, nrs_grid_update* u, void* stream);
 void   nrs_rng_seed(uint64_t seed, uint64_t* state_out, uint64_t* inc_out);
diff --git a/nerfshop_amd/_abi.py b/nerfshop_amd/_abi.py
--- a/nerfshop_amd/_abi.py
+++ b/nerfshop_amd/_abi.py
@@ -221,7 +221,7 @@
     "nrs_ctx_create", "nrs_ctx_destroy", "nrs_ctx_device_info", "nrs_ctx_set_lane_teams", "nrs_ctx_set_ray_handover", "nrs_ctx_ray_handovers",
     "nrs_model_create", "nrs_model_destroy", "nrs_model_n_params", "nrs_model_level_table",
     "nrs_model_set_params", "nrs_model_set_params_device", "nrs_model_set_numerics", "nrs_model_set_cell_cache", "nrs_model_cell_cache_bytes", "nrs_model_set_sparse_cell_cache", "nrs_model_sparse_cell_cache_bytes", "nrs_model_set_density_bitfield", "nrs_model_set_density_grid",
-    "nrs_model_get_density_bitfield", "nrs_model_get_march_accelerator", "nrs_model_get_density_grid", "nrs_model_update_density_grid", "nrs_rng_seed",
+    "nrs_model_get_density_bitfield", "nrs_model_get_march_accelerator", "nrs_model_get_look_pyramid", "nrs_model_get_density_grid", "nrs_model_update_density_grid", "nrs_rng_seed",
     "nrs_network_inference", "nrs_network_density", "nrs_hashgrid_encode", "nrs_density_on_grid", "nrs_rgba_on_grid", "nrs_network_input_gradient", "nrs_network_visualize_activation",
     "nrs_poisson_boundary", "nrs_poisson_sample_coords", "nrs_project_selection_pixels", "nrs_upper_cell_idx", "nrs_selection_cells",
     "nrs_edit_create", "nrs_edit_create_affine", "nrs_edit_destroy", "nrs_edit_map_rays", "nrs_edit_map_positions",
@@ -322,6 +322,8 @@
     lib.nrs_model_get_density_bitfield.argtypes = [P, P, C.c_size_t]
     lib.nrs_model_get_density_grid.argtypes = [P, P, C.c_size_t]
     lib.nrs_model_get_march_accelerator.argtypes = [P, I, P, P]
+    if hasattr(lib, "nrs_model_get_look_pyramid"):
+        lib.nrs_model_get_look_pyramid.argtypes = [P, I, P]
     lib.nrs_model_update_density_grid.argtypes = [P, C.POINTER(P), I, C.POINTER(GridUpdate), P]
     lib.nrs_rng_seed.argtypes = [C.c_uint64, C.POINTER(C.c_uint64), C.POINTER(C.c_uint64)]
     lib.nrs_rng_seed.restype = None
diff --git a/nerfshop_amd/csrc/nrs_api_model.cpp b/nerfshop_amd/csrc/nrs_api_model.cpp
--- a/nerfshop_amd/csrc/nrs_api_model.cpp
+++ b/nerfshop_amd/csrc/nrs_api_model.cpp
@@ -10,8 +10,9 @@
 
 static int refresh_accel(nrs_model* m, void* stream) {
 	hipStream_t s = (hipStream_t)stream;
-	float* d_out = reinterpret_cast<float*>(m->d_accel_masks.get() + 2 * kCoarseWords);
-	NRS_LAUNCH(launch_occ_accel(m->dm.bitfield, m->d_accel_masks.get(), d_out, m->d_accel_masks.get() + 2 * kCoarseWords + 24, stream));
+	static const bool flat_pyramid = dev_knob("NRS_NO_LOOK_PYRAMID") != nullptr;
+	float* d_out = reinterpret_cast<float*>(m->d_accel_masks.get() + 2 * kLookWords);
+	NRS_LAUNCH(launch_occ_accel(m->dm.bitfield, m->d_accel_masks.get(), d_out, m->d_accel_masks.get() + 2 * kLookWords + 24, flat_pyramid, stream));
 	float h[24];
 	HIP_TRY(hipMemcpyAsync(h, d_out, sizeof(h), hipMemcpyDeviceToHost, s));
 	HIP_TRY(hipStreamSynchronize(s));
@@ -24,7 +25,7 @@
 			acc[f]->inv_cell[k] = h[f * 12 + 9 + k];
 		}
 	m->accel_any.mask = m->d_accel_masks.get();
-	m->accel_exact.mask = m->d_accel_masks.get() + kCoarseWords;
+	m->accel_exact.mask = m->d_accel_masks.get() + kLookWords;
 	return NRS_OK;
 }
 DeviceModel nrs::model_for_launch(const nrs_model* m, const nrs_render_params& p) {
@@ -88,8 +89,8 @@
 	hipError_t he = m->d_grid.alloc(m->total_entries);
 	if (he == hipSuccess) he = m->d_wfrag.alloc(kWfragDeviceBytes / 2);
 	if (he == hipSuccess) he = m->d_bitfield.alloc(NRS_BITFIELD_BYTES);
-	if (he == hipSuccess) he = m->d_accel_masks.alloc(2 * kCoarseWords + 64);
-	if (he == hipSuccess) he = hipMemset(m->d_accel_masks.get(), 0, 2 * kCoarseWords * 4);
+	if (he == hipSuccess) he = m->d_accel_masks.alloc(2 * kLookWords + 64);
+	if (he == hipSuccess) he = hipMemset(m->d_accel_masks.get(), 0, 2 * kLookWords * 4);
 	if (he == hipSuccess) he = m->d_density_grid.alloc((size_t)kGridVol * kCascades);
 	if (he == hipSuccess) he = hipMemset(m->d_density_grid.get(), 0, (size_t)kGridVol * kCascades * 4);
 	if (he != hipSuccess) {
@@ -414,6 +415,14 @@
 	HIP_TRY(hipMemcpy(h_mask, a.mask, kCoarseWords * 4, hipMemcpyDeviceToHost));
 	return NRS_OK;
 }
+int nrs_model_get_look_pyramid(nrs_model* m, int which, uint32_t* h_pyramid) {
+	if (!m || !h_pyramid || which < 0 || which > 1) return fail(NRS_ERR_INVALID_ARG, "nrs_model_get_look_pyramid: bad argument");
+	if (!m->have_bitfield) return fail(NRS_ERR_STATE, "nrs_model_get_look_pyramid: occupancy not set (nrs_model_set_density_bitfield/_grid)");
+	HIP_TRY(hipSetDevice(m->ctx->device));
+	const OccAccel& a = which ? m->accel_exact : m->accel_any;
+	HIP_TRY(hipMemcpy(h_pyramid, a.mask + kCoarseWords, (kLookWords - kCoarseWords) * 4, hipMemcpyDeviceToHost));
+	return NRS_OK;
+}
 int nrs_model_get_density_bitfield(nrs_model* m, uint8_t* h_out, size_t n_bytes) {
 	if (!m || !h_out || n_bytes != NRS_BITFIELD_BYTES) return fail(NRS_ERR_INVALID_ARG, "nrs_model_get_density_bitfield: bad argument");
 	HIP_TRY(hipSetDevice(m->ctx->device));
diff --git a/nerfshop_amd/csrc/nrs_device.cuh b/nerfshop_amd/csrc/nrs_device.cuh
--- a/nerfshop_amd/csrc/nrs_device.cuh
+++ b/nerfshop_amd/csrc/nrs_device.cuh
@@ -369,6 +369,10 @@
 	return tnear <= tfar;
 }
 
+template <uint32_t LEVEL>
+__device__ __forceinline__ uint32_t look_bit(const uint32_t* __restrict__ mask, uint32_t idx) {
+	return (mask[look_level_word(LEVEL) + (idx >> 5)] >> (idx & 31u)) & 1u;
+}
 __device__ __forceinline__ float coarse_safe_until(const DeviceModel& m, const uint32_t* __restrict__ mask, f3 o, f3 d, f3 idir, float t) {
 	const Box3& b = m.occ.box;
 	const float ax = (b.mn[0] - o.x) * idir.x, bx = (b.mx[0] - o.x) * idir.x;
@@ -379,25 +383,37 @@
 	if (!(tnear <= tfar)) return -1.f;
 	const f3 p = o + d * tnear;
 	const float hi = (float)(kCoarse - 1);
-	int cx = (int)__builtin_amdgcn_fmed3f((p.x - b.mn[0]) * m.occ.inv_cell[0], 0.f, hi);
-	int cy = (int)__builtin_amdgcn_fmed3f((p.y - b.mn[1]) * m.occ.inv_cell[1], 0.f, hi);
-	int cz = (int)__builtin_amdgcn_fmed3f((p.z - b.mn[2]) * m.occ.inv_cell[2], 0.f, hi);
-	const int sx = d.x >= 0.f ? 1 : -1, sy = d.y >= 0.f ? 1 : -1, sz = d.z >= 0.f ? 1 : -1;
+	uint32_t cx = (uint32_t)__builtin_amdgcn_fmed3f((p.x - b.mn[0]) * m.occ.inv_cell[0], 0.f, hi);
+	uint32_t cy = (uint32_t)__builtin_amdgcn_fmed3f((p.y - b.mn[1]) * m.occ.inv_cell[1], 0.f, hi);
+	uint32_t cz = (uint32_t)__builtin_amdgcn_fmed3f((p.z - b.mn[2]) * m.occ.inv_cell[2], 0.f, hi);
+	const uint32_t fx = (~__float_as_uint(d.x)) >> 31, fy = (~__float_as_uint(d.y)) >> 31, fz = (~__float_as_uint(d.z)) >> 31;
 	const float inf = __builtin_huge_valf();
-	float tmx = d.x != 0.f ? ((b.mn[0] + (float)(cx + (sx > 0 ? 1 : 0)) * m.occ.cell[0]) - o.x) * idir.x : inf;
-	float tmy = d.y != 0.f ? ((b.mn[1] + (float)(cy + (sy > 0 ? 1 : 0)) * m.occ.cell[1]) - o.y) * idir.y : inf;
-	float tmz = d.z != 0.f ? ((b.mn[2] + (float)(cz + (sz > 0 ? 1 : 0)) * m.occ.cell[2]) - o.z) * idir.z : inf;
-	const float tdx = fabsf(m.occ.cell[0] * idir.x), tdy = fabsf(m.occ.cell[1] * idir.y), tdz = fabsf(m.occ.cell[2] * idir.z);
 	float t_enter = tnear;
+	uint32_t c = (cz << 10) | (cy << 5) | cx;
 	#pragma unroll 1
 	for (int it = 0; it < (int)(3 * kCoarse); ++it) {
-		const uint32_t idx = ((uint32_t)cz * kCoarse + (uint32_t)cy) * kCoarse + (uint32_t)cx;
-		if ((mask[idx >> 5] >> (idx & 31)) & 1u) return fmaxf(t_enter - 1e-4f, 0.f);
+		cx = c & 31u; cy = (c >> 5) & 31u; cz = c >> 10;
+		const uint32_t m0 = look_bit<0>(mask, c);
+		const uint32_t m1 = look_bit<1>(mask, ((cz >> 1) << 8) | ((cy >> 1) << 4) | (cx >> 1));
+		const uint32_t m2 = look_bit<2>(mask, ((cz >> 2) << 6) | ((cy >> 2) << 3) | (cx >> 2));
+		const uint32_t m3 = look_bit<3>(mask, ((cz >> 3) << 4) | ((cy >> 3) << 2) | (cx >> 3));
+		if (m0) return fmaxf(t_enter - 1e-4f, 0.f);
+		const uint32_t L = m1 ? 0u : (m2 ? 1u : (m3 ? 2u : 3u));
+		__builtin_amdgcn_sched_barrier(0);
+		const uint32_t ex = ((cx >> L) + fx) << L, ey = ((cy >> L) + fy) << L, ez = ((cz >> L) + fz) << L;
+		const float tmx = d.x != 0.f ? ((b.mn[0] + (float)ex * m.occ.cell[0]) - o.x) * idir.x : inf;
+		const float tmy = d.y != 0.f ? ((b.mn[1] + (float)ey * m.occ.cell[1]) - o.y) * idir.y : inf;
+		const float tmz = d.z != 0.f ? ((b.mn[2] + (float)ez * m.occ.cell[2]) - o.z) * idir.z : inf;
 		const bool step_x = tmx <= tmy && tmx <= tmz, step_y = !step_x && tmy <= tmz, step_z = !step_x && !step_y;
 		t_enter = step_x ? tmx : (step_y ? tmy : tmz);
-		cx += step_x ? sx : 0; cy += step_y ? sy : 0; cz += step_z ? sz : 0;
-		tmx += step_x ? tdx : 0.f; tmy += step_y ? tdy : 0.f; tmz += step_z ? tdz : 0.f;
-		if ((uint32_t)(cx | cy | cz) > kCoarse - 1) return -1.f;
+		const uint32_t crossed = (step_x ? ex + fx : (step_y ? ey + fy : ez + fz)) - 1u;
+		if (crossed > kCoarse - 1) return -1.f;
+		__builtin_amdgcn_sched_barrier(0);
+		const f3 q = o + d * t_enter;
+		const uint32_t nx = (uint32_t)__builtin_amdgcn_fmed3f((q.x - b.mn[0]) * m.occ.inv_cell[0], (float)cx, fx ? hi : 0.f);
+		const uint32_t ny = (uint32_t)__builtin_amdgcn_fmed3f((q.y - b.mn[1]) * m.occ.inv_cell[1], (float)cy, fy ? hi : 0.f);
+		const uint32_t nz = (uint32_t)__builtin_amdgcn_fmed3f((q.z - b.mn[2]) * m.occ.inv_cell[2], (float)cz, fz ? hi : 0.f);
+		c = ((step_z ? crossed : nz) << 10) | ((step_y ? crossed : ny) << 5) | (step_x ? crossed : nx);
 	}
 	return 0.f;
 }
@@ -463,10 +479,10 @@
 
 constexpr float kJumpSpan = 0.06f;
 constexpr int kLookEvery = 6;
-constexpr uint32_t kMarchLdsWords = kCoarseWords + kGrid;
+constexpr uint32_t kMarchLdsWords = kLookWords + kGrid;
 __device__ __forceinline__ void stage_march_lds(uint32_t* __restrict__ lds, const uint32_t* __restrict__ mask) {
-	for (uint32_t i = threadIdx.x; i < kCoarseWords; i += blockDim.x) lds[i] = mask[i];
-	for (uint32_t i = threadIdx.x; i < kGrid; i += blockDim.x) lds[kCoarseWords + i] = expand_bits(i);
+	for (uint32_t i = threadIdx.x; i < kLookWords; i += blockDim.x) lds[i] = mask[i];
+	for (uint32_t i = threadIdx.x; i < kGrid; i += blockDim.x) lds[kLookWords + i] = expand_bits(i);
 }
 struct OccWord { uint32_t tag; uint32_t lo, hi; };
 __device__ __forceinline__ uint32_t occupancy_bit_index(f3 pos, uint32_t mip, const uint32_t* __restrict__ march_lds) {
@@ -475,7 +491,7 @@
 	q = q * mip_scale;
 	q = q + mk3(0.5f, 0.5f, 0.5f);
 	const int ix = (int)(q.x * (float)kGrid), iy = (int)(q.y * (float)kGrid), iz = (int)(q.z * (float)kGrid);
-	const uint32_t* spread = march_lds + kCoarseWords;
+	const uint32_t* spread = march_lds + kLookWords;
 	return (spread[clampi_(ix, 0, kGrid - 1)] | (spread[clampi_(iy, 0, kGrid - 1)] << 1) | (spread[clampi_(iz, 0, kGrid - 1)] << 2)) + mip * kGridVol;
 }
 __device__ __forceinline__ bool occupied_at_cached(f3 pos, const uint8_t* __restrict__ bitfield, uint32_t mip, const uint32_t* __restrict__ march_lds, OccWord& w) {
@@ -494,11 +510,11 @@
 	q = q * mip_scale;
 	q = q + mk3(0.5f, 0.5f, 0.5f);
 	const int ix = (int)(q.x * (float)kGrid), iy = (int)(q.y * (float)kGrid), iz = (int)(q.z * (float)kGrid);
-	const uint32_t* spread = march_lds + kCoarseWords;
+	const uint32_t* spread = march_lds + kLookWords;
 	const uint32_t idx = spread[clampi_(ix, 0, kGrid - 1)] | (spread[clampi_(iy, 0, kGrid - 1)] << 1) | (spread[clampi_(iz, 0, kGrid - 1)] << 2);
 	return get_bitfield_at(idx, mip, bitfield);
 }
-template <bool JUMP = false>
+template <bool JUMP = false, bool LOOK_TWICE = false>
 __device__ __forceinline__ bool march_to_occupied(const nrs_render_params& p, const DeviceModel& m, const uint32_t* __restrict__ march_lds, f3 o, f3 d,
                                                   float& t, f3& pos, float& dt, uint32_t* n_iter = nullptr) {
 	const uint32_t* __restrict__ coarse_mask = march_lds;
@@ -536,6 +552,7 @@
 		if (!in_occ && !ray_meets_box_ahead(occ_box, o, idir, t)) return false;
 		if (until_look-- == 0) {
 			until_look = kLookEvery;
+			if (LOOK_TWICE) { f3 o2 = o; asm volatile("" : "+v"(o2.x), "+v"(o2.y), "+v"(o2.z)); const float t2 = coarse_safe_until(m, coarse_mask, o2, d, idir, t); asm volatile("" :: "v"(t2)); }
 			float t_safe = coarse_safe_until(m, coarse_mask, o, d, idir, t);
 			if (t_safe < 0.f) return false;
 			{
@@ -586,7 +603,11 @@
 	float dt = calc_dt(r.t, p.cone_angle_constant);
 	r.t += ld_random_val(SPP ? spp : p.spp_index, pixel_idx * 786433u) * dt;
 	f3 pos;
+#if defined(NRS_MEASURE) && NRS_MEASURE == 6
+	return march_to_occupied<true, true>(p, m, march_lds, r.o, r.d, r.t, pos, dt, n_iter);
+#else
 	return march_to_occupied<true>(p, m, march_lds, r.o, r.d, r.t, pos, dt, n_iter);
+#endif
 }
 
 __device__ __forceinline__ float scalar_tp(f3 a, f3 b, f3 c) { return dot3(a, cross3(b, c)); }
diff --git a/nerfshop_amd/csrc/nrs_internal.h b/nerfshop_amd/csrc/nrs_internal.h
--- a/nerfshop_amd/csrc/nrs_internal.h
+++ b/nerfshop_amd/csrc/nrs_internal.h
@@ -21,6 +21,10 @@
 constexpr uint32_t kCoarse = 32;
 constexpr uint32_t kCoarseWords = kCoarse * kCoarse * kCoarse / 32;
 static_assert((kCoarse & (kCoarse - 1)) == 0, "the block walk's bounds test (cx | cy | cz) needs a power of two");
+constexpr uint32_t kLookLevels = 4;
+constexpr uint32_t look_level_word(uint32_t level) { return level == 0 ? 0u : look_level_word(level - 1) + (kCoarseWords >> (3u * (level - 1))); }
+constexpr uint32_t kLookWords = kCoarseWords + kCoarseWords / 8 + kCoarseWords / 64 + kCoarseWords / 512;
+static_assert(kCoarse == 32 && kCoarseWords / 512 == 2, "four levels down to 4^3 = two words");
 constexpr uint32_t kDensityW = 64 * 32 + 16 * 64;
 constexpr uint32_t kRgbW = 64 * 32 + 64 * 64 + 16 * 64;
 constexpr uint32_t kCanonW = kDensityW + kRgbW + 64 * 64 + 64 * 16;
@@ -197,7 +201,7 @@
                      const float* d_density_grid, float* d_out, int n_cus, void* stream);
 int launch_map_rays(const DeviceEdit& e, uint32_t n, float* d_coords, uint32_t ld, int with_dir, uint8_t* d_empty, void* stream);
 int launch_grid_to_bitfield(const float* d_grid, uint8_t* d_bitfield, float* d_scratch_mean, void* stream);
-int launch_occ_accel(const uint8_t* d_bitfield, uint32_t* d_masks, float* d_out, uint32_t* d_keys, void* stream);
+int launch_occ_accel(const uint8_t* d_bitfield, uint32_t* d_masks, float* d_out, uint32_t* d_keys, bool flat_pyramid, void* stream);
 int launch_grid_update(const DeviceModel& m, const DeviceEdit* d_edits, int n_edits, const nrs_grid_update& u, uint64_t rng_state_nonuniform,
                        float* d_grid, uint32_t* d_grid_tmp, int n_cus, void* stream);
 int launch_accumulate(uint32_t n_pixels, const float* d_frame, float* d_accum, uint32_t sample_count, int color_space, void* stream);
diff --git a/nerfshop_amd/csrc/nrs_occupancy.hip b/nerfshop_amd/csrc/nrs_occupancy.hip
--- a/nerfshop_amd/csrc/nrs_occupancy.hip
+++ b/nerfshop_amd/csrc/nrs_occupancy.hip
@@ -162,19 +162,43 @@
 	}
 	__syncthreads();
 	for (uint32_t j = threadIdx.x; j < 2 * kCoarseWords; j += 256)
-		if (lmask[j]) atomicOr(&masks[j], lmask[j]);
-}
-int launch_occ_accel(const uint8_t* d_bitfield, uint32_t* d_masks, float* d_out, uint32_t* d_keys, void* stream) {
+		if (lmask[j]) atomicOr(&masks[(j / kCoarseWords) * kLookWords + j % kCoarseWords], lmask[j]);
+}
+__global__ void __launch_bounds__(256) occ_accel_pyramid_kernel(uint32_t* __restrict__ masks, uint32_t flat) {
+	__shared__ uint32_t lds[kLookWords];
+	uint32_t* mask = masks + blockIdx.x * kLookWords;
+	for (uint32_t w = threadIdx.x; w < kLookWords; w += 256) lds[w] = w < kCoarseWords ? mask[w] : (flat ? 0xffffffffu : 0u);
+	__syncthreads();
+	uint32_t* child = lds;
+	for (uint32_t L = 1; L < kLookLevels && !flat; ++L) {
+		const uint32_t R = kCoarse >> L, Rc = 2u * R;
+		uint32_t* out = child + Rc * Rc * Rc / 32u;
+		for (uint32_t i = threadIdx.x; i < R * R * R; i += 256) {
+			const uint32_t x = i % R, y = (i / R) % R, z = i / (R * R);
+			uint32_t any = 0u;
+			for (uint32_t c = 0; c < 8u; ++c) {
+				const uint32_t ci = ((2u * z + (c >> 2)) * Rc + 2u * y + ((c >> 1) & 1u)) * Rc + 2u * x + (c & 1u);
+				any |= (child[ci >> 5] >> (ci & 31u)) & 1u;
+			}
+			if (any) atomicOr(&out[i >> 5], 1u << (i & 31u));
+		}
+		__syncthreads();
+		child = out;
+	}
+	for (uint32_t w = kCoarseWords + threadIdx.x; w < kLookWords; w += 256) mask[w] = lds[w];
+}
+int launch_occ_accel(const uint8_t* d_bitfield, uint32_t* d_masks, float* d_out, uint32_t* d_keys, bool flat_pyramid, void* stream) {
 	hipStream_t s = (hipStream_t)stream;
 	static const uint32_t init_keys[12] = {0xffffffffu, 0xffffffffu, 0xffffffffu, 0u, 0u, 0u, 0xffffffffu, 0xffffffffu, 0xffffffffu, 0u, 0u, 0u};
 	hipError_t e = hipMemcpyAsync(d_keys, init_keys, sizeof(init_keys), hipMemcpyHostToDevice, s);
-	if (e == hipSuccess) e = hipMemsetAsync(d_masks, 0, 2 * kCoarseWords * 4, s);
+	if (e == hipSuccess) e = hipMemsetAsync(d_masks, 0, 2 * kLookWords * 4, s);
 	if (e != hipSuccess) return hip_fail(e, "occ_accel: clear");
 	const uint32_t n_words = kCascades * (kGridVol / 64);
 	static_assert(kCascades * (kGridVol / 64) % 256 == 0, "one thread per bitfield word, no tail");
 	hipLaunchKernelGGL(occ_accel_bounds_kernel, dim3(n_words / 256), dim3(256), 0, s, (const uint64_t*)d_bitfield, d_keys);
 	hipLaunchKernelGGL(occ_accel_box_kernel, dim3(1), dim3(64), 0, s, d_keys, (OccAccelOut*)d_out);
 	hipLaunchKernelGGL(occ_accel_mask_kernel, dim3(kAccelMaskBlocks), dim3(256), 0, s, (const uint64_t*)d_bitfield, (const OccAccelOut*)d_out, d_masks);
+	hipLaunchKernelGGL(occ_accel_pyramid_kernel, dim3(2), dim3(256), 0, s, d_masks, flat_pyramid ? 1u : 0u);
 	NRS_LAUNCH_CHECK("occ_accel launch");
 	return NRS_OK;
 }
diff --git a/nerfshop_amd/csrc/nrs_render.cuh b/nerfshop_amd/csrc/nrs_render.cuh
--- a/nerfshop_amd/csrc/nrs_render.cuh
+++ b/nerfshop_amd/csrc/nrs_render.cuh
@@ -360,6 +360,15 @@
 			}
 			if (TEAM != 1) alive = alive && first_of_team;
 			const unsigned long long am = __ballot(alive);
+#if NRS_MEASURE == 7
+			if (!BATCH && am == 0ull && inside) {
+				uint32_t x2 = x; asm volatile("" : "+v"(x2));
+				Ray r2 = init_ray<EXTRA>(p1, x2, y, off_x, off_y);
+				bool a2 = r2.alive;
+				if (a2) a2 = first_hit(p1, m1, sm.coarse, x2 + (uint32_t)p1.resolution[0] * y, r2, nullptr);
+				asm volatile("" :: "v"(r2.t), "s"((int)__ballot(a2)));
+			}
+#endif
 			if (alive) {
 				const uint32_t slot = ring_head + ring_count + __builtin_amdgcn_mbcnt_hi((uint32_t)(am >> 32), __builtin_amdgcn_mbcnt_lo((uint32_t)am, 0u));
 				ring[slot & (kRing - 1)] = make_uint2(BATCH ? x | (y << kBatchXYBits) | (bs << (2u * kBatchXYBits)) : x | (y << 16), __float_as_uint(t0));
diff --git a/nerfshop_amd/runtime.py b/nerfshop_amd/runtime.py
--- a/nerfshop_amd/runtime.py
+++ b/nerfshop_amd/runtime.py
@@ -156,6 +156,12 @@
         check(self.lib.nrs_model_get_march_accelerator(self.h, int(which), box.ctypes.data, mask.ctypes.data))
         bits = np.unpackbits(mask.view(np.uint8), bitorder="little").reshape(32, 32, 32).astype(bool)
         return box, bits
+
+    def get_look_pyramid(self, which):
+        words = np.zeros(128 + 16 + 2, np.uint32)
+        check(self.lib.nrs_model_get_look_pyramid(self.h, int(which), words.ctypes.data))
+        bits = np.unpackbits(words.view(np.uint8), bitorder="little").astype(bool)
+        return bits[:4096].reshape(16, 16, 16), bits[4096:4608].reshape(8, 8, 8), bits[4608:4672].reshape(4, 4, 4)
 
     def get_density_grid(self):
         out = np.zeros(_abi.GRID_VOLUME * _abi.GRID_CASCADES, np.float32)
```

Result: no change. 13200 Msamples/s (-0.3%).
